# lazzati-astro/MCRaT

Hardware: AMD Instinct MI355X
Metric: photon-scatter-events/sec at 1e6 photons, 2D FLASH jet (higher is better)
Workload: dtype f64

## Files before the change

include/mcrat_hip.h:

```cpp
#ifndef MCRAT_HIP_H
#define MCRAT_HIP_H

#include <stddef.h>
#include <stdint.h>

#ifdef __cplusplus
extern "C" {
#endif
#if defined(__GNUC__)
#pragma GCC visibility push(default)
#endif

#define MCRAT_HIP_ABI_VERSION 1

#define MCRAT_HIP_OK        0
#define MCRAT_HIP_EINVAL   (-1)
#define MCRAT_HIP_ENODEV   (-2)
#define MCRAT_HIP_ENOMEM   (-3)
#define MCRAT_HIP_EHIP     (-4)
#define MCRAT_HIP_ESTATE   (-5)
#define MCRAT_HIP_EREFUSED (-6)

#define MCRAT_HIP_CARTESIAN        0
#define MCRAT_HIP_SPHERICAL        1
// ... 251 lines not shown
#define MCRAT_HIP_MODE_FAST  1
int mcrat_hip_propagate_frame_mode(mcrat_hip_ctx *ctx, double *time_now, double remaining_time, uint64_t seed, int mode, int fast_windows,
                                   mcrat_hip_frame_stats *stats);
int mcrat_hip_pool_propagate_frames_fast(mcrat_hip_ctx *pool, const int *open, const uint64_t *seeds, const double *time_now,
                                         const double *remaining_time, int fast_windows, mcrat_hip_frame_stats *stats);
int mcrat_hip_fast_cadence(mcrat_hip_ctx *ctx, int set_windows);

int mcrat_hip_begin_frame(mcrat_hip_ctx *ctx, uint64_t seed, double time_now, double remaining_time);
int mcrat_hip_run(mcrat_hip_ctx *ctx, long long max_iterations, mcrat_hip_frame_stats *stats);

int mcrat_hip_snapshot_photons(mcrat_hip_ctx *ctx);
int mcrat_hip_restore_photons(mcrat_hip_ctx *ctx);

int mcrat_hip_num_virtual_ranks(const mcrat_hip_ctx *ctx);
int mcrat_hip_rank_stats(mcrat_hip_ctx *ctx, int rank, mcrat_hip_frame_stats *stats);

typedef struct mcrat_hip_rank_summary {
    double min_r, max_r, min_theta, max_theta;
    double avg_scatt, avg_r;
    double avg_energy;
    int    max_scatt, min_scatt;
    int    num_output;
    int    list_capacity;
} mcrat_hip_rank_summary;
int mcrat_hip_profile_totals(const mcrat_hip_ctx *ctx, double *loop_kernel_ms, long long *loop_kernel_launches);
int mcrat_hip_pool_create(mcrat_hip_ctx *pool, int n_ranks, int slots_per_rank);
int mcrat_hip_pool_rank(mcrat_hip_ctx *pool, int rank, uint32_t rng_stream, mcrat_hip_ctx **view);
int mcrat_hip_pool_summaries(mcrat_hip_ctx *pool, mcrat_hip_rank_summary *out );
typedef struct mcrat_hip_pool_cs_list {
    int      open;
    int      emit_pool;
    int      scatt_frame_number, inj_frame_number;
    uint64_t seed;
    double   time_now, remaining_time;
    double   r_inj, ph_weight_suggest, theta_min, theta_max;
} mcrat_hip_pool_cs_list;
int mcrat_hip_pool_scatter_frames_cyclosynch(mcrat_hip_ctx *pool, const mcrat_hip_cyclosynch *cs, int max_photons, double fps,
                                             const mcrat_hip_pool_cs_list *lists, mcrat_hip_frame_stats *stats, mcrat_hip_cyclosynch_counts *counts);
typedef struct mcrat_hip_pool_inject_list {
    int      inject;
    char     spect;
    int      min_photons, max_photons;
    double   r_inj, ph_weight, theta_min, theta_max;
    uint64_t seed;
    int      num_photons;
    double   ph_weight_adjusted;
    int      status;
} mcrat_hip_pool_inject_list;
int mcrat_hip_pool_inject_photons(mcrat_hip_ctx *pool, double fps, mcrat_hip_pool_inject_list *lists);
int mcrat_hip_pool_set_photons(mcrat_hip_ctx *pool, int count, const int *rank_of, const mcrat_hip_photon_list *lists);
int mcrat_hip_pool_begin_frames(mcrat_hip_ctx *pool, const int *open, const uint64_t *seeds, const double *time_now, const double *remaining_time);
int mcrat_hip_pool_frame_stats(mcrat_hip_ctx *pool, mcrat_hip_frame_stats *out );
int mcrat_hip_pool_layout(const mcrat_hip_ctx *pool, int *n_ranks, int *slots_per_rank);
typedef struct mcrat_hip_frame_plan {
    int n_frames;
    int chain_clock;
    int restore_each_frame;
    int capture_frames;
    const int      *open;
    const uint64_t *seeds;
    const double   *time_now;
    const double   *remaining_time;
    const double   *frame_end;
    mcrat_hip_ctx *const *hydro;
} mcrat_hip_frame_plan;
int mcrat_hip_pool_run_frames(mcrat_hip_ctx *pool, const mcrat_hip_frame_plan *plan, mcrat_hip_frame_stats *stats );

int mcrat_hip_pool_select_frame(mcrat_hip_ctx *pool, int frame);

int mcrat_hip_step_locate_sample(mcrat_hip_ctx *ctx, int find_nearest_block_switch);
int mcrat_hip_frame_statistics(mcrat_hip_ctx *ctx, mcrat_hip_frame_stats *stats);
int mcrat_hip_update_photon_position(mcrat_hip_ctx *ctx, double t);
int mcrat_hip_step_event(mcrat_hip_ctx *ctx, mcrat_hip_frame_stats *stats);

size_t mcrat_hip_shared_clock_bytes_per_rank(void);
int mcrat_hip_shared_clock_attach(mcrat_hip_ctx *ctx, int world, int rank, long long slot_base, void *send, void *recv);
int mcrat_hip_shared_clock_buffers(mcrat_hip_ctx *ctx, void **send, void **recv);
int mcrat_hip_shared_clock_attach_device(mcrat_hip_ctx *ctx, int world, int rank, long long slot_base);
int mcrat_hip_shared_clock_peer_buffers(mcrat_hip_ctx *ctx, void **recv, size_t *recv_bytes, void **flags, size_t *flags_bytes);
int mcrat_hip_shared_clock_set_peers(mcrat_hip_ctx *ctx, void *const *peer_recv, void *const *peer_flags);
int mcrat_hip_shared_clock_exchange_push(mcrat_hip_ctx *ctx);
int mcrat_hip_shared_clock_exchange_wait(mcrat_hip_ctx *ctx);
int mcrat_hip_shared_clock_exchange(mcrat_hip_ctx *ctx);
int mcrat_hip_shared_clock_reset_exchange(mcrat_hip_ctx *ctx);
int mcrat_hip_shared_clock_propose(mcrat_hip_ctx *ctx);
int mcrat_hip_shared_clock_resolve(mcrat_hip_ctx *ctx);
int mcrat_hip_shared_clock_poll(mcrat_hip_ctx *ctx, int *frame_done, mcrat_hip_frame_stats *stats);
int mcrat_hip_shared_clock_finish(mcrat_hip_ctx *ctx, mcrat_hip_frame_stats *stats);

int mcrat_hip_set_rng_tape(mcrat_hip_ctx *ctx, const double *uniforms, long long n);
int mcrat_hip_rng_tape_position(mcrat_hip_ctx *ctx, long long *position, int *ran_out);

int mcrat_hip_pool_set_rng_tapes(mcrat_hip_ctx *pool, const double *const *uniforms , const long long *n );
int mcrat_hip_pool_rng_tape_positions(mcrat_hip_ctx *pool, long long *position , int *ran_out );

#define MCRAT_HIP_FN_KN_CROSS_SECTION       1
#define MCRAT_HIP_FN_LORENTZ_BOOST_PHOTON   2
#define MCRAT_HIP_FN_LORENTZ_BOOST_ELECTRON 3
#define MCRAT_HIP_FN_STOKES_ROTATION        4
#define MCRAT_HIP_FN_THERMAL_ELECTRON       5
#define MCRAT_HIP_FN_THERMAL_ELECTRON_WAVE  6
#define MCRAT_HIP_FN_ELECTRON_AND_SCATTER   7
#define MCRAT_HIP_FN_RCP_NR                 8
#define MCRAT_HIP_FN_RSQRT_NR               9
#define MCRAT_HIP_FN_SQRT_NR               10
#define MCRAT_HIP_FN_CELL_OPERANDS         11
#define MCRAT_HIP_FN_BOOST_WITH_PHOTON     12
#define MCRAT_HIP_FN_BOOST_WITH_ELECTRON   13
#define MCRAT_HIP_FN_BOOST_STAGED_PHOTON   14
#define MCRAT_HIP_FN_OPTICAL_DEPTH_STAGED  15
#define MCRAT_HIP_FN_AZIMUTH               16
#define MCRAT_HIP_FN_HYDRO_COORDS          17
#define MCRAT_HIP_FN_THERMAL_CROSS_SECTION 18
#define MCRAT_HIP_FN_KN_CROSS_SECTION_IEEE 19
#define MCRAT_HIP_FN_COUNT                 20
int mcrat_hip_eval_function(mcrat_hip_ctx *ctx, int fn, int n, const double *in, double *out, uint64_t seed);

int mcrat_hip_ph_minmax(mcrat_hip_ctx *ctx, double *min_r, double *max_r, double *min_theta, double *max_theta);
int mcrat_hip_scatt_stats(mcrat_hip_ctx *ctx, int *max_scatt, int *min_scatt, double *avg_scatt, double *avg_r);
int mcrat_hip_avg_energy(mcrat_hip_ctx *ctx, double *erg);

typedef struct mcrat_hip_observer {
    int n_obs; const double *cos_obs, *sin_obs, *cos_lo, *cos_hi;
    int n_t;   const double *t_edges;
    int n_e;   const double *e_edges;
} mcrat_hip_observer;
typedef struct mcrat_hip_observation {
    long long *count; double *w, *we, *i, *q, *u, *v;
    long long *n_accepted, *n_outside;
} mcrat_hip_observation;
int mcrat_hip_observe(mcrat_hip_ctx *ctx, const mcrat_hip_observer *obs, double time_now, mcrat_hip_observation *out);
int mcrat_hip_pool_observe(mcrat_hip_ctx *pool, const mcrat_hip_observer *obs, const double *time_now , mcrat_hip_observation *out);
int mcrat_hip_observe_path(const mcrat_hip_ctx *ctx);

#define MCRAT_HIP_SIGHTLINE_SKIPPED 0
#define MCRAT_HIP_SIGHTLINE_LEFT_MESH 1
#define MCRAT_HIP_SIGHTLINE_OPAQUE 2
#define MCRAT_HIP_SIGHTLINE_STEP_CAP 3
#define MCRAT_HIP_SIGHTLINE_OFF_TABLE 4
typedef struct mcrat_hip_sightline_params { double step_frac, h_min; int max_steps; double tau_stop, surface_level; } mcrat_hip_sightline_params;
typedef struct mcrat_hip_sightlines {
    double *tau, *path; int *steps, *status; int *surface_step; double *surface_r0, *surface_r1, *surface_r2;
    long long n_status[5];
} mcrat_hip_sightlines;
int mcrat_hip_sightline_rays(mcrat_hip_ctx *ctx, const mcrat_hip_ctx *hydro , const mcrat_hip_sightline_params *params, int n,
                             const double *r0, const double *r1, const double *r2, const double *p0, const double *p1, const double *p2,
                             const double *p3 , mcrat_hip_sightlines *out);
int mcrat_hip_sightline_photons(mcrat_hip_ctx *ctx, const mcrat_hip_ctx *hydro, const mcrat_hip_sightline_params *params, mcrat_hip_sightlines *out);
int mcrat_hip_pool_sightline_photons(mcrat_hip_ctx *pool, const mcrat_hip_ctx *hydro, const mcrat_hip_sightline_params *params, mcrat_hip_sightlines *out);

int mcrat_hip_synchronize(mcrat_hip_ctx *ctx);
size_t mcrat_hip_device_bytes(const mcrat_hip_ctx *ctx);
int mcrat_hip_lookup_cell(mcrat_hip_ctx *ctx, int n, const double *a0, const double *a1, const double *a2, int *cell_out);

#if defined(__GNUC__)
#pragma GCC visibility pop
#endif
#ifdef __cplusplus
}
#endif
#endif
```

mcrat_amd/csrc/device_types.hpp:

```cpp
#pragma once
#include <stddef.h>
#include <stdint.h>

namespace mcrat {

constexpr double A_RAD = 7.56e-15;
constexpr double C_LIGHT = 2.99792458e10;
constexpr double PL_CONST = 6.6260755e-27;
constexpr double K_B = 1.380658e-16;
constexpr double M_P = 1.6726231e-24;
constexpr double THOM_X_SECT = 6.65246e-25;
constexpr double M_EL = 9.1093879e-28;

constexpr int GEOM_CARTESIAN = 0, GEOM_SPHERICAL = 1, GEOM_CYLINDRICAL = 2, GEOM_POLAR = 3;
constexpr int DIM_TWO = 0, DIM_TWO_POINT_FIVE = 1, DIM_THREE = 2;

constexpr unsigned FLAG_RECALC = 1u;
constexpr unsigned FLAG_MOVES = 2u;
constexpr unsigned FLAG_VALID = 4u;
constexpr unsigned FLAG_TAU_FRESH = 8u;

constexpr int TOPK = 4;
constexpr int MAX_SEG = 8;
constexpr int STEP_BLOCK = 256;
constexpr int STEP_QCAP = 1024;
#ifndef MCRAT_EVENT_BLOCK
#define MCRAT_EVENT_BLOCK 256
#endif
constexpr int SHORTLIST_CAP = MCRAT_EVENT_BLOCK;
constexpr int EVENT_BLOCK = MCRAT_EVENT_BLOCK;

struct PhotonDev {
    double *r0, *r1, *r2;
    double *p0, *p1, *p2, *p3;
    double *c0, *c1, *c2, *c3;
    double *s0, *s1, *s2, *s3;
    double *num_scatt;
    double *weight;
    double *tau;
    double *tts;
    double *u0, *u1, *u2;
    double *ntau;
    double *tau_next;
    int *idx;
    unsigned char *flags;
    char *type;
    int n;
    int n_pad;
    unsigned col_stride;
};
#if defined(__HIPCC__)
__host__ __device__
#endif
inline void offset_photons(PhotonDev &ph, size_t first)
{
    double **cols[24] = {&ph.r0, &ph.r1, &ph.r2, &ph.p0, &ph.p1, &ph.p2, &ph.p3, &ph.c0, &ph.c1, &ph.c2, &ph.c3, &ph.s0, &ph.s1, &ph.s2, &ph.s3,
                         &ph.num_scatt, &ph.weight, &ph.tau, &ph.tts, &ph.u0, &ph.u1, &ph.u2, &ph.ntau, &ph.tau_next};
    for (int k = 0; k < 24; ++k) *cols[k] += first;
    ph.idx += first; ph.flags += first; ph.type += first;
}

struct alignas(32) CellGeom {
    double c0, c1, s0, s1;
};
struct alignas(16) CellGeom2 {
    double c2, s2;
};
struct alignas(32) CellFluid {
    double a, b, c, w;
    double nsig, gam, kf, pad;
};
#if defined(__HIPCC__)
__host__ __device__
#endif
inline void cell_staged_operands(double a, double b, double c, double gamma_cell, double dens_lab, CellFluid &f)
{
    const double beta_g = __builtin_sqrt(1.0 - 1.0 / (gamma_cell * gamma_cell));
    const double v2 = (a * a + b * b) + c * c;
    f.a = a; f.b = b; f.c = c;
    f.w = beta_g / __builtin_sqrt(v2);
    f.nsig = (dens_lab / M_P) * THOM_X_SECT;
    f.gam = 1.0 / __builtin_sqrt(1.0 - v2);
    f.kf = (f.gam * f.gam) / (f.gam + 1.0);
    f.pad = 0.0;
}

struct alignas(32) FatCell {
    double c0, c1, s0, s1;
    double a, b, w, nsig;
    double gam;
    int cell;
    int pad;
    double c;
    double c2, s2;
    double pad2[3];
};
static_assert(sizeof(FatCell) == 128, "one cache line per bucket-list entry");

constexpr unsigned GRID_NO_HINT = 15u;
constexpr int GRID_CODE_OCT_SHIFT = 27;
constexpr int GRID_CODE_HINT_OK = 1 << 30;
constexpr int GRID_CODE_BUCKET_MASK = (1 << GRID_CODE_OCT_SHIFT) - 1;
struct alignas(16) BucketDir {
    int e0;
    int n;
    unsigned hints;
    unsigned pad;
};

struct GridDev {
    const BucketDir *dir;
    const FatCell *cells;
    double org[3];
    double inv[3];
    int dim[3];
    int logmap[3];
    int naxes;
};

struct HydroDev {
    const CellGeom *geom;
    const CellGeom2 *geom2;
    const CellFluid *fluid;
    const double *temp;
    const double *fluid_c;
    const double *gamma;
    const double *k2e;
    int M;
    double dom0[2], dom1[2], dom2[2];
    GridDev grid;
    const double *hot_table;
    int hot_n_ph_e, hot_n_t;
    double hot_e0, hot_de, hot_t0, hot_dt;
    int *table_fallbacks;
    int hot_fallback_calls;
};

struct alignas(16) Cand {
    double t;
    int idx;
    int pad;
};

struct alignas(256) LoopState {
    double remaining_time;
    double time_now;
    unsigned long long iteration;
    int done;
    int nseg;
    int skip_idx;
    int last_scattered_index;
    double seg[MAX_SEG];
    double last_time_step;
    double last_scattered_temp;
    long long iterations;
    long long frame_scatt_cnt;
    long long n_relocated;
    long long not_found;
    long long kn_rejections;
    long long rescans;
    double t_cut;
    double t_est;
    int force_relocate;
    int photon_event_called;
    union {
        long long stamps[8];
        long long slot_steps;
    };
};

struct alignas(16) Shortlist {
    int count;
    int pad[3];
    Cand items[SHORTLIST_CAP];
};

struct alignas(16) RankDesc {
    int len;
    uint32_t stream;
    uint64_t seed;
};

struct RngKey {
    uint64_t seed;
    uint32_t stream;
    uint32_t slot_base;
};

constexpr int SC_K = 4;
constexpr int SC_MAX_WORLD = 16;
constexpr int LOOP_DONE = 1;
constexpr int LOOP_MIDPASS = 2;
constexpr int LOOP_SC_GAVE_UP = 4;

struct alignas(16) ScRecord {
    double t;
    long long gid;
    double r[3], u[3], p[4], pc[4], s[4];
    int cell;
    unsigned flags;
};

struct alignas(16) ScProposal {
    int n;
    int pad0;
    long long horizon_gid;
    double horizon_t;
    double pad1;
    ScRecord rec[SC_K];
};

struct alignas(64) ScState {
    double cursor_t;
    long long cursor_gid;
    double old_scatt_time;
    double t_first;
    double cut_mid;
    int first;
    int pad0;
    long long rounds, midpass_rounds;
};

}
```

mcrat_amd/csrc/engine.hip:

```cpp
#include <hip/hip_runtime.h>
#include <algorithm>
#include <chrono>
#include <cmath>
#include <cstdio>
#include <cstdlib>
#include <cstring>
#include <mutex>
#include <new>
#include <string>
#include <vector>

#include "../../include/mcrat_hip.h"
#include "device_types.hpp"
#include "launch.hpp"
#include "observe_plan.hpp"
#include "sightline_plan.hpp"
#include "photon_cols.hpp"
#include "photon_plan.hpp"
#include "rng.hpp"

using namespace mcrat;

static_assert(sizeof(mcrat_hip_photon) == 176, "struct photon layout (Src/mcrat.h:142-171) must be 176 bytes");
static_assert(offsetof(mcrat_hip_photon, num_scatt) == 128 && offsetof(mcrat_hip_photon, recalc_properties) == 136 &&
// ... 360 lines not shown
    if (c->obs_buf) (void)hipFree(c->obs_buf);
    if (c->sl_buf) (void)hipFree(c->sl_buf);
    if (c->own_stream && c->stream) (void)hipStreamDestroy(c->stream);
    delete c;
}

extern "C" int mcrat_hip_bind_thread(mcrat_hip_ctx *c)
{
    if (!c) return MCRAT_HIP_EINVAL;
    if (hipSetDevice(c->cfg.device) != hipSuccess) return MCRAT_HIP_ENODEV;
    return MCRAT_HIP_OK;
}

extern "C" int mcrat_hip_synchronize(mcrat_hip_ctx *c)
{
    if (!c) return MCRAT_HIP_EINVAL;
    HIPCHK(c, hipStreamSynchronize(c->stream));
    return MCRAT_HIP_OK;
}

extern "C" size_t mcrat_hip_device_bytes(const mcrat_hip_ctx *c)
{
    if (!c) return 0;
    return c->ph_bytes + c->hy_bytes + c->grid_bytes + c->grid_count_cap * sizeof(unsigned) + sizeof(Shortlist) + sizeof(LoopState) + c->partials_bytes +
           sizeof(ReducePartial) * mcrat_hip_ctx::RED_BLOCKS + c->obs_bytes + c->sl_bytes;
}

extern "C" int mcrat_hip_create_hot_cross_section(mcrat_hip_ctx *c, double *thermal_table, int n_ph_e, int n_t, double log_ph_e_min,
                                                  double log_ph_e_max, double log_t_min, double log_t_max, long long calls, uint64_t seed)
{
    if (!c || !thermal_table || n_ph_e < 1 || n_t < 1 || n_ph_e > 100000 || n_t > 100000 || calls < 1 || !(log_ph_e_max > log_ph_e_min) ||
        !(log_t_max > log_t_min))
        return MCRAT_HIP_EINVAL;
    const size_t count = (size_t)(n_ph_e + 1) * (size_t)(n_t + 1);
    if (count > 0x7fffffffull) return MCRAT_HIP_EINVAL;
    double *d = nullptr;
    HIPCHK(c, hipMalloc((void **)&d, count * sizeof(double)));
    HotTableParams p{n_ph_e, n_t, log_ph_e_min, log_ph_e_max, log_t_min, log_t_max, calls, (unsigned long long)seed};
    __atomic_store_n(&c->hot_creating, 1, __ATOMIC_RELEASE);
    hipError_t e = launch_hot_table(p, d, c->stream);
    if (e == hipSuccess) e = hipMemcpyAsync(thermal_table, d, count * sizeof(double), hipMemcpyDeviceToHost, c->stream);
    if (e == hipSuccess) e = hipStreamSynchronize(c->stream);
    __atomic_store_n(&c->hot_creating, 0, __ATOMIC_RELEASE);
    (void)hipFree(d);
    HIPCHK(c, e);
    return MCRAT_HIP_OK;
}


static void apply_hot_table(mcrat_hip_ctx *c)
{
    HydroDev &hy = c->hy;
    const bool table = c->cfg.tau_calculation == MCRAT_HIP_TAU_TABLE && c->d_hot_table;
    hy.hot_table = table ? c->d_hot_table : nullptr;
    hy.hot_n_ph_e = c->hot_n_ph_e; hy.hot_n_t = c->hot_n_t;
    hy.hot_e0 = c->hot_grid[0]; hy.hot_t0 = c->hot_grid[2];
    hy.hot_de = table ? (c->hot_grid[1] - c->hot_grid[0]) / c->hot_n_ph_e : 0.0;
    hy.hot_dt = table ? (c->hot_grid[3] - c->hot_grid[2]) / c->hot_n_t : 0.0;
    hy.table_fallbacks = c->d_table_fallbacks;
    hy.hot_fallback_calls = c->hot_fallback_calls;
}

extern "C" int mcrat_hip_table_fallback_calls(mcrat_hip_ctx *c, int calls)
{
    if (!c) return MCRAT_HIP_EINVAL;
    if (calls > 0) {
        c->hot_fallback_calls = calls;
        apply_hot_table(c);
        drop_graph(c);
        sync_views(c);
    }
    return c->hot_fallback_calls;
}

extern "C" int mcrat_hip_set_hot_cross_section(mcrat_hip_ctx *c, const double *thermal_table, int n_ph_e, int n_t,
                                               double log_ph_e_min, double log_ph_e_max, double log_t_min, double log_t_max)
{
    if (!c || !thermal_table || n_ph_e < 1 || n_t < 1 || !(log_ph_e_max > log_ph_e_min) || !(log_t_max > log_t_min)) return MCRAT_HIP_EINVAL;
    if (c->parent) return view_refuses(c, "set_hot_cross_section");
    if (c->cfg.tau_calculation != MCRAT_HIP_TAU_TABLE) { c->last_error = "the context was created with TAU_CALCULATION == DIRECT"; return MCRAT_HIP_ESTATE; }
    const size_t count = (size_t)(n_ph_e + 1) * (size_t)(n_t + 1);
    for (size_t k = 0; k < count; ++k)
        if (!(thermal_table[k] == thermal_table[k])) { c->last_error = "NaN in the cross-section table"; return MCRAT_HIP_EINVAL; }
    HIPCHK(c, hipStreamSynchronize(c->stream));
    release_shared_hydro(c);
    detach_sharers(c, "replaced its cross-section table");
    if (c->d_hot_table) { (void)hipFree(c->d_hot_table); c->d_hot_table = nullptr; }
    HIPCHK(c, hipMalloc((void **)&c->d_hot_table, count * sizeof(double)));
    HIPCHK(c, hipMemcpy(c->d_hot_table, thermal_table, count * sizeof(double), hipMemcpyHostToDevice));
    c->hot_n_ph_e = n_ph_e; c->hot_n_t = n_t;
    c->hot_grid[0] = log_ph_e_min; c->hot_grid[1] = log_ph_e_max; c->hot_grid[2] = log_t_min; c->hot_grid[3] = log_t_max;
    apply_hot_table(c);
    drop_graph(c);
    sync_views(c);
    return MCRAT_HIP_OK;
}

static int ensure_aos(mcrat_hip_ctx *c, size_t bytes);
static int flush_pending(mcrat_hip_ctx *c);

static void sync_views(mcrat_hip_ctx *c)
{
    for (mcrat_hip_ctx *v : c->views) {
        if (!v) continue;
        v->hy = c->hy;
        v->hcol = c->hcol; v->hcol_buf = c->hcol_buf; v->hcol_M = c->hcol_M;
        v->have_hydro = c->have_hydro;
        v->d_hot_table = c->d_hot_table; v->hot_n_ph_e = c->hot_n_ph_e; v->hot_n_t = c->hot_n_t;
        v->hot_fallback_calls = c->hot_fallback_calls;
        for (int k = 0; k < 4; ++k) v->hot_grid[k] = c->hot_grid[k];
        drop_graph(v);
    }
}

static int ensure_counts(mcrat_hip_ctx *c, size_t n)
{
    if (c->parent) {
        int rc = ensure_counts(c->parent, n);
        c->grid_count = c->parent->grid_count; c->grid_count_cap = c->parent->grid_count_cap; c->d_grid_total = c->parent->d_grid_total;
        return rc;
    }
    if (!c->d_grid_total) HIPCHK(c, hipMalloc((void **)&c->d_grid_total, sizeof(unsigned long long)));
    if (c->grid_count_cap < n) {
        if (c->grid_count) { HIPCHK(c, hipFree(c->grid_count)); c->grid_count = nullptr; c->grid_count_cap = 0; }
        HIPCHK(c, hipMalloc((void **)&c->grid_count, sizeof(unsigned) * n));
        c->grid_count_cap = n;
    }
    return MCRAT_HIP_OK;
}

static int view_refuses(mcrat_hip_ctx *c, const char *what)
{
    c->last_error = std::string(what) + ": a rank view shares its pool's hydro frame; call this on the pool context";
    return MCRAT_HIP_ESTATE;
}

static int capture_refuses(mcrat_hip_ctx *c, const char *what)
{
    if (c->selected_frame < 0) return MCRAT_HIP_OK;
    c->last_error = std::string(what) + ": a captured frame is selected (mcrat_hip_pool_select_frame(pool, -1) first)";
    return MCRAT_HIP_ESTATE;
}

namespace {

struct HydroStage {
    mcrat_hip_ctx *c;
    int M, naxes;
    CellLayout cells{};
    GridLayout grid{};
    GridScale scale{};
    GridPlan plan{};
    long long nb = 0, entries = 0;
    bool any_hot = false;
    template <class T> T *cell_at(size_t o) const { return reinterpret_cast<T *>(static_cast<char *>(c->hy_buf) + o); }
    template <class T> T *grid_at(size_t o) const { return reinterpret_cast<T *>(static_cast<char *>(c->grid_buf) + o); }
};
struct HostFrame {
    const mcrat_hip_hydro *h;
    GridHost grid;
    std::vector<char> image;
};

int host_build_grid(HydroStage &s, HostFrame &hf)
{
    const mcrat_hip_hydro *h = hf.h;
    const double *ctr[3] = {h->r0, h->r1, h->r2}, *size[3] = {h->r0_size, h->r1_size, h->r2_size};
    if (!build_grid(ctr, size, s.M, s.naxes, hf.grid)) { s.c->last_error = "cell-lookup grid: degenerate mesh"; return MCRAT_HIP_EINVAL; }
    s.plan = hf.grid.plan; s.nb = hf.grid.nb; s.entries = (long long)hf.grid.cells.size();
    for (int i = 0; i < s.M; ++i) s.any_hot = s.any_hot || (h->temp[i] >= 1e7);
    return MCRAT_HIP_OK;
}

int ensure_cell_buffer(HydroStage &s, bool reserve_k2e)
{
    mcrat_hip_ctx *c = s.c;
    s.cells = cell_layout(c->kc.dimensions, s.M, reserve_k2e);
    HIPCHK(c, hipStreamSynchronize(c->stream));
    return ensure_device_bytes(c, &c->hy_buf, &c->hy_bytes, s.cells.total);
}

int stage_cells_device(HydroStage &s)
{
    mcrat_hip_ctx *c = s.c;
    const CellLayout &l = s.cells;
    const int M = s.M, nblk = stage_cells_blocks(M), stride = plan_stride(M), nsamp = (M + stride - 1) / stride;
    const size_t scratch_bytes = sizeof(StagePartial) * (size_t)nblk + sizeof(double) * 2 * s.naxes * (size_t)nsamp;
    int rc = ensure_aos(c, scratch_bytes);
    if (rc) return rc;
    StagePartial *d_part = static_cast<StagePartial *>(c->aos_buf);
    double *d_samp = reinterpret_cast<double *>(d_part + nblk);
    HIPCHK(c, launch_stage_cells(c->kc.dimensions, c->kc.geometry, c->hcol, M, s.cell_at<CellGeom>(l.geom), l.has_geom2 ? s.cell_at<CellGeom2>(l.geom2) : nullptr,
                                 s.cell_at<CellFluid>(l.fluid), l.has_fluid_c ? s.cell_at<double>(l.fluid_c) : nullptr, s.cell_at<double>(l.temp),
                                 s.cell_at<double>(l.gamma), d_part, d_samp, stride, nsamp, c->stream));
    std::vector<char> hs(scratch_bytes);
    HIPCHK(c, hipMemcpyAsync(hs.data(), c->aos_buf, scratch_bytes, hipMemcpyDeviceToHost, c->stream));
    HIPCHK(c, hipStreamSynchronize(c->stream));
    const StagePartial *part = reinterpret_cast<const StagePartial *>(hs.data());
    const MeshStats ms = mesh_stats_from_partials(part, nblk, reinterpret_cast<const double *>(part + nblk), nsamp, s.naxes, &s.any_hot);
    if (!grid_plan_from_stats(ms, M, s.naxes, s.scale)) { c->last_error = "cell-lookup grid: degenerate mesh"; return MCRAT_HIP_EINVAL; }
    return MCRAT_HIP_OK;
}

int stage_cells_host(HydroStage &s, HostFrame &hf)
{
    mcrat_hip_ctx *c = s.c;
    const mcrat_hip_hydro *h = hf.h;
    const CellLayout &l = s.cells;
    const int M = s.M;
    hf.image.assign(l.total, 0);
    char *host = hf.image.data();
    CellGeom *geom = reinterpret_cast<CellGeom *>(host + l.geom);
    CellFluid *fluid = reinterpret_cast<CellFluid *>(host + l.fluid);
    double *fc = l.has_fluid_c ? reinterpret_cast<double *>(host + l.fluid_c) : nullptr;
    for (int i = 0; i < M; ++i) {
        geom[i].c0 = h->r0[i]; geom[i].c1 = h->r1[i]; geom[i].s0 = h->r0_size[i]; geom[i].s1 = h->r1_size[i];
        double v[3];
        cell_velocity_staged(c->kc.dimensions, c->kc.geometry, h->v0[i], h->v1[i], l.has_fluid_c ? h->v2[i] : 0.0, h->r1[i], l.has_geom2 ? h->r2[i] : 0.0, v);
        if (fc) fc[i] = v[2];
        cell_staged_operands(v[0], v[1], v[2], h->gamma[i], h->dens_lab[i], fluid[i]);
    }
    if (l.has_geom2) {
        CellGeom2 *g2 = reinterpret_cast<CellGeom2 *>(host + l.geom2);
        for (int i = 0; i < M; ++i) { g2[i].c2 = h->r2[i]; g2[i].s2 = h->r2_size[i]; }
    }
    memcpy(host + l.temp, h->temp, sizeof(double) * M);
    memcpy(host + l.gamma, h->gamma, sizeof(double) * M);
    HIPCHK(c, hipMemcpy(c->hy_buf, host, l.total, hipMemcpyHostToDevice));
    return MCRAT_HIP_OK;
}

void publish_cells(HydroStage &s, const double *dom0, const double *dom1, const double *dom2)
{
    const CellLayout &l = s.cells;
    HydroDev &hy = s.c->hy;
    hy.geom = s.cell_at<const CellGeom>(l.geom);
    hy.geom2 = l.has_geom2 ? s.cell_at<const CellGeom2>(l.geom2) : nullptr;
    hy.fluid = s.cell_at<const CellFluid>(l.fluid);
    hy.temp = s.cell_at<const double>(l.temp);
    hy.fluid_c = l.has_fluid_c ? s.cell_at<const double>(l.fluid_c) : nullptr;
    hy.k2e = s.any_hot ? s.cell_at<const double>(l.k2e) : nullptr;
    hy.gamma = s.cell_at<const double>(l.gamma);
    hy.M = s.M;
    hy.dom0[0] = dom0[0]; hy.dom0[1] = dom0[1];
    hy.dom1[0] = dom1[0]; hy.dom1[1] = dom1[1];
    hy.dom2[0] = dom2[0]; hy.dom2[1] = dom2[1];
}

int count_grid_entries(HydroStage &s, const GridPlan &plan, long long nb, unsigned long long *total)
{
    mcrat_hip_ctx *c = s.c;
    { int rc = ensure_counts(c, (size_t)nb); if (rc) return rc; }
    HIPCHK(c, grid_count(plan, c->hy.geom, c->hy.geom2, s.M, c->grid_count, nb, c->d_grid_total, c->stream));
    HIPCHK(c, hipMemcpyAsync(total, c->d_grid_total, sizeof *total, hipMemcpyDeviceToHost, c->stream));
    HIPCHK(c, hipStreamSynchronize(c->stream));
    return MCRAT_HIP_OK;
}
int choose_scale_device(HydroStage &s)
{
    mcrat_hip_ctx *c = s.c;
    int rc = ensure_counts(c, 1);
    if (rc) return rc;
    const GridChoice ch = choose_grid_scale(s.scale, s.M, [&](const GridPlan &plan, long long nb, long long) {
        unsigned long long total = 0;
        rc = count_grid_entries(s, plan, nb, &total);
        return rc ? -1LL : (long long)std::min(total, 0x7fffffffffffffffull);
    });
    if (ch.result == GRID_SCALE_ABANDONED) return rc;
    if (ch.result != GRID_SCALE_OK) { c->last_error = "cell-lookup grid: no bucket size fits this mesh"; return MCRAT_HIP_EINVAL; }
    s.plan = ch.plan; s.nb = ch.nb; s.entries = ch.entries;
    if (getenv("MCRAT_HIP_VERBOSE"))
        fprintf(stderr, "mcrat_hip: cell-lookup grid %d x %d x %d buckets, %lld entries for %d cells (%.2f per bucket), built on the device\n",
                s.plan.dim[0], s.plan.dim[1], s.plan.dim[2], s.entries, s.M, (double)s.entries / (double)s.nb);
    return MCRAT_HIP_OK;
}

int ensure_grid_buffer(HydroStage &s)
{
    s.grid = grid_layout(s.nb, s.entries, grid_scan_scratch_ints(s.nb));
    return ensure_device_bytes(s.c, &s.c->grid_buf, &s.c->grid_bytes, s.grid.total);
}

int build_grid_device(HydroStage &s)
{
    mcrat_hip_ctx *c = s.c;
    const GridLayout &g = s.grid;
    HIPCHK(c, grid_build(s.plan, c->hy.geom, c->hy.geom2, c->hy.fluid, c->hy.fluid_c, s.M, c->grid_count, s.grid_at<int>(g.start), s.grid_at<int>(g.scan),
                         s.grid_at<int>(g.entries), s.grid_at<FatCell>(g.cells), s.grid_at<BucketDir>(g.dir), s.nb, s.entries, c->stream));
    HIPCHK(c, hipStreamSynchronize(c->stream));
    return MCRAT_HIP_OK;
}

int upload_host_grid(HydroStage &s, const HostFrame &hf)
{
    const GridHost &g = hf.grid;
    const CellGeom *geom = reinterpret_cast<const CellGeom *>(hf.image.data() + s.cells.geom);
    const CellFluid *fluid = reinterpret_cast<const CellFluid *>(hf.image.data() + s.cells.fluid);
    const bool three = s.cells.has_geom2;
    std::vector<char> gh(s.grid.start, 0);
    BucketDir *dir = reinterpret_cast<BucketDir *>(gh.data() + s.grid.dir);
    for (size_t b = 0; b < (size_t)s.nb; ++b) {
        dir[b].e0 = g.start[b]; dir[b].n = g.start[b + 1] - g.start[b]; dir[b].hints = g.hints[b]; dir[b].pad = 0;
    }
    FatCell *fat = reinterpret_cast<FatCell *>(gh.data() + s.grid.cells);
    for (size_t e = 0; e < g.cells.size(); ++e) {
        const int ci = g.cells[e];
        fat[e] = fat_cell(geom[ci], fluid[ci], three ? hf.h->r2[ci] : 0.0, three ? hf.h->r2_size[ci] : 0.0, ci);
    }
    HIPCHK(s.c, hipMemcpy(s.c->grid_buf, gh.data(), s.grid.start, hipMemcpyHostToDevice));
    return MCRAT_HIP_OK;
}

void publish_grid(HydroStage &s)
{
    HydroDev &hy = s.c->hy;
    hy.grid.dir = s.grid_at<const BucketDir>(s.grid.dir);
    hy.grid.cells = s.grid_at<const FatCell>(s.grid.cells);
    grid_plan_to_dev(s.plan, hy.grid);
    apply_hot_table(s.c);
}

int finish_frame(HydroStage &s)
{
    mcrat_hip_ctx *c = s.c;
    if (s.any_hot) {
        HIPCHK(c, launch_k2e(c->hy.temp, s.cell_at<double>(s.cells.k2e), s.M, c->stream));
        HIPCHK(c, hipStreamSynchronize(c->stream));
    }
    c->have_hydro = true;
    drop_graph(c);
    sync_views(c);
    return MCRAT_HIP_OK;
}

}

static int stage_hydro_device(HydroStage &s, const double *dom0, const double *dom1, const double *dom2)
{
    int rc;
    if ((rc = ensure_cell_buffer(s, true))) return rc;
    if ((rc = stage_cells_device(s))) return rc;
    publish_cells(s, dom0, dom1, dom2);
    if ((rc = choose_scale_device(s))) return rc;
    if ((rc = ensure_grid_buffer(s))) return rc;
    if ((rc = build_grid_device(s))) return rc;
    publish_grid(s);
    return finish_frame(s);
}
static int stage_hydro_host(HydroStage &s, const mcrat_hip_hydro *h, const double *dom0, const double *dom1, const double *dom2)
{
    HostFrame hf{h};
    int rc;
    if ((rc = host_build_grid(s, hf))) return rc;
    if ((rc = ensure_cell_buffer(s, s.any_hot))) return rc;
    if ((rc = stage_cells_host(s, hf))) return rc;
    publish_cells(s, dom0, dom1, dom2);
    if ((rc = ensure_grid_buffer(s))) return rc;
    if ((rc = upload_host_grid(s, hf))) return rc;
    publish_grid(s);
    return finish_frame(s);
}
static int stage_hydro(mcrat_hip_ctx *c, const mcrat_hip_hydro *h, int M, const double *dom0, const double *dom1, const double *dom2)
{
    if (c->hydro_owner) { c->last_error = "stage_hydro on a context that reads another one's frame"; return MCRAT_HIP_ESTATE; }
    HydroStage s{c, M, c->kc.dimensions == DIM_THREE ? 3 : 2};
    return h ? stage_hydro_host(s, h, dom0, dom1, dom2) : stage_hydro_device(s, dom0, dom1, dom2);
}

static void release_shared_hydro(mcrat_hip_ctx *c)
{
    std::lock_guard<std::mutex> lock(g_share_mutex);
    if (!c->hydro_owner) return;
    auto &v = c->hydro_owner->hydro_sharers;
    v.erase(std::remove(v.begin(), v.end(), c), v.end());
    forget_shared_frame(c);
}

extern "C" int mcrat_hip_share_hydro(mcrat_hip_ctx *c, mcrat_hip_ctx *owner)
{
    if (!c || !owner || c == owner) return MCRAT_HIP_EINVAL;
    if (c->parent) return view_refuses(c, "share_hydro");
    if (owner->parent) owner = owner->parent;
    if (!owner->have_hydro || owner->hydro_owner == c) return MCRAT_HIP_ESTATE;
    if (owner->hydro_owner) owner = owner->hydro_owner;
    if (c->kc.dimensions != owner->kc.dimensions || c->kc.geometry != owner->kc.geometry || c->kc.table != owner->kc.table ||
        c->cfg.device != owner->cfg.device) {
        c->last_error = "share_hydro: the two contexts differ in DIMENSIONS / GEOMETRY / TAU_CALCULATION or device";
        return MCRAT_HIP_EINVAL;
    }
    HIPCHK(c, hipStreamSynchronize(c->stream));
    HIPCHK(c, hipStreamSynchronize(owner->stream));
    release_shared_hydro(c);
    detach_sharers(c, "shares another context's frame now");
    if (c->hy_buf) { HIPCHK(c, hipFree(c->hy_buf)); c->hy_buf = nullptr; c->hy_bytes = 0; }
    if (c->grid_buf) { HIPCHK(c, hipFree(c->grid_buf)); c->grid_buf = nullptr; c->grid_bytes = 0; }
    if (c->hcol_buf) { HIPCHK(c, hipFree(c->hcol_buf)); c->hcol_buf = nullptr; c->hcol_bytes = 0; }
    if (c->d_hot_table) { HIPCHK(c, hipFree(c->d_hot_table)); c->d_hot_table = nullptr; }
    c->hy = owner->hy;
    c->hcol = owner->hcol; c->hcol_buf = owner->hcol_buf; c->hcol_M = owner->hcol_M;
    c->d_hot_table = owner->d_hot_table; c->hot_n_ph_e = owner->hot_n_ph_e; c->hot_n_t = owner->hot_n_t;
    for (int k = 0; k < 4; ++k) c->hot_grid[k] = owner->hot_grid[k];
    apply_hot_table(c);
    c->have_hydro = true;
    {
        std::lock_guard<std::mutex> lock(g_share_mutex);
        c->hydro_owner = owner;
        owner->hydro_sharers.push_back(c);
    }
    c->frame_open = false;
    drop_graph(c);
    sync_views(c);
    return MCRAT_HIP_OK;
}

static int ensure_hcol(mcrat_hip_ctx *c, int M)
{
    release_shared_hydro(c);
    detach_sharers(c, "staged another frame");
    const size_t stride = align_up(sizeof(double) * (size_t)M, 256), total = 19 * stride;
    HIPCHK(c, hipStreamSynchronize(c->stream));
    { int rc = ensure_device_bytes(c, &c->hcol_buf, &c->hcol_bytes, total); if (rc) return rc; }
    char *b = static_cast<char *>(c->hcol_buf);
    double **cols[19] = {&c->hcol.r0, &c->hcol.r1, &c->hcol.r2, &c->hcol.s0, &c->hcol.s1, &c->hcol.s2, &c->hcol.v0, &c->hcol.v1, &c->hcol.v2,
                         &c->hcol.dens, &c->hcol.dens_lab, &c->hcol.pres, &c->hcol.temp, &c->hcol.gamma, &c->hcol.r, &c->hcol.theta,
                         &c->hcol.B0, &c->hcol.B1, &c->hcol.B2};
    for (int k = 0; k < 19; ++k) *cols[k] = reinterpret_cast<double *>(b + k * stride);
    c->hcol_M = M;
    return MCRAT_HIP_OK;
}

extern "C" int mcrat_hip_set_hydro(mcrat_hip_ctx *c, const mcrat_hip_hydro *h)
{
    if (!c || !h || h->num_elements <= 0) return MCRAT_HIP_EINVAL;
    if (c->parent) return view_refuses(c, "set_hydro");
    const int M = h->num_elements;
    const bool three = c->kc.dimensions == DIM_THREE, two = c->kc.dimensions == DIM_TWO;
    if (!h->r0 || !h->r1 || !h->r0_size || !h->r1_size || !h->v0 || !h->v1 || !h->dens_lab || !h->temp || !h->gamma) return MCRAT_HIP_EINVAL;
    if (three && (!h->r2 || !h->r2_size)) return MCRAT_HIP_EINVAL;
    if (!two && !h->v2) return MCRAT_HIP_EINVAL;
    c->have_hydro = false;
    sync_views(c);
    int rc = ensure_hcol(c, M);
    if (rc) return rc;
    HIPCHK(c, hipMemsetAsync(c->hcol_buf, 0, c->hcol_bytes, c->stream));
    const struct { double *dst; const double *src; } copy[12] = {
        {c->hcol.r0, h->r0}, {c->hcol.r1, h->r1}, {c->hcol.r2, three ? h->r2 : nullptr}, {c->hcol.s0, h->r0_size}, {c->hcol.s1, h->r1_size},
        {c->hcol.s2, three ? h->r2_size : nullptr}, {c->hcol.v0, h->v0}, {c->hcol.v1, h->v1}, {c->hcol.v2, !two ? h->v2 : nullptr},
        {c->hcol.dens_lab, h->dens_lab}, {c->hcol.temp, h->temp}, {c->hcol.gamma, h->gamma}};
    for (const auto &cp : copy)
        if (cp.src) HIPCHK(c, hipMemcpyAsync(cp.dst, cp.src, sizeof(double) * (size_t)M, hipMemcpyHostToDevice, c->stream));
    HIPCHK(c, launch_fill_spherical(c->kc.dimensions, c->kc.geometry, c->hcol, M, c->stream));
    return stage_hydro(c, getenv("MCRAT_HIP_HOST_GRID") ? h : nullptr, M, h->r0_domain, h->r1_domain, h->r2_domain);
}

extern "C" void mcrat_hip_outflow_defaults(int simulation_type, mcrat_hip_outflow *o)
{
    if (!o) return;
    memset(o, 0, sizeof *o);
    o->simulation_type = simulation_type;
    if (simulation_type == MCRAT_HIP_CYLINDRICAL_OUTFLOW) { o->gamma_infinity = 100; o->t_comov = 1e5; o->ddensity = 3e-7; }
    if (simulation_type == MCRAT_HIP_SPHERICAL_OUTFLOW) { o->gamma_infinity = 100; o->lumi = 1e54; o->r00 = 1e8; }
    if (simulation_type == MCRAT_HIP_STRUCTURED_SPHERICAL_OUTFLOW) { o->gamma_infinity = 100; o->lumi = 1e52; o->r00 = 1e8; o->theta_j = 1e-2; o->p = 4; }
}

namespace {

struct RawPacker {
    mcrat_hip_ctx *c;
    size_t off = 0;
    std::vector<std::pair<size_t, std::pair<const void *, size_t>>> items;
    size_t add(const void *src, size_t bytes) { const size_t o = off; off = align_up(off + bytes, 256); items.push_back({o, {src, bytes}}); return o; }
// ... 2965 lines not shown
    double *d_in = reinterpret_cast<double *>(d + plan.out_bytes);
    ObserveDev a{};
    a.n_slots = n_slots; a.n_obs = plan.n_obs; a.n_t = plan.n_t; a.n_e = plan.n_e; a.n_bins = plan.n_bins;
    a.staged = d_in;
    a.clocks = clocks ? d_in + plan.staged_doubles : nullptr;
    a.slots_per_clock = slots_per_clock;
    a.time_now = time_now;
    a.cube = reinterpret_cast<double *>(d);
    a.n_accepted = reinterpret_cast<unsigned long long *>(d + plan.cube_bytes);
    a.n_outside = a.n_accepted + n_obs;
    HIPCHK(c, hipMemsetAsync(d, 0, plan.out_bytes, c->stream));
    HIPCHK(c, hipMemcpyAsync(d_in, in.data(), sizeof(double) * in.size(), hipMemcpyHostToDevice, c->stream));
    HIPCHK(c, launch_observe(c->ph, a, plan, c->kc.stokes != 0, device_cus(c), c->stream));
    const size_t plane = sizeof(double) * (size_t)plan.n_bins;
    void *planes[OBSERVE_PLANES] = {out->count, out->w, out->we, out->i, out->q, out->u, out->v};
    static_assert(sizeof(long long) == 8, "the count plane is read back as it is");
    for (int k = 0; k < OBSERVE_PLANES; ++k)
        if (planes[k]) HIPCHK(c, hipMemcpyAsync(planes[k], d + plane * (size_t)k, plane, hipMemcpyDeviceToHost, c->stream));
    if (out->n_accepted) HIPCHK(c, hipMemcpyAsync(out->n_accepted, a.n_accepted, sizeof(long long) * n_obs, hipMemcpyDeviceToHost, c->stream));
    if (out->n_outside) HIPCHK(c, hipMemcpyAsync(out->n_outside, a.n_outside, sizeof(long long) * n_obs, hipMemcpyDeviceToHost, c->stream));
    HIPCHK(c, hipStreamSynchronize(c->stream));
    c->obs_path = plan.path;
    return MCRAT_HIP_OK;
}

extern "C" int mcrat_hip_observe(mcrat_hip_ctx *c, const mcrat_hip_observer *obs, double time_now, mcrat_hip_observation *out)
{
    if (!c || !obs || !out) return MCRAT_HIP_EINVAL;
    if (!c->have_photons) return MCRAT_HIP_ESTATE;
    if (c->is_pool) { c->last_error = "observe: a rank pool's lists have clocks of their own (mcrat_hip_pool_observe, or mcrat_hip_observe on a view)"; return MCRAT_HIP_ESTATE; }
    int rc = flush_pending(c);
    if (rc) return rc;
    return observe_run(c, obs, c->ph.n, nullptr, 0, 1, time_now, out);
}

extern "C" int mcrat_hip_pool_observe(mcrat_hip_ctx *c, const mcrat_hip_observer *obs, const double *time_now, mcrat_hip_observation *out)
{
    if (!c || !obs || !time_now || !out) return MCRAT_HIP_EINVAL;
    if (!c->is_pool) return MCRAT_HIP_ESTATE;
    return observe_run(c, obs, c->ph.n, time_now, c->n_ranks, c->rank_stride, 0.0, out);
}

extern "C" int mcrat_hip_observe_path(const mcrat_hip_ctx *c) { return c ? c->obs_path : 0; }

static int sightline_run(mcrat_hip_ctx *c, const mcrat_hip_ctx *hydro, const mcrat_hip_sightline_params *params, int n, const double *const *rays,
                         mcrat_hip_sightlines *out)
{
    const mcrat_hip_ctx *h = hydro ? hydro : c;
    if (!h->have_hydro) { c->last_error = "sightline: no staged hydro frame"; return MCRAT_HIP_ESTATE; }
    if (h != c && (h->kc.dimensions != c->kc.dimensions || h->kc.geometry != c->kc.geometry || h->kc.table != c->kc.table || h->cfg.device != c->cfg.device)) {
        c->last_error = "sightline: a frame staged on a context with other switches (DIMENSIONS, GEOMETRY, TAU_CALCULATION) or on another device";
        return MCRAT_HIP_EINVAL;
    }
    if (c->kc.table && !h->hy.hot_table) {
        c->last_error = "TAU_CALCULATION == TABLE needs mcrat_hip_set_hot_cross_section first";
        return MCRAT_HIP_ESTATE;
    }
    const SightlineParams p{params->step_frac, params->h_min, params->max_steps, params->tau_stop, params->surface_level};
    int forced;
    SightlinePlan plan;
    const SightlineRefusal bad_switch = sightline_refill_switch(getenv("MCRAT_HIP_SIGHTLINE_REFILL"), &forced);
    SightlineRefusal why = sightline_plan(n, p, forced, &plan);
    if (why == SIGHTLINE_OK) why = bad_switch;
    if (why != SIGHTLINE_OK) { c->last_error = sightline_refusal_text(why); return MCRAT_HIP_EINVAL; }

    mcrat_hip_ctx *owner = c->parent ? c->parent : c;
    HIPCHK(c, hipStreamSynchronize(c->stream));
    if (h != c) HIPCHK(c, hipStreamSynchronize(h->stream));
    int rc = ensure_device_bytes(c, &owner->sl_buf, &owner->sl_bytes, plan.ray_offset + (rays ? plan.ray_bytes : 0));
    if (rc) return rc;
    char *d = static_cast<char *>(owner->sl_buf);
    const int blocks = sightline_grid(plan, device_cus(c));
    SightlineDev a{};
    a.n = n;
    a.step_frac = p.step_frac; a.h_min = p.h_min; a.max_steps = p.max_steps; a.tau_stop = p.tau_stop; a.surface_level = p.surface_level;
    a.head = reinterpret_cast<unsigned long long *>(d);
    a.f8 = reinterpret_cast<double *>(d + plan.f8_offset);
    a.i4 = reinterpret_cast<int *>(d + plan.i4_offset);
    a.refill = plan.refill ? 1 : 0;
    a.own_rays = plan.refill ? sightline_own_rays(n, blocks) : 0;
    HIPCHK(c, hipMemsetAsync(d, 0, sizeof(unsigned long long) * SIGHTLINE_HEAD_WORDS, c->stream));
    if (rays) {
        double *d_ray = reinterpret_cast<double *>(d + plan.ray_offset);
        for (int k = 0; k < SIGHTLINE_RAY_PLANES; ++k)
            HIPCHK(c, hipMemcpyAsync(d_ray + (size_t)k * (size_t)n, rays[k], sizeof(double) * (size_t)n, hipMemcpyHostToDevice, c->stream));
        a.ray = d_ray;
    }
    HIPCHK(c, launch_sightline(c->kc, c->ph, h->hy, a, blocks, c->stream));
    double *f8[SIGHTLINE_F8_PLANES] = {out->tau, out->path, out->surface_r0, out->surface_r1, out->surface_r2};
    int *i4[SIGHTLINE_I4_PLANES] = {out->steps, out->status, out->surface_step};
    for (int k = 0; k < SIGHTLINE_F8_PLANES; ++k)
        if (f8[k]) HIPCHK(c, hipMemcpyAsync(f8[k], d + sightline_f8_plane(plan, k), sizeof(double) * (size_t)n, hipMemcpyDeviceToHost, c->stream));
    for (int k = 0; k < SIGHTLINE_I4_PLANES; ++k)
        if (i4[k]) HIPCHK(c, hipMemcpyAsync(i4[k], d + sightline_i4_plane(plan, k), sizeof(int) * (size_t)n, hipMemcpyDeviceToHost, c->stream));
    static_assert(sizeof(long long) == 8, "the status counts are read back as they are");
    HIPCHK(c, hipMemcpyAsync(out->n_status, d, sizeof(long long) * SIGHTLINE_N_STATUS, hipMemcpyDeviceToHost, c->stream));
    HIPCHK(c, hipStreamSynchronize(c->stream));
    return MCRAT_HIP_OK;
}

extern "C" int mcrat_hip_sightline_rays(mcrat_hip_ctx *c, const mcrat_hip_ctx *hydro, const mcrat_hip_sightline_params *params, int n, const double *r0,
                                        const double *r1, const double *r2, const double *p0, const double *p1, const double *p2, const double *p3,
                                        mcrat_hip_sightlines *out)
{
    if (!c || !params || !out) return MCRAT_HIP_EINVAL;
    if (n > 0 && (!r0 || !r1 || !r2 || !p0 || !p1 || !p2 || !p3)) { c->last_error = "sightline: a null ray array"; return MCRAT_HIP_EINVAL; }
    if (c->have_photons) {
        int rc = flush_pending(c);
        if (rc) return rc;
    }
    const double *const rays[SIGHTLINE_RAY_PLANES] = {r0, r1, r2, p0, p1, p2, p3};
    return sightline_run(c, hydro, params, n, rays, out);
}

extern "C" int mcrat_hip_sightline_photons(mcrat_hip_ctx *c, const mcrat_hip_ctx *hydro, const mcrat_hip_sightline_params *params, mcrat_hip_sightlines *out)
{
    if (!c || !params || !out) return MCRAT_HIP_EINVAL;
    if (!c->have_photons) return MCRAT_HIP_ESTATE;
    if (c->is_pool) { c->last_error = "sightline: one list is a stand-alone context or a view of a pool (mcrat_hip_pool_sightline_photons takes the pool)"; return MCRAT_HIP_ESTATE; }
    int rc = flush_pending(c);
    if (rc) return rc;
    return sightline_run(c, hydro, params, c->ph.n, nullptr, out);
}

extern "C" int mcrat_hip_pool_sightline_photons(mcrat_hip_ctx *c, const mcrat_hip_ctx *hydro, const mcrat_hip_sightline_params *params, mcrat_hip_sightlines *out)
{
    if (!c || !params || !out) return MCRAT_HIP_EINVAL;
    if (!c->is_pool) return MCRAT_HIP_ESTATE;
    int rc = flush_pending(c);
    if (rc) return rc;
    return sightline_run(c, hydro, params, c->ph.n, nullptr, out);
}

extern "C" int mcrat_hip_eval_function(mcrat_hip_ctx *c, int fn, int n, const double *in, double *out, uint64_t seed)
{
    static const int in_w[MCRAT_HIP_FN_COUNT] = {0, 1, 7, 7, 13, 5, 5, 9, 1, 1, 1, 5, 9, 9, 7, 9, 2, 3, 2, 1};
    static const int out_w[MCRAT_HIP_FN_COUNT] = {0, 1, 4, 4, 4, 4, 4, 13, 1, 1, 1, 5, 4, 4, 4, 2, 4, 3, 4, 1};
    if (!c || n <= 0 || !in || !out || fn < 1 || fn >= MCRAT_HIP_FN_COUNT) return MCRAT_HIP_EINVAL;
    if (fn == MCRAT_HIP_FN_THERMAL_CROSS_SECTION && __atomic_load_n(&c->hot_creating, __ATOMIC_ACQUIRE)) return MCRAT_HIP_EINVAL;
    const size_t bi = sizeof(double) * (size_t)in_w[fn] * (size_t)n, bo = sizeof(double) * (size_t)out_w[fn] * (size_t)n;
    double *d_in = nullptr, *d_out = nullptr;
    HIPCHK(c, hipMalloc((void **)&d_in, bi));
    if (hipMalloc((void **)&d_out, bo) != hipSuccess) { (void)hipFree(d_in); return MCRAT_HIP_ENOMEM; }
    hipError_t e = hipMemcpyAsync(d_in, in, bi, hipMemcpyHostToDevice, c->stream);
    if (e == hipSuccess) e = launch_eval_function(c->kc, c->hy, fn, n, d_in, d_out, seed, c->key.stream, c->stream);
    if (e == hipSuccess) e = hipMemcpyAsync(out, d_out, bo, hipMemcpyDeviceToHost, c->stream);
    if (e == hipSuccess) e = hipStreamSynchronize(c->stream);
    (void)hipFree(d_in);
    (void)hipFree(d_out);
    HIPCHK(c, e);
    return MCRAT_HIP_OK;
}

extern "C" int mcrat_hip_lookup_cell(mcrat_hip_ctx *c, int n, const double *a0, const double *a1, const double *a2, int *out)
{
    if (!c || n <= 0 || !a0 || !a1 || !out) return MCRAT_HIP_EINVAL;
    if (!c->have_hydro) return MCRAT_HIP_ESTATE;
    double *d = nullptr;
    int *dout = nullptr;
    HIPCHK(c, hipMalloc((void **)&d, sizeof(double) * 3 * (size_t)n));
    if (hipMalloc((void **)&dout, sizeof(int) * (size_t)n) != hipSuccess) { (void)hipFree(d); return MCRAT_HIP_ENOMEM; }
    int rc = MCRAT_HIP_OK;
    std::vector<double> zeros;
    if (!a2) { zeros.assign(n, 0.0); a2 = zeros.data(); }
    if (hipMemcpy(d, a0, sizeof(double) * n, hipMemcpyHostToDevice) != hipSuccess ||
        hipMemcpy(d + n, a1, sizeof(double) * n, hipMemcpyHostToDevice) != hipSuccess ||
        hipMemcpy(d + 2 * (size_t)n, a2, sizeof(double) * n, hipMemcpyHostToDevice) != hipSuccess ||
        launch_lookup(c->kc, c->hy, n, d, d + n, d + 2 * (size_t)n, dout, c->stream) != hipSuccess ||
        hipStreamSynchronize(c->stream) != hipSuccess ||
        hipMemcpy(out, dout, sizeof(int) * n, hipMemcpyDeviceToHost) != hipSuccess) {
        c->last_error = "lookup_cell failed";
        rc = MCRAT_HIP_EHIP;
    }
    (void)hipFree(d);
    (void)hipFree(dout);
    return rc;
}
```

mcrat_amd/csrc/grid_build.hip:

```cpp
#include <hip/hip_runtime.h>
#include <math.h>
#include "device_types.hpp"
#include "launch.hpp"

namespace mcrat {

namespace {

__device__ __forceinline__ int bucket_of(double x, int logmap, double org, double inv, int dim)
{
    const double u = logmap ? log(x) : x;
    const double f = floor((u - org) * inv);
    if (!(f == f)) return 0;
    if (f < 0.0) return 0;
    if (f > (double)(dim - 1)) return dim - 1;
    return (int)f;
}

struct CellBox {
    double c[3], s[3];
};

__device__ __forceinline__ CellBox load_box(const CellGeom *geom, const CellGeom2 *geom2, int i, int naxes)
{
// ... 1 lines not shown
    CellBox b;
    b.c[0] = g.c0; b.c[1] = g.c1; b.s[0] = g.s0; b.s[1] = g.s1;
    b.c[2] = 0; b.s[2] = 0;
    if (naxes == 3) { const CellGeom2 g2 = geom2[i]; b.c[2] = g2.c2; b.s[2] = g2.s2; }
    return b;
}

__device__ __forceinline__ void bucket_range(const GridPlan &p, const CellBox &b, int lo[3], int hi[3])
{
#pragma unroll
    for (int k = 0; k < 3; ++k) {
        lo[k] = 0; hi[k] = 0;
        if (k < p.naxes) {
            const double m = 1e-9 * (fabs(b.c[k]) + b.s[k]);
            double a = b.c[k] - 0.5 * b.s[k] - m;
            const double e = b.c[k] + 0.5 * b.s[k] + m;
            if (p.logmap[k] && a <= 0) a = 1e-300;
            lo[k] = bucket_of(a, p.logmap[k], p.org[k], p.inv[k], p.dim[k]);
            hi[k] = bucket_of(e, p.logmap[k], p.org[k], p.inv[k], p.dim[k]);
        }
    }
}

__global__ __launch_bounds__(256) void grid_count_kernel(GridPlan p, const CellGeom *__restrict__ geom, const CellGeom2 *__restrict__ geom2, int M,
                                                         unsigned *__restrict__ count, unsigned long long *__restrict__ total)
{
    __shared__ unsigned long long s_sum[4];
    const int i = blockIdx.x * 256 + threadIdx.x;
    unsigned long long mine = 0;
    if (i < M) {
        const CellBox b = load_box(geom, geom2, i, p.naxes);
        int lo[3], hi[3];
        bucket_range(p, b, lo, hi);
        mine = (unsigned long long)(hi[0] - lo[0] + 1) * (hi[1] - lo[1] + 1) * (hi[2] - lo[2] + 1);
        if (mine > 4096) mine = 1ull << 40;
        else
            for (int z = lo[2]; z <= hi[2]; ++z)
                for (int y = lo[1]; y <= hi[1]; ++y)
                    for (int x = lo[0]; x <= hi[0]; ++x) atomicAdd(&count[((size_t)z * p.dim[1] + y) * p.dim[0] + x], 1u);
    }
    for (int off = 32; off > 0; off >>= 1) mine += __shfl_xor(mine, off, 64);
    if ((threadIdx.x & 63) == 0) s_sum[threadIdx.x >> 6] = mine;
    __syncthreads();
    if (threadIdx.x == 0) atomicAdd(total, s_sum[0] + s_sum[1] + s_sum[2] + s_sum[3]);
}

constexpr int SCAN_PER_BLOCK = 2048;

__global__ __launch_bounds__(256) void scan_blocks_kernel(const unsigned *__restrict__ count, long long n, int *__restrict__ start, int *__restrict__ sums)
{
    __shared__ int s_w[4];
    const long long base = (long long)blockIdx.x * SCAN_PER_BLOCK + (long long)threadIdx.x * 8;
    int v[8], acc = 0;
#pragma unroll
    for (int k = 0; k < 8; ++k) {
        const long long e = base + k;
        const int c = (e < n) ? (int)count[e] : 0;
        v[k] = acc;
        acc += c;
    }
    int incl = acc;
    const int lane = threadIdx.x & 63, w = threadIdx.x >> 6;
    for (int off = 1; off < 64; off <<= 1) {
        const int o = __shfl_up(incl, off, 64);
        if (lane >= off) incl += o;
    }
    if (lane == 63) s_w[w] = incl;
    __syncthreads();
    int wbase = 0;
    for (int k = 0; k < w; ++k) wbase += s_w[k];
    const int excl = wbase + incl - acc;
#pragma unroll
    for (int k = 0; k < 8; ++k) {
        const long long e = base + k;
        if (e < n) start[e] = excl + v[k];
    }
    if (threadIdx.x == 255) sums[blockIdx.x] = wbase + incl;
}

__global__ __launch_bounds__(256) void scan_sums_kernel(int *__restrict__ sums, int nblocks)
{
    __shared__ int s_w[4];
    __shared__ int s_carry;
    if (threadIdx.x == 0) s_carry = 0;
    __syncthreads();
    for (int b0 = 0; b0 < nblocks; b0 += 256) {
        const int e = b0 + threadIdx.x;
        const int c = (e < nblocks) ? sums[e] : 0;
        int incl = c;
        const int lane = threadIdx.x & 63, w = threadIdx.x >> 6;
        for (int off = 1; off < 64; off <<= 1) {
            const int o = __shfl_up(incl, off, 64);
            if (lane >= off) incl += o;
        }
        if (lane == 63) s_w[w] = incl;
        __syncthreads();
        int wbase = s_carry;
        for (int k = 0; k < w; ++k) wbase += s_w[k];
        if (e < nblocks) sums[e] = wbase + incl - c;
        __syncthreads();
        if (threadIdx.x == 255) s_carry = wbase + incl;
        __syncthreads();
    }
}

__global__ __launch_bounds__(256) void scan_add_kernel(int *__restrict__ start, long long n, const int *__restrict__ sums, int total)
{
    const long long e = (long long)blockIdx.x * 256 + threadIdx.x;
    if (e < n) start[e] += sums[e / SCAN_PER_BLOCK];
    if (e == n) start[e] = total;
}

__global__ __launch_bounds__(256) void grid_fill_kernel(GridPlan p, const CellGeom *__restrict__ geom, const CellGeom2 *__restrict__ geom2, int M,
                                                        const int *__restrict__ start, unsigned *__restrict__ cursor, int *__restrict__ entries)
{
    const int i = blockIdx.x * 256 + threadIdx.x;
    if (i >= M) return;
    const CellBox b = load_box(geom, geom2, i, p.naxes);
    int lo[3], hi[3];
    bucket_range(p, b, lo, hi);
    for (int z = lo[2]; z <= hi[2]; ++z)
        for (int y = lo[1]; y <= hi[1]; ++y)
            for (int x = lo[0]; x <= hi[0]; ++x) {
                const size_t bk = ((size_t)z * p.dim[1] + y) * p.dim[0] + x;
                const unsigned pos = atomicAdd(&cursor[bk], 1u);
                entries[start[bk] + (int)pos] = i;
            }
}

__device__ __forceinline__ double mapped(double x, int logmap) { return logmap ? log(fmax(x, 1e-300)) : x; }

__global__ __launch_bounds__(256) void grid_records_kernel(int naxes, long long total, const int *__restrict__ entries,
                                                           const CellGeom *__restrict__ geom, const CellGeom2 *__restrict__ geom2,
                                                           const CellFluid *__restrict__ fluid, const double *__restrict__ fluid_c,
                                                           FatCell *__restrict__ cells)
{
    const long long e = (long long)blockIdx.x * 256 + threadIdx.x;
    if (e >= total) return;
    const int ci = entries[e];
    const CellGeom g = geom[ci];
    const CellFluid f = fluid[ci];
    FatCell fc;
    fc.c0 = g.c0; fc.c1 = g.c1; fc.s0 = g.s0; fc.s1 = g.s1;
    fc.a = f.a; fc.b = f.b; fc.c = f.c; fc.w = f.w;
    fc.nsig = f.nsig; fc.gam = f.gam;
    fc.c2 = 0; fc.s2 = 0;
    if (naxes == 3) { const CellGeom2 g2 = geom2[ci]; fc.c2 = g2.c2; fc.s2 = g2.s2; }
    fc.cell = ci; fc.pad = 0; fc.pad2[0] = fc.pad2[1] = fc.pad2[2] = 0.0;
    cells[e] = fc;
}

__global__ __launch_bounds__(256) void grid_finish_kernel(GridPlan p, long long nb, const int *__restrict__ start, int *__restrict__ entries,
                                                          const CellGeom *__restrict__ geom, const CellGeom2 *__restrict__ geom2,
                                                          BucketDir *__restrict__ dir)
{
    const long long b = (long long)blockIdx.x * 256 + threadIdx.x;
    if (b >= nb) return;
    const int e0 = start[b], n = start[b + 1] - e0;
    for (int a = 1; a < n; ++a) {
        const int key = entries[e0 + a];
        int j = a - 1;
        while (j >= 0 && entries[e0 + j] > key) { entries[e0 + j + 1] = entries[e0 + j]; --j; }
        entries[e0 + j + 1] = key;
    }
    int bi[3];
    bi[0] = (int)(b % p.dim[0]);
    bi[1] = (int)((b / p.dim[0]) % p.dim[1]);
    bi[2] = (int)(b / ((long long)p.dim[0] * p.dim[1]));
    const int nocts = 1 << p.naxes;
    double olo[3][2] = {{0, 0}, {0, 0}, {0, 0}}, half[3] = {0, 0, 0};
    for (int k = 0; k < p.naxes; ++k) {
        const double w = 1.0 / p.inv[k];
        olo[k][0] = p.org[k] + (bi[k] + 0.0) * w;
        olo[k][1] = p.org[k] + (bi[k] + 0.5) * w;
        half[k] = 0.5 * w;
    }
    unsigned char cnt[8] = {0, 0, 0, 0, 0, 0, 0, 0}, first[8] = {0, 0, 0, 0, 0, 0, 0, 0};
    for (int e = 0; e < n; ++e) {
        const int ci = entries[e0 + e];
        const CellGeom g = geom[ci];
        double c2 = 0, s2 = 0;
        if (p.naxes == 3) { const CellGeom2 g2 = geom2[ci]; c2 = g2.c2; s2 = g2.s2; }
        const double cc[3] = {g.c0, g.c1, c2}, ss[3] = {g.s0, g.s1, s2};
        bool r[3][2] = {{true, true}, {true, true}, {true, true}};
        for (int k = 0; k < p.naxes; ++k) {
            const double m = 1e-9 * (fabs(cc[k]) + ss[k]);
            const double clo = mapped(cc[k] - 0.5 * ss[k] + m, p.logmap[k]), chi = mapped(cc[k] + 0.5 * ss[k] - m, p.logmap[k]);
            for (int h = 0; h < 2; ++h) r[k][h] = (clo < olo[k][h] + half[k]) && (chi > olo[k][h]);
        }
        for (int o = 0; o < nocts; ++o) {
            const bool reaches = r[0][o & 1] && r[1][(o >> 1) & 1] && r[2][(o >> 2) & 1];
            if (reaches) {
                if (cnt[o] == 0) first[o] = (unsigned char)(e < (int)GRID_NO_HINT ? e : GRID_NO_HINT);
                if (cnt[o] < 2) cnt[o] += 1;
            }
        }
    }
    unsigned hints = 0;
    for (int o = 0; o < 8; ++o) {
        const unsigned pick = (o < nocts && cnt[o] == 1) ? (unsigned)first[o] : GRID_NO_HINT;
        hints |= pick << (4 * o);
    }
    BucketDir d;
    d.e0 = e0; d.n = n; d.hints = hints; d.pad = 0;
    dir[b] = d;
}

}

hipError_t grid_count(const GridPlan &p, const CellGeom *geom, const CellGeom2 *geom2, int M, unsigned *count, long long nb,
                      unsigned long long *d_total, hipStream_t stream)
{
    hipError_t e = hipMemsetAsync(count, 0, sizeof(unsigned) * (size_t)nb, stream);
    if (e != hipSuccess) return e;
    if ((e = hipMemsetAsync(d_total, 0, sizeof(unsigned long long), stream)) != hipSuccess) return e;
    grid_count_kernel<<<dim3((M + 255) / 256), dim3(256), 0, stream>>>(p, geom, geom2, M, count, d_total);
    return hipGetLastError();
}

size_t grid_scan_scratch_ints(long long nb) { return (size_t)((nb + SCAN_PER_BLOCK - 1) / SCAN_PER_BLOCK) + 1; }

hipError_t launch_exclusive_scan(const unsigned *count, long long n, int *start, int *scratch, long long total, hipStream_t stream)
{
    const int nblocks = (int)((n + SCAN_PER_BLOCK - 1) / SCAN_PER_BLOCK);
    scan_blocks_kernel<<<dim3(nblocks), dim3(256), 0, stream>>>(count, n, start, scratch);
    scan_sums_kernel<<<dim3(1), dim3(256), 0, stream>>>(scratch, nblocks);
    scan_add_kernel<<<dim3((unsigned)((n + 1 + 255) / 256)), dim3(256), 0, stream>>>(start, n, scratch, (int)total);
    return hipGetLastError();
}

hipError_t grid_build(const GridPlan &p, const CellGeom *geom, const CellGeom2 *geom2, const CellFluid *fluid, const double *fluid_c, int M,
                      unsigned *count, int *start, int *scan_scratch, int *entries, FatCell *cells, BucketDir *dir, long long nb,
                      long long total, hipStream_t stream)
{
    hipError_t e = launch_exclusive_scan(count, nb, start, scan_scratch, total, stream);
    if (e != hipSuccess) return e;
    e = hipMemsetAsync(count, 0, sizeof(unsigned) * (size_t)nb, stream);
    if (e != hipSuccess) return e;
    grid_fill_kernel<<<dim3((M + 255) / 256), dim3(256), 0, stream>>>(p, geom, geom2, M, start, count, entries);
    grid_finish_kernel<<<dim3((unsigned)((nb + 255) / 256)), dim3(256), 0, stream>>>(p, nb, start, entries, geom, geom2, dir);
    if (total > 0)
        grid_records_kernel<<<dim3((unsigned)((total + 255) / 256)), dim3(256), 0, stream>>>(p.naxes, total, entries, geom, geom2, fluid, fluid_c, cells);
    return hipGetLastError();
}

}
```

mcrat_amd/csrc/hydro_plan.hpp:

```cpp
#pragma once
#include <math.h>
#include <stddef.h>
#include <stdio.h>
#include <stdlib.h>
#include <string.h>
#include <algorithm>
#include <vector>
#include "../../include/mcrat_hip.h"
#include "device_types.hpp"

namespace mcrat {

struct GridPlan {
    double org[3], inv[3];
    int dim[3], logmap[3];
    int naxes;
};
struct StagePartial {
    double lo[3], hi[3], smin[3], smax[3];
    int any_hot, pad;
};
struct SlabDev {
    int dimensions, geometry, ph_inj_switch;
    double r_inj_095;
    double r_lo, r_hi, th_lo, th_hi;
};
struct ChomboBox {
    long long first_cell;
    long long data_off;
    int level;
    int lo[3], n[3];
    int cb[3];
    int pad[2];
};


inline int bucket_of(double x, int logmap, double org, double inv, int dim)
{
    double u = logmap ? log(x) : x;
    double f = floor((u - org) * inv);
    if (!(f == f)) return 0;
    if (f < 0.0) return 0;
    if (f > (double)(dim - 1)) return dim - 1;
    return (int)f;
}

struct MeshStats {
    double lo[3], hi[3], smin[3], smax[3];
    std::vector<double> sc[3], ss[3];
};
inline int plan_stride(int M) { return std::max(1, M / 4096); }

inline MeshStats mesh_stats_from_columns(const double *const c[3], const double *const s[3], int M, int naxes)
{
    MeshStats ms{};
    for (int k = 0; k < naxes; ++k) {
        double lo = INFINITY, hi = -INFINITY, smin = INFINITY, smax = 0;
        for (int i = 0; i < M; ++i) {
            lo = std::min(lo, c[k][i] - 0.5 * s[k][i]);
            hi = std::max(hi, c[k][i] + 0.5 * s[k][i]);
            smin = std::min(smin, s[k][i]);
            smax = std::max(smax, s[k][i]);
        }
        ms.lo[k] = lo; ms.hi[k] = hi; ms.smin[k] = smin; ms.smax[k] = smax;
        for (int i = 0; i < M; i += plan_stride(M)) { ms.sc[k].push_back(c[k][i]); ms.ss[k].push_back(s[k][i]); }
    }
    return ms;
}
inline MeshStats mesh_stats_from_partials(const StagePartial *part, int nblk, const double *samp, int nsamp, int naxes, bool *any_hot)
{
    MeshStats ms{};
    for (int k = 0; k < naxes; ++k) {
        double lo = INFINITY, hi = -INFINITY, smin = INFINITY, smax = 0;
        for (int b = 0; b < nblk; ++b) {
            lo = std::min(lo, part[b].lo[k]);
            hi = std::max(hi, part[b].hi[k]);
            smin = (part[b].smin[k] < smin || !(part[b].smin[k] == part[b].smin[k])) ? part[b].smin[k] : smin;
            smax = std::max(smax, part[b].smax[k]);
        }
        ms.lo[k] = lo; ms.hi[k] = hi; ms.smin[k] = smin; ms.smax[k] = smax;
        ms.sc[k].assign(samp + (size_t)(2 * k) * nsamp, samp + (size_t)(2 * k + 1) * nsamp);
        ms.ss[k].assign(samp + (size_t)(2 * k + 1) * nsamp, samp + (size_t)(2 * k + 2) * nsamp);
    }
    *any_hot = false;
    for (int b = 0; b < nblk; ++b) *any_hot = *any_hot || part[b].any_hot;
    return ms;
}

struct GridScale {
    double ext_lo[3] = {0, 0, 0}, ext_hi[3] = {0, 0, 0}, ncell[3] = {1, 1, 1}, f0 = 1.0;
    int logmap[3] = {0, 0, 0}, naxes = 2;
};
inline bool grid_plan_from_stats(const MeshStats &ms, int M, int naxes, GridScale &g)
{
    g.naxes = naxes;
    for (int k = 0; k < naxes; ++k) {
        const double lo = ms.lo[k], hi = ms.hi[k], smin = ms.smin[k], smax = ms.smax[k];
        if (!(hi > lo) || !(smin > 0)) return false;
        g.logmap[k] = (lo > 0 && smax / smin > 4.0) ? 1 : 0;
        std::vector<double> w;
        for (size_t i = 0; i < ms.sc[k].size(); ++i) {
            const double a = ms.sc[k][i] - 0.5 * ms.ss[k][i], b = ms.sc[k][i] + 0.5 * ms.ss[k][i];
            w.push_back(g.logmap[k] ? log(b) - log(std::max(a, 1e-300)) : b - a);
        }
        if (w.empty()) return false;
        std::nth_element(w.begin(), w.begin() + w.size() / 4, w.end());
        const double med = w[w.size() / 4];
        g.ext_lo[k] = g.logmap[k] ? log(lo) : lo;
        g.ext_hi[k] = g.logmap[k] ? log(hi) : hi;
        g.ncell[k] = std::max(1.0, (g.ext_hi[k] - g.ext_lo[k]) / med);
    }
    double prod = 1;
    for (int k = 0; k < naxes; ++k) prod *= g.ncell[k];
    const double target = std::min(std::max(4.0 * (double)M, 1.0), 16777216.0);
    g.f0 = (prod > target) ? pow(target / prod, 1.0 / naxes) : 1.0;
    return true;
}

inline GridPlan grid_dims(const GridScale &g, double f, long long *nb)
{
    GridPlan p{};
    p.naxes = g.naxes;
    *nb = 1;
    for (int k = 0; k < 3; ++k) {
        p.dim[k] = 1; p.org[k] = 0; p.inv[k] = 0; p.logmap[k] = g.logmap[k];
        if (k < g.naxes) {
            const int nbk = (int)std::max(1.0, std::min(65536.0, floor(g.ncell[k] * f)));
            const double width = (g.ext_hi[k] - g.ext_lo[k]) / nbk;
            p.dim[k] = nbk + 1;
            p.org[k] = g.ext_lo[k] - 0.5 * width;
            p.inv[k] = 1.0 / width;
        }
        *nb *= p.dim[k];
    }
    return p;
}
inline void grid_plan_to_dev(const GridPlan &p, GridDev &d)
{
    for (int k = 0; k < 3; ++k) { d.org[k] = p.org[k]; d.inv[k] = p.inv[k]; d.dim[k] = p.dim[k]; d.logmap[k] = p.logmap[k]; }
    d.naxes = p.naxes;
}

enum GridScaleResult { GRID_SCALE_OK = 0, GRID_SCALE_NONE_FITS, GRID_SCALE_ABANDONED };
struct GridChoice {
    GridScaleResult result;
    GridPlan plan;
    long long nb, entries;
};
template <class Count>
inline GridChoice choose_grid_scale(const GridScale &g, int M, Count count)
{
    GridChoice ch{};
    const long long limit = std::min(64LL * M + 1024, 2000000000LL);
    double f = g.f0;
    for (int attempt = 0; attempt < 12; ++attempt, f *= 0.5) {
        ch.plan = grid_dims(g, f, &ch.nb);
        if (ch.nb > (long long)GRID_CODE_BUCKET_MASK) continue;
        ch.entries = count(ch.plan, ch.nb, limit);
        if (ch.entries < 0) { ch.result = GRID_SCALE_ABANDONED; return ch; }
        if (ch.entries > limit) continue;
        ch.result = GRID_SCALE_OK;
        return ch;
    }
    ch.result = GRID_SCALE_NONE_FITS;
    return ch;
}

struct GridHost {
    GridPlan plan;
    long long nb = 0;
    std::vector<int> start, cells;
    std::vector<unsigned> hints;
};
inline void cell_bucket_range(const GridPlan &p, int k, double c, double s, int &b0, int &b1)
{
    const double m = 1e-9 * (fabs(c) + s);
    double a = c - 0.5 * s - m, b = c + 0.5 * s + m;
    if (p.logmap[k] && a <= 0) a = 1e-300;
    b0 = bucket_of(a, p.logmap[k], p.org[k], p.inv[k], p.dim[k]);
    b1 = bucket_of(b, p.logmap[k], p.org[k], p.inv[k], p.dim[k]);
}
inline unsigned bucket_hints(const GridPlan &p, const int bi[3], const int *list, int n, const double *const c[3], const double *const s[3])
{
    const int naxes = p.naxes, nocts = 1 << naxes;
    unsigned h = 0;
    for (int o = 0; o < 8; ++o) {
        unsigned pick = GRID_NO_HINT;
        if (o < nocts) {
            int found = 0;
            for (int e = 0; e < n && found < 2; ++e) {
                const int ci = list[e];
                bool reaches = true;
                for (int k = 0; k < naxes && reaches; ++k) {
                    const double w = 1.0 / p.inv[k];
                    const double olo = p.org[k] + (bi[k] + 0.5 * ((o >> k) & 1)) * w, ohi = olo + 0.5 * w;
                    const double m = 1e-9 * (fabs(c[k][ci]) + s[k][ci]);
                    double clo = c[k][ci] - 0.5 * s[k][ci] + m, chi = c[k][ci] + 0.5 * s[k][ci] - m;
                    if (p.logmap[k]) { clo = log(std::max(clo, 1e-300)); chi = log(std::max(chi, 1e-300)); }
                    reaches = (clo < ohi) && (chi > olo);
                }
                if (reaches) { found += 1; if (e < (int)GRID_NO_HINT) pick = (unsigned)e; else found = 2; }
            }
            if (found != 1) pick = GRID_NO_HINT;
        }
        h |= pick << (4 * o);
    }
    return h;
}
inline bool build_grid(const double *const c[3], const double *const s[3], int M, int naxes, GridHost &g)
{
    GridScale scale;
    if (!grid_plan_from_stats(mesh_stats_from_columns(c, s, M, naxes), M, naxes, scale)) return false;
    std::vector<long long> count;
    const GridChoice ch = choose_grid_scale(scale, M, [&](const GridPlan &p, long long nb, long long limit) {
        count.assign((size_t)nb + 1, 0);
        long long total = 0;
        for (int i = 0; i < M && total <= limit; ++i) {
            int lo[3] = {0, 0, 0}, hi[3] = {0, 0, 0};
            for (int k = 0; k < naxes; ++k) cell_bucket_range(p, k, c[k][i], s[k][i], lo[k], hi[k]);
            for (int z = lo[2]; z <= hi[2]; ++z)
                for (int y = lo[1]; y <= hi[1]; ++y)
                    for (int x = lo[0]; x <= hi[0]; ++x) count[((size_t)z * p.dim[1] + y) * p.dim[0] + x + 1]++;
            total += (long long)(hi[0] - lo[0] + 1) * (hi[1] - lo[1] + 1) * (hi[2] - lo[2] + 1);
        }
        return total;
    });
    if (ch.result != GRID_SCALE_OK) return false;
    const GridPlan &p = g.plan = ch.plan;
    const long long nb = g.nb = ch.nb, total = ch.entries;
    for (size_t b = 0; b < (size_t)nb; ++b) count[b + 1] += count[b];
    g.start.resize((size_t)nb + 1);
    for (size_t b = 0; b <= (size_t)nb; ++b) g.start[b] = (int)count[b];
    if (getenv("MCRAT_HIP_VERBOSE"))
        fprintf(stderr, "mcrat_hip: cell-lookup grid %d x %d x %d buckets, %lld entries for %d cells (%.2f per bucket)\n",
                p.dim[0], p.dim[1], p.dim[2], total, M, (double)total / (double)nb);
    g.cells.assign((size_t)total, -1);
    std::vector<int> fill(g.start.begin(), g.start.end() - 1);
    for (int i = 0; i < M; ++i) {
        int lo[3] = {0, 0, 0}, hi[3] = {0, 0, 0};
        for (int k = 0; k < naxes; ++k) cell_bucket_range(p, k, c[k][i], s[k][i], lo[k], hi[k]);
        for (int z = lo[2]; z <= hi[2]; ++z)
            for (int y = lo[1]; y <= hi[1]; ++y)
                for (int x = lo[0]; x <= hi[0]; ++x) g.cells[(size_t)fill[((size_t)z * p.dim[1] + y) * p.dim[0] + x]++] = i;
    }
    g.hints.assign((size_t)nb, 0);
    for (long long b = 0; b < nb; ++b) {
        const int bi[3] = {(int)(b % p.dim[0]), (int)((b / p.dim[0]) % p.dim[1]), (int)(b / ((long long)p.dim[0] * p.dim[1]))};
        const int e0 = g.start[(size_t)b];
        g.hints[(size_t)b] = bucket_hints(p, bi, g.cells.data() + e0, g.start[(size_t)b + 1] - e0, c, s);
    }
    if (getenv("MCRAT_HIP_VERBOSE")) {
        const int nocts = 1 << naxes;
        long long hinted = 0;
        for (long long b = 0; b < nb; ++b)
            for (int o = 0; o < nocts; ++o) hinted += ((g.hints[(size_t)b] >> (4 * o)) & 15u) != GRID_NO_HINT;
        fprintf(stderr, "mcrat_hip: %.1f %% of the bucket octants have a single-cell hint\n", 100.0 * hinted / ((double)nb * nocts));
    }
    return true;
}

inline void cell_velocity_staged(int dimensions, int geometry, double v0, double v1, double v2, double x1, double x2, double out[3])
{
    if (dimensions != DIM_THREE) {
        if (geometry == GEOM_SPHERICAL) {
            out[0] = v0 * sin(x1) + v1 * cos(x1);
            out[1] = v0 * cos(x1) - v1 * sin(x1);
        } else {
            out[0] = v0;
            out[1] = v1;
        }
        out[2] = v2;
    } else if (geometry == GEOM_CARTESIAN) {
        out[0] = v0; out[1] = v1; out[2] = v2;
    } else if (geometry == GEOM_SPHERICAL) {
        out[0] = v0 * sin(x1) * cos(x2) + v1 * cos(x1) * cos(x2) - v2 * sin(x2);
        out[1] = v0 * sin(x1) * sin(x2) + v1 * cos(x1) * sin(x2) + v2 * cos(x2);
        out[2] = v0 * cos(x1) - v1 * sin(x1);
    } else {
        out[0] = v0 * cos(x1) - v1 * sin(x1);
        out[1] = v0 * sin(x1) + v1 * cos(x1);
        out[2] = v2;
    }
}
inline FatCell fat_cell(const CellGeom &geom, const CellFluid &fluid, double c2, double s2, int ci)
{
    FatCell f{};
    f.c0 = geom.c0; f.c1 = geom.c1; f.s0 = geom.s0; f.s1 = geom.s1;
    f.a = fluid.a; f.b = fluid.b; f.c = fluid.c; f.w = fluid.w;
    f.nsig = fluid.nsig; f.gam = fluid.gam;
    f.c2 = c2; f.s2 = s2;
    f.cell = ci; f.pad = 0; f.pad2[0] = f.pad2[1] = f.pad2[2] = 0.0;
    return f;
}

inline size_t layout_take(size_t &off, size_t bytes) { const size_t o = off; off = (off + bytes + 255) / 256 * 256; return o; }
struct CellLayout {
    size_t geom, geom2, fluid, temp, fluid_c, k2e, gamma, total;
    bool has_geom2, has_fluid_c, has_k2e;
};
inline CellLayout cell_layout(int dimensions, int M, bool reserve_k2e)
{
    CellLayout l{};
    l.has_geom2 = dimensions == DIM_THREE; l.has_fluid_c = dimensions != DIM_TWO; l.has_k2e = reserve_k2e;
    size_t off = 0;
    l.geom = layout_take(off, sizeof(CellGeom) * M);
    l.geom2 = l.has_geom2 ? layout_take(off, sizeof(CellGeom2) * M) : 0;
    l.fluid = layout_take(off, sizeof(CellFluid) * M);
    l.temp = layout_take(off, sizeof(double) * M);
    l.fluid_c = l.has_fluid_c ? layout_take(off, sizeof(double) * M) : 0;
    l.k2e = l.has_k2e ? layout_take(off, sizeof(double) * M) : 0;
    l.gamma = layout_take(off, sizeof(double) * M);
    l.total = off;
    return l;
}
struct GridLayout {
    size_t dir, cells, start, scan, entries, total;
};
inline GridLayout grid_layout(long long nb, long long entries, size_t scan_scratch_ints)
{
    GridLayout l{};
    size_t off = 0;
    l.dir = layout_take(off, sizeof(BucketDir) * (size_t)nb);
    l.cells = layout_take(off, sizeof(FatCell) * std::max<size_t>((size_t)entries, 1));
    l.start = layout_take(off, sizeof(int) * ((size_t)nb + 1));
    l.scan = layout_take(off, sizeof(int) * scan_scratch_ints);
    l.entries = layout_take(off, sizeof(int) * std::max<size_t>((size_t)entries, 1));
    l.total = off;
    return l;
}

inline SlabDev slab_for(int dimensions, int geometry, const mcrat_hip_slab *s, int elem_factor)
{
    SlabDev d{};
    d.dimensions = dimensions; d.geometry = geometry; d.ph_inj_switch = s->ph_inj_switch;
    d.r_inj_095 = 0.95 * s->r_inj;
    if (s->ph_inj_switch == 0) {
        d.r_lo = s->min_r - elem_factor * C_LIGHT / s->fps;
        d.r_hi = s->max_r + elem_factor * C_LIGHT / s->fps;
        d.th_lo = s->min_theta - 2 * 0.017453292519943295;
        d.th_hi = s->max_theta + 2 * 0.017453292519943295;
    }
    return d;
}
inline bool slab_ok(const mcrat_hip_slab *s) { return s && s->fps > 0 && (s->ph_inj_switch == 0 || s->ph_inj_switch == 1); }
inline bool outflow_ok(const mcrat_hip_outflow *o) { return !o || (o->simulation_type >= MCRAT_HIP_SCIENCE && o->simulation_type <= MCRAT_HIP_STRUCTURED_SPHERICAL_OUTFLOW); }

struct ChomboPlan {
    std::vector<ChomboBox> boxes;
    std::vector<int> level_first_box;
    std::vector<double> xs[3], dxs[3];
    long long total = 0, cells = 0;
    int kv[5] = {-1, -1, -1, -1, -1};
};
inline const char *chombo_plan(const mcrat_hip_chombo *h, int dimensions, ChomboPlan &p)
{
    const bool three = dimensions == DIM_THREE;
    const int nd = three ? 3 : 2, bi = 2 * nd, nl = h->num_levels, nv = h->num_vars;
    p = ChomboPlan{};
    p.level_first_box.assign(nl + 1, 0);
    std::vector<ChomboBox> &boxes = p.boxes;
    long long total = 0;
    for (int i = 0; i < nl; ++i) {
        const mcrat_hip_chombo_level &L = h->levels[i];
        if (L.n_boxes < 0 || (L.n_boxes > 0 && (!L.boxes || !L.box_offsets)) || L.data_len < 0 || L.ref_ratio <= 0) return "";
        int ext[3] = {1, 1, 1}, cb[3] = {0, 0, 0};
        for (int a = 0; a < nd; ++a) {
            ext[a] = L.prob_domain[nd + a] - L.prob_domain[a] + 1;
            if (ext[a] <= 0) return "";
            cb[a] = (int)p.xs[a].size();
        }
        for (int j = 0; j < ext[0]; ++j) {
            const int g = L.prob_domain[0] + j;
            if (L.logr == 0) { p.xs[0].push_back(L.dombeg1 + L.dx * (g + 0.5)); p.dxs[0].push_back(L.dx); }
            else {
                p.xs[0].push_back(L.dombeg1 * 0.5 * (exp(L.dx * (g + 1)) + exp(L.dx * g)));
                p.dxs[0].push_back(L.dombeg1 * (exp(L.dx * (g + 1)) - exp(L.dx * g)));
            }
        }
        for (int j = 0; j < ext[1]; ++j) { p.xs[1].push_back(L.dombeg2 + L.dx * L.g_x2stretch * (L.prob_domain[1] + j + 0.5)); p.dxs[1].push_back(L.dx * L.g_x2stretch); }
        for (int j = 0; three && j < ext[2]; ++j) { p.xs[2].push_back(L.dombeg3 + L.dx * L.g_x3stretch * (L.prob_domain[2] + j + 0.5)); p.dxs[2].push_back(L.dx * L.g_x3stretch); }
        p.level_first_box[i] = (int)boxes.size();
        for (int j = 0; j < L.n_boxes; ++j) {
            const int *b = L.boxes + (size_t)j * bi;
            ChomboBox r{};
            r.level = i;
            long long ncell = 1;
            for (int a = 0; a < 3; ++a) {
                r.lo[a] = a < nd ? b[a] : 0;
                r.n[a] = a < nd ? b[nd + a] - b[a] + 1 : 1;
                r.cb[a] = cb[a];
                if (r.n[a] <= 0 || (a < nd && (r.lo[a] < 0 || r.lo[a] + r.n[a] > ext[a]))) return "PLUTO-Chombo ingest: a box lies outside its level's prob_domain";
                ncell *= r.n[a];
            }
            r.data_off = total + L.box_offsets[j];
            r.first_cell = r.data_off / nv;
            if (L.box_offsets[j] < 0 || L.box_offsets[j] + ncell * nv > L.data_len) return "PLUTO-Chombo ingest: a box's data lies outside its level's data";
            if (!boxes.empty() && r.first_cell != boxes.back().first_cell + (long long)boxes.back().n[0] * boxes.back().n[1] * boxes.back().n[2])
                return "PLUTO-Chombo ingest: box data do not follow one another in data:offsets order";
            boxes.push_back(r);
        }
        total += L.data_len;
    }
    p.level_first_box[nl] = (int)boxes.size();
    p.total = total;
    p.cells = total / nv;
    if (boxes.empty() || p.cells <= 0 || p.cells > 0x7fffffffLL || boxes.front().first_cell != 0) return "";
    static const char *want[5] = {"rho", "vx1", "vx2", "vx3", "prs"};
    for (int k = 0; k < nv; ++k)
        for (int w = 0; w < 5; ++w)
            if (h->var_names[k] && strcmp(h->var_names[k], want[w]) == 0) p.kv[w] = k;
    if (p.kv[0] < 0 || p.kv[1] < 0 || p.kv[2] < 0 || p.kv[4] < 0 || (dimensions != DIM_TWO && p.kv[3] < 0))
        return "PLUTO-Chombo ingest: a component (rho, vx1, vx2, [vx3], prs) is missing";
    return nullptr;
}

}
```

mcrat_amd/csrc/kernels.hip:

```cpp
#include <hip/hip_runtime.h>
#include <limits.h>
#include <math.h>
#include <stdio.h>
#include <type_traits>
#include "device_types.hpp"
#include "launch.hpp"
#include "sc_exchange.hpp"
#include "physics.hpp"
#include "photon_cols.hpp"
#include "rng.hpp"
#include "cs_device.hpp"

#if !defined(MCRAT_TAU_TABLE_TU) || !defined(MCRAT_TU_DIMS)
#error "compile kernels.hip through kernels_d*.hip / kernels_table_d*.hip"
#endif
#define MCRAT_NS_CAT2(a, b) a##b
#define MCRAT_NS_CAT(a, b) MCRAT_NS_CAT2(a, b)
#if MCRAT_TAU_TABLE_TU
#define MCRAT_TU_NS MCRAT_NS_CAT(tau_table_d, MCRAT_TU_DIMS)
#else
#define MCRAT_TU_NS MCRAT_NS_CAT(tau_direct_d, MCRAT_TU_DIMS)
#endif

namespace mcrat {
// ... 91 lines not shown
    i = __builtin_amdgcn_readlane(i, 63);
}

template <int CTRL, int ROWS>
__device__ __forceinline__ int dpp_add_step(int v) { return v + __builtin_amdgcn_update_dpp(0, v, CTRL, ROWS, 0xf, false); }

__device__ __forceinline__ int wave_sum_lane63_dpp(int v)
{
    v = dpp_add_step<0x111, 0xf>(v);
    v = dpp_add_step<0x112, 0xf>(v);
    v = dpp_add_step<0x114, 0xf>(v);
    v = dpp_add_step<0x118, 0xf>(v);
    v = dpp_add_step<0x142, 0xa>(v);
    v = dpp_add_step<0x143, 0xc>(v);
    return v;
}

template <int NW>
__device__ __forceinline__ void block_topk(TopK &mine, Cand (*s_w)[TOPK], Cand *out)
{
    static_assert(NW * TOPK <= 64, "second stage is one wave");
    const int lane = threadIdx.x & 63, w = threadIdx.x >> 6;
#pragma unroll
    for (int r = 0; r < TOPK; ++r) {
        double ht = mine.t[0];
        int hi = mine.i[0];
        wave_min_pair(ht, hi);
        if (mine.i[0] == hi && mine.t[0] == ht) mine.pop();
        if (lane == 0) { s_w[w][r].t = ht; s_w[w][r].idx = hi; }
    }
    __syncthreads();
    if (w == 0) {
        TopK m2;
        m2.init();
        if (lane < NW * TOPK) m2.insert(s_w[lane / TOPK][lane % TOPK].t, s_w[lane / TOPK][lane % TOPK].idx);
#pragma unroll
        for (int r = 0; r < TOPK; ++r) {
            double ht = m2.t[0];
            int hi = m2.i[0];
            wave_min_pair(ht, hi);
            if (m2.i[0] == hi && m2.t[0] == ht) m2.pop();
            if (lane == 0) { out[r].t = ht; out[r].idx = hi; out[r].pad = 0; }
        }
    }
    __syncthreads();
}

__device__ __forceinline__ double div_by_c(double x)
{
    constexpr double INV_C = 1.0 / C_LIGHT;
    const double q = x * INV_C;
    const double r = fma(-q, C_LIGHT, x);
    return fma(r, INV_C, q);
}

__device__ __forceinline__ double sample_free_time(double ntau , uint64_t bits)
{
    const double rnd = bits_to_uniform_pos(bits);
    const double mfp = ntau * log(rnd);
    return div_by_c(mfp);
}

__device__ __forceinline__ int xcd_contiguous_chunk(int b, int G)
{
    const int x = b & 7, q = G >> 3, rem = G & 7;
    return x * q + (x < rem ? x : rem) + (b >> 3);
}

struct MinCand {
    double t;
    int i;
    __device__ __forceinline__ void init() { t = INFINITY; i = INT_MAX; }
    __device__ __forceinline__ void offer(double tt, int ii)
    {
        if (tt != tt) tt = INFINITY;
        if (cand_less(tt, ii, t, i)) { t = tt; i = ii; }
    }
};

__device__ __forceinline__ void shortlist_push(Shortlist *sl, double t, int i)
{
    const int pos = atomicAdd(&sl->count, 1);
    if (pos < SHORTLIST_CAP) { sl->items[pos].t = t; sl->items[pos].idx = i; sl->items[pos].pad = 0; }
}

constexpr int Q_RECALC_ONLY = (int)0x80000000;
constexpr int Q_DEFERRED = 0x40000000;

template <int DIMS, int GEOM, bool FORCE, class PH>
__device__ __forceinline__ double fast_one(const PH &ph, const HydroDev &hy, int i, unsigned fl, int cell,
                                           double r0, double r1, double r2, double ntau, uint64_t bits, int &queue, int &bucket,
                                           double &a0, double &a1, double &a2)
{
    queue = 0;
    bucket = -1;
    a0 = a1 = a2 = 0;
    if (!(fl & FLAG_VALID)) return INFINITY;
    if (MC_DIAG(DIAG_SKIP_COORDS)) { a0 = r0 + r1; a1 = r2; a2 = 0; }
    else phys::hydro_coords<DIMS, GEOM>(r0, r1, r2, a0, a1, a2);
    if (phys::in_domain<DIMS>(hy, a0, a1, a2) && (cell != -1)) {
        if constexpr (FORCE) {
            queue = 1;
        } else {
            if (MC_DIAG(DIAG_SKIP_INCELL)) queue = 0;
            else if (!phys::check_in_block<DIMS>(hy, cell, a0, a1, a2)) queue = 1;
            else if (fl & FLAG_RECALC) {
                if (fl & FLAG_TAU_FRESH) {
                    ph.flags(i) = (unsigned char)(fl & ~(FLAG_RECALC | FLAG_TAU_FRESH));
                    ph.tau(i) = ph.tau_next(i);
                } else {
                    queue = 2;
                }
            }
        }
        if (queue == 1) bucket = phys::grid_bucket_of<DIMS>(hy.grid, a0, a1, a2);
        if (queue) return INFINITY;
        if (MC_DIAG(DIAG_SKIP_SAMPLE)) return 1e-3 + (double)i * 1e-12 + (double)(bits & 1) * 0.0 + ntau * 0.0;
        return sample_free_time(ntau, bits);
    }
    if (cell != -1) ph.idx(i) = -1;
    return 1e12 / C_LIGHT;
}

__device__ __forceinline__ double free_time_from_log(double ntau, double log_u) { return div_by_c(ntau * log_u); }

struct TableSite {
    uint64_t seed, pass;
    uint32_t stream, slot_base;
    int first;
    int mode;
    bool deferred;
    double norm, eps, theta;
    __device__ __forceinline__ TableSite(const RngKey &key, unsigned long long iter, int first_ = 0, int mode_ = 0)
        : seed(key.seed), pass(iter), stream(key.stream), slot_base(key.slot_base), first(first_), mode(mode_), deferred(false), norm(1), eps(0), theta(0) {}
};

template <int DIMS, int GEOM, bool LOGS = false, class PH>
__device__ __forceinline__ double slow_one(const PH &ph, const HydroDev &hy, int i, bool relocate, int bucket, bool count_it,
                                           uint64_t bits, int &relocated, int &not_found, TableSite &ts)
{
    const double r0 = ph.r0(i), r1 = ph.r1(i), r2 = ph.r2(i);
    const double p0 = ph.p0(i), p1 = ph.p1(i), p2 = ph.p2(i), p3 = ph.p3(i);
    const unsigned fl = ph.flags(i);
    int cell;
    bool need_tau = (fl & FLAG_RECALC) != 0;
    bool new_cell = false;
    double fa = 0, fb = 0, fc = 0, fw = 0, fnsig = 0, fgam = 1, fkf = 0.5;
    double a0 = 0, a1 = 0, a2 = 0;
    if (MC_DIAG(DIAG_SLOW_EMPTY)) { ph.tts(i) = 1e-3 + i * 1e-12; return 1e-3 + i * 1e-12; }
    if (MC_DIAG(DIAG_SLOW_NO_SEARCH)) relocate = false;
    if (relocate) {
        phys::hydro_coords<DIMS, GEOM>(r0, r1, r2, a0, a1, a2);
        FatCell hit;
        cell = phys::find_in_bucket<DIMS>(hy.grid, bucket, a0, a1, a2, hit);
        ph.idx(i) = cell;
        if (cell != -1) {
            fa = hit.a; fb = hit.b; fc = hit.c; fw = hit.w; fnsig = hit.nsig; fgam = hit.gam; fkf = phys::kf_of_gamma(hit.gam);
            new_cell = true;
            need_tau = true;
            if (count_it) relocated += 1;
        } else {
            not_found += 1;
        }
    } else {
        cell = ph.idx(i);
        if (cell != -1) {
            const CellFluid f = hy.fluid[cell];
            fa = f.a; fb = f.b; fc = f.c; fw = f.w; fnsig = f.nsig;
        }
    }
    double t;
    if (MC_DIAG(DIAG_SLOW_NO_PHYSICS)) need_tau = false;
    if (cell != -1) {
        double ntau;
        if (need_tau) {
            double cphi, sphi;
            if (new_cell) phys::relocation_azimuth<DIMS, GEOM>(r0, r1, a0, cphi, sphi);
            else phys::cos_sin_of_atan2(r1, r0, cphi, sphi);
            double beta[3];
            phys::beta_from_record<DIMS>(fa, fb, fc, cphi, sphi, beta);
            double comv0 = 0;
            if (new_cell) {
                const double lab[4] = {p0, p1, p2, p3};
                double comv[4];
                phys::boost_with<true>(beta, fgam, fkf, lab, comv);
                ph.c0(i) = comv[0]; ph.c1(i) = comv[1]; ph.c2(i) = comv[2]; ph.c3(i) = comv[3];
                comv0 = comv[0];
            }
            double norm = 1.0;
            if constexpr (TABLE_MODE) {
                if (!new_cell) comv0 = ph.c0(i);
                if (ts.mode == 2) {
                    norm = ts.norm;
                } else if (phys::thermal_cross_section_lookup(hy, comv0, hy.temp[cell], norm, ts.eps, ts.theta)) {
                    if (ts.mode == 1) {
                        ts.deferred = true;
                        if (new_cell && count_it) relocated -= 1;
                        return 0.0;
                    }
                    norm = phys::table_fallback_lane(ts.eps, ts.theta, ts.seed, ts.pass, ts.slot_base + (uint32_t)(i - ts.first), ts.stream, hy.hot_fallback_calls);
                    atomicAdd(hy.table_fallbacks, 1);
                }
            }
            const double tau = phys::optical_depth_staged(beta, fw, fnsig, p1, p2, p3, norm);
            ntau = -phys::rcp_nr(tau);
            ph.tau(i) = tau;
            ph.ntau(i) = ntau;
            if (fl & FLAG_RECALC) ph.flags(i) = (unsigned char)(fl & ~(FLAG_RECALC | FLAG_TAU_FRESH));
        } else {
            ntau = ph.ntau(i);
        }
        t = LOGS ? free_time_from_log(ntau, __longlong_as_double((long long)bits)) : sample_free_time(ntau, bits);
    } else {
        t = 1e12 / C_LIGHT;
    }
    ph.tts(i) = t;
    return t;
}

struct LockstepProbe {
    const int *cached;
    bool force;
    bool *same;
};

template <int DIMS, int GEOM, int K, bool LOGS = false, class PH>
__device__ __forceinline__ void relocate_lockstep(const PH &ph, const HydroDev &hy, const int (&slot)[K], bool (&todo)[K],
                                                  const double (&r0)[K], const double (&r1)[K], const double (&a0)[K], const double (&a1)[K],
                                                  const double (&a2)[K], const int (&code)[K], const uint64_t (&bits)[K], const unsigned (&fl)[K],
                                                  bool count_it, double (&t)[K], int &relocated, const LockstepProbe *probe = nullptr)
{
    static_assert(!TABLE_MODE, "DIRECT optical depths");
    const GridDev &g = hy.grid;
    BucketDir d[K];
    double p0[K], p1[K], p2[K], p3[K];
    bool take[K];
#pragma unroll
    for (int k = 0; k < K; ++k) {
        take[k] = todo[k] && code[k] >= 0;
        d[k] = g.dir[take[k] ? (code[k] & GRID_CODE_BUCKET_MASK) : 0];
        const int i = slot[k];
        p0[k] = ph.p0(i); p1[k] = ph.p1(i); p2[k] = ph.p2(i); p3[k] = ph.p3(i);
    }
    FatCell f[K];
#pragma unroll
    for (int k = 0; k < K; ++k) {
        const unsigned hint = (d[k].hints >> (4 * ((code[k] >> GRID_CODE_OCT_SHIFT) & 7))) & 15u;
        take[k] = take[k] & (d[k].n > 0) & ((code[k] & GRID_CODE_HINT_OK) != 0) & (hint != GRID_NO_HINT);
        f[k] = g.cells[take[k] ? d[k].e0 + (int)hint : 0];
    }
    double comv[K][4], tau[K], ntau[K];
#pragma unroll
    for (int k = 0; k < K; ++k) {
        take[k] = take[k] & phys::well_in_fat_cell<DIMS>(f[k], a0[k], a1[k], a2[k]);
        double cphi, sphi;
        phys::relocation_azimuth<DIMS, GEOM>(r0[k], r1[k], a0[k], cphi, sphi);
        double beta[3];
        phys::beta_from_record<DIMS>(f[k].a, f[k].b, f[k].c, cphi, sphi, beta);
        const double lab[4] = {p0[k], p1[k], p2[k], p3[k]};
        phys::boost_with<true>(beta, f[k].gam, phys::kf_of_gamma(f[k].gam), lab, comv[k]);
        tau[k] = phys::optical_depth_staged(beta, f[k].w, f[k].nsig, p1[k], p2[k], p3[k], 1.0);
        ntau[k] = -phys::rcp_nr(tau[k]);
        t[k] = LOGS ? free_time_from_log(ntau[k], __longlong_as_double((long long)bits[k])) : sample_free_time(ntau[k], bits[k]);
    }
#pragma unroll
    for (int k = 0; k < K; ++k)
        asm volatile("" : "+v"(comv[k][0]), "+v"(comv[k][1]), "+v"(comv[k][2]), "+v"(comv[k][3]), "+v"(tau[k]), "+v"(ntau[k]), "+v"(t[k]));
#pragma unroll
    for (int k = 0; k < K; ++k) {
        if (!take[k]) continue;
        if (probe) {
            probe->same[k] = !probe->force && f[k].cell == probe->cached[k];
            if (probe->same[k]) { todo[k] = false; continue; }
        }
        const int i = slot[k];
        ph.idx(i) = f[k].cell;
        ph.c0(i) = comv[k][0]; ph.c1(i) = comv[k][1]; ph.c2(i) = comv[k][2]; ph.c3(i) = comv[k][3];
        ph.tau(i) = tau[k];
        ph.ntau(i) = ntau[k];
        if (fl[k] & FLAG_RECALC) ph.flags(i) = (unsigned char)(fl[k] & ~(FLAG_RECALC | FLAG_TAU_FRESH));
        ph.tts(i) = t[k];
        if (count_it) relocated += 1;
        todo[k] = false;
    }
}

struct PairIn {
    double2 R0, R1, R2, U0, U1, U2, NTAU;
    int2 ID;
    uchar2 FL;
};

__device__ __forceinline__ PairIn load_pair(const PhotonDev &ph, int i0, bool need_u)
{
    PairIn in;
    in.R0 = *reinterpret_cast<const double2 *>(ph.r0 + i0);
    in.R1 = *reinterpret_cast<const double2 *>(ph.r1 + i0);
    in.R2 = *reinterpret_cast<const double2 *>(ph.r2 + i0);
    in.NTAU = *reinterpret_cast<const double2 *>(ph.ntau + i0);
    in.ID = *reinterpret_cast<const int2 *>(ph.idx + i0);
    in.FL = *reinterpret_cast<const uchar2 *>(ph.flags + i0);
    if (need_u) {
        in.U0 = *reinterpret_cast<const double2 *>(ph.u0 + i0);
        in.U1 = *reinterpret_cast<const double2 *>(ph.u1 + i0);
        in.U2 = *reinterpret_cast<const double2 *>(ph.u2 + i0);
    } else {
        in.U0 = in.U1 = in.U2 = make_double2(0, 0);
    }
    return in;
}

template <int DIMS, int GEOM, bool FORCE>
#ifndef STEP_WAVES_PER_SIMD
#define STEP_WAVES_PER_SIMD 3
#endif
__global__ __launch_bounds__(STEP_BLOCK, STEP_WAVES_PER_SIMD) void step_kernel(PhotonDev ph, HydroDev hy, LoopState *st, RngKey key,
                                                          Cand *__restrict__ block_min, Shortlist *sl)
{
    __shared__ int s_qn;
    __shared__ int s_q[STEP_QCAP];
    __shared__ int s_qb[STEP_QCAP];
    __shared__ double s_wt[STEP_BLOCK / 64];
    __shared__ int s_wi[STEP_BLOCK / 64];
    if (st->done) return;
    const PtrCols pc(ph);
    const int nseg = st->nseg;
    const int skip = st->skip_idx;
    const unsigned long long iter = st->iteration;
    const double t_cut = st->t_cut;
    const int G = gridDim.x;
    const int lane = threadIdx.x & 63;

    MinCand best;
    best.init();
    int relocated = 0, not_found = 0;
    TableSite ts(key, iter);
    const int nchunks = ph.n_pad / (2 * STEP_BLOCK);
    if (threadIdx.x == 0) s_qn = 0;
    for (int e = threadIdx.x; e < STEP_QCAP; e += STEP_BLOCK) s_q[e] = -1;
    __syncthreads();

    auto process = [&](PairIn &in, int pair) {
        const int i0 = pair << 1;
        if (nseg > 0 && !MC_DIAG(DIAG_SKIP_ADVANCE)) {
            const bool m0 = (in.FL.x & FLAG_MOVES) && (i0 != skip);
            const bool m1 = (in.FL.y & FLAG_MOVES) && (i0 + 1 != skip);
            for (int s = 0; s < nseg; ++s) {
                const double t = st->seg[s];
                if (m0) { in.R0.x += in.U0.x * t; in.R1.x += in.U1.x * t; in.R2.x += in.U2.x * t; }
                if (m1) { in.R0.y += in.U0.y * t; in.R1.y += in.U1.y * t; in.R2.y += in.U2.y * t; }
            }
            *reinterpret_cast<double2 *>(ph.r0 + i0) = in.R0;
            *reinterpret_cast<double2 *>(ph.r1 + i0) = in.R1;
            *reinterpret_cast<double2 *>(ph.r2 + i0) = in.R2;
        }
        Philox4 blk;
        if (MC_DIAG(DIAG_SKIP_PHILOX)) { blk.w[0] = pair * 2654435761u; blk.w[1] = pair ^ 0x9e3779b9u; blk.w[2] = ~blk.w[0]; blk.w[3] = blk.w[1] + 7u; }
        else blk = keyed_block(key.seed, iter, (uint32_t)pair + (key.slot_base >> 1), RNG_FREEPATH, key.stream);
        const uint64_t bits0 = (uint64_t)blk.w[0] | ((uint64_t)blk.w[1] << 32);
        const uint64_t bits1 = (uint64_t)blk.w[2] | ((uint64_t)blk.w[3] << 32);

        int q0, q1, b0, b1;
        double2 T;
        double A0[2], A1[2], A2[2];
        T.x = fast_one<DIMS, GEOM, FORCE>(pc, hy, i0, in.FL.x, in.ID.x, in.R0.x, in.R1.x, in.R2.x, in.NTAU.x, bits0, q0, b0, A0[0], A1[0], A2[0]);
        T.y = fast_one<DIMS, GEOM, FORCE>(pc, hy, i0 + 1, in.FL.y, in.ID.y, in.R0.y, in.R1.y, in.R2.y, in.NTAU.y, bits1, q1, b1, A0[1], A1[1], A2[1]);
        if constexpr (FORCE) {
            if constexpr (!TABLE_MODE) {
                const int slot[2] = {i0, i0 + 1}, code[2] = {b0, b1};
                bool todo[2] = {q0 != 0, q1 != 0};
                const double R0[2] = {in.R0.x, in.R0.y}, R1[2] = {in.R1.x, in.R1.y};
                const uint64_t bits[2] = {bits0, bits1};
                const unsigned fl[2] = {in.FL.x, in.FL.y};
                double tt[2];
                int dummy = 0;
                if (todo[0] || todo[1]) {
                    relocate_lockstep<DIMS, GEOM, 2>(pc, hy, slot, todo, R0, R1, A0, A1, A2, code, bits, fl, false, tt, dummy);
                    if (q0 && !todo[0]) { T.x = tt[0]; q0 = 0; }
                    if (q1 && !todo[1]) { T.y = tt[1]; q1 = 0; }
                }
            }
            if (q0) T.x = slow_one<DIMS, GEOM>(pc, hy, i0, true, b0, false, bits0, relocated, not_found, ts);
            if (q1) T.y = slow_one<DIMS, GEOM>(pc, hy, i0 + 1, true, b1, false, bits1, relocated, not_found, ts);
            q0 = q1 = 0;
        } else {
            const unsigned long long m0 = __ballot(q0 != 0), m1 = __ballot(q1 != 0);
            if (m0 | m1) {
                const int c0 = __popcll(m0), c1 = __popcll(m1);
                int base = 0;
                if (lane == 0) base = atomicAdd(&s_qn, c0 + c1);
                base = __builtin_amdgcn_readfirstlane(base);
                if (base + c0 + c1 <= STEP_QCAP) {
                    const unsigned long long below = (lane == 0) ? 0ull : (~0ull >> (64 - lane));
                    if (q0) { const int e = base + __popcll(m0 & below); s_q[e] = i0 | (q0 == 2 ? Q_RECALC_ONLY : 0); s_qb[e] = b0; }
                    if (q1) { const int e = base + c0 + __popcll(m1 & below); s_q[e] = (i0 + 1) | (q1 == 2 ? Q_RECALC_ONLY : 0); s_qb[e] = b1; }
                } else {
                    if (q0) { T.x = slow_one<DIMS, GEOM>(pc, hy, i0, q0 == 1, b0, true, bits0, relocated, not_found, ts); q0 = 0; }
                    if (q1) { T.y = slow_one<DIMS, GEOM>(pc, hy, i0 + 1, q1 == 1, b1, true, bits1, relocated, not_found, ts); q1 = 0; }
                }
            }
        }
        if (q0) T.x = __longlong_as_double((long long)bits0);
        if (q1) T.y = __longlong_as_double((long long)bits1);
        *reinterpret_cast<double2 *>(ph.tts + i0) = T;
        if ((in.FL.x & FLAG_VALID) && !q0) { best.offer(T.x, i0); if (T.x < t_cut) shortlist_push(sl, T.x, i0); }
        if ((in.FL.y & FLAG_VALID) && !q1) { best.offer(T.y, i0 + 1); if (T.y < t_cut) shortlist_push(sl, T.y, i0 + 1); }
    };

    for (int chunk = xcd_contiguous_chunk(blockIdx.x, G); chunk < nchunks; chunk += G) {
        const int pa = chunk * STEP_BLOCK + threadIdx.x;
        PairIn A = load_pair(ph, pa << 1, nseg > 0);
        process(A, pa);
    }

    if constexpr (!FORCE) {
        __syncthreads();
        int qn = s_qn;
        if (qn > STEP_QCAP) qn = STEP_QCAP;
        if (MC_DIAG(DIAG_SKIP_SLOW)) qn = 0;
        for (int e = threadIdx.x; e < qn; e += STEP_BLOCK) {
            const int entry = s_q[e];
            if (entry == -1) continue;
            const int i = entry & ~Q_RECALC_ONLY;
            const uint64_t bits = (uint64_t)__double_as_longlong(ph.tts[i]);
            const double t = slow_one<DIMS, GEOM>(pc, hy, i, !(entry & Q_RECALC_ONLY), s_qb[e], true, bits, relocated, not_found, ts);
            best.offer(t, i);
            if (t < t_cut) shortlist_push(sl, t, i);
        }
    }

    wave_min_pair_dpp(best.t, best.i);
    if (lane == 0) { s_wt[threadIdx.x >> 6] = best.t; s_wi[threadIdx.x >> 6] = best.i; }
    __syncthreads();
    if (threadIdx.x == 0) {
        MinCand m;
        m.init();
#pragma unroll
// ... 1797 lines not shown
```

mcrat_amd/csrc/launch.hpp:

```cpp
#pragma once
#include <hip/hip_runtime.h>
#include "device_types.hpp"
#include "frame_queue.hpp"
#include "list_plan.hpp"
#include "hydro_plan.hpp"
#include "rank_form_plan.hpp"

namespace mcrat {

struct KernelConfig {
    int dimensions;
    int geometry;
    int stokes;
    int table;
};

struct ReducePartial {
    double r_min, r_max, th_min, th_max;
    double sum_scatt, sum_r, e_sum, w_sum;
    double max_scatt, min_scatt;
    long long count;
};

int step_grid_blocks(int n_pad);
// ... 106 lines not shown
hipError_t launch_inject_count(const InjectParams &p, const HydroDev &hy, double ph_weight_adjusted, unsigned long long attempt, RngKey key,
                               unsigned *count, unsigned long long *d_total, hipStream_t stream);
hipError_t launch_inject_generate(const InjectParams &p, const HydroDev &hy, double ph_weight_adjusted, RngKey key, const int *start,
                                  const PhotonDev &ph, hipStream_t stream);
struct alignas(8) InjectSlabCell { int cell; int pad; double v43, g; };
constexpr int POOL_INJECT_CAP = 8192;
struct alignas(8) PoolInject {
    int inject, group;
    unsigned long long seed;
    unsigned stream; int pad;
    double weight_in;
    int min_photons, max_photons;
    double weight_out;
    int n, error;
};
hipError_t launch_inject_slab_flag(const InjectParams &p, const HydroDev &hy, unsigned *flag, unsigned long long *d_total, int *n_slab, hipStream_t stream);
hipError_t launch_inject_slab_write(const InjectParams &p, const HydroDev &hy, const unsigned *flag, int n_slab, int *start, int *scratch, InjectSlabCell *out,
                                    hipStream_t stream);
hipError_t launch_inject_pool(const InjectParams &p, const HydroDev &hy, const PhotonDev &pool, int stride, int n_ranks, const InjectSlabCell *slab, int n_slab,
                              PoolInject *lists, int group, hipStream_t stream);
struct HydroCols {
    double *r0, *r1, *r2, *s0, *s1, *s2;
    double *v0, *v1, *v2;
    double *dens, *dens_lab, *pres, *temp, *gamma;
    double *r, *theta;
    double *B0, *B1, *B2;
};
struct FlashDev {
    const double *coord, *bsize;
    const int *node;
    const double *velx, *vely, *dens, *pres;
    int coord_stride, bsize_stride;
    long long n_blocks;
    double L, D, P;
};
struct PlutoDev {
    int nx, ny, nz;
    const double *x1, *dx1, *x2, *dx2, *x3, *dx3;
    const double *rho, *vx1, *vx2, *vx3, *prs;
    double L, D, P;
};
struct ChomboDev {
    const ChomboBox *boxes;
    int n_boxes;
    long long cells;
    const double *data;
    const double *x[3], *dx[3];
    const unsigned char *covered;
    int kv[5];
    double L, D, P;
};
hipError_t ingest_count_chombo(const ChomboDev &h, const SlabDev &slab, unsigned *block_count, unsigned long long *d_total, hipStream_t stream);
hipError_t ingest_write_chombo(const ChomboDev &h, const SlabDev &slab, const int *block_start, const HydroCols &out, hipStream_t stream);
hipError_t launch_chombo_mask(const ChomboBox *boxes, int c0, int c1, int f0, int f1, int ref_ratio, int three, unsigned char *covered, hipStream_t stream);
struct CsParams {
    int dimensions, b_field_calc;
    double epsilon_b;
};
struct CsAbsPartial { double abs_weight; int abs_count, scatt_count; };
int cs_absorb_blocks(int n);
hipError_t launch_cs_absorb(const CsParams &p, const PhotonDev &ph, const double *temp, const HydroCols &h, CsAbsPartial *partials, hipStream_t stream);
struct OutflowDev {
    int simulation_type;
    double gamma_infinity, lumi, r00, t_comov, ddensity, theta_j, p;
};
long long ingest_blocks(long long n_virtual);
hipError_t ingest_count_flash(const FlashDev &f, const SlabDev &slab, unsigned *block_count, unsigned long long *d_total, hipStream_t stream);
hipError_t ingest_write_flash(const FlashDev &f, const SlabDev &slab, const int *block_start, const HydroCols &out, hipStream_t stream);
hipError_t ingest_count_pluto(const PlutoDev &g, const SlabDev &slab, unsigned *block_count, unsigned long long *d_total, hipStream_t stream);
hipError_t ingest_write_pluto(const PlutoDev &g, const SlabDev &slab, const int *block_start, const HydroCols &out, hipStream_t stream);
hipError_t launch_fill_spherical(int dims, int geom, const HydroCols &h, int M, hipStream_t stream);
hipError_t launch_outflow_prep(int dims, int geom, const OutflowDev &o, const HydroCols &h, int M, hipStream_t stream);
int stage_cells_blocks(int M);
hipError_t launch_stage_cells(int dims, int geom, const HydroCols &h, int M, CellGeom *og, CellGeom2 *og2, CellFluid *of, double *ofc, double *otemp,
                              double *ogamma, StagePartial *partials, double *samples, int stride, int nsamp, hipStream_t stream);
constexpr int HOT_TABLE_SUBSTREAMS = 256;
struct HotTableParams {
    int n_ph_e, n_t;
    double log_ph_e_min, log_ph_e_max, log_t_min, log_t_max;
    long long calls;
    unsigned long long seed;
};
hipError_t launch_hot_table(const HotTableParams &p, double *table, hipStream_t stream);
struct CsEmitParams {
    int dimensions, geometry, b_field_calc;
    double epsilon_b;
    double rmin, rmax, theta_min, theta_max;
};
struct CsHookArgs { CsEmitParams p; HydroCols h; };
hipError_t launch_cs_emit_count(const CsEmitParams &p, const HydroDev &hy, const HydroCols &h, double ph_weight_adjusted, unsigned long long attempt,
                                RngKey key, unsigned *count, unsigned long long *d_total, unsigned *d_flags, hipStream_t stream);
hipError_t launch_cs_emit_generate(const CsEmitParams &p, const HydroDev &hy, const HydroCols &h, double ph_weight_adjusted, RngKey key, const int *start,
                                   int n_emit, const int *null_slots, const PhotonDev &ph, hipStream_t stream);
constexpr int LOOP_CS_HALT = 3;
constexpr int CS_HALT_GROW = 1;
constexpr int CS_HALT_REBIN = 2;
constexpr int CS_HALT_HOOK = 3;
struct CsFrame {
    int halt;
    int saved_done;
    int emitted;
    int scatt_num;
    int max_photons;
    int pad;
    unsigned long long last_iteration;
    double n_comptonized;
};
hipError_t launch_cs_replace(const CsEmitParams &p, const HydroDev &hy, const HydroCols &h, RngKey key, LoopState *st, const PhotonDev &ph,
                             CsFrame *frame, int resume, hipStream_t stream);
struct alignas(8) CsShellCell { int cell; int pad; double integral; double volume; };
struct alignas(8) CsPoolEmit {
    int open, group;
    unsigned long long seed;
    double weight_in, max_photons;
    double weight_out;
    int n_emit, error;
};
hipError_t launch_cs_shell_flag(const CsEmitParams &p, const HydroDev &hy, unsigned *flag, unsigned long long *d_total, int *n_shell, hipStream_t stream);
hipError_t launch_cs_shell_write(const CsEmitParams &p, const HydroDev &hy, const HydroCols &h, const unsigned *flag, int n_shell, int *start, int *scratch,
                                 CsShellCell *out, unsigned *not_converged, hipStream_t stream);
hipError_t launch_cs_emit_pool(const CsEmitParams &p, const HydroDev &hy, const HydroCols &h, const PhotonDev &pool, int stride, int n_ranks, RankDesc *desc,
                               const CsShellCell *shell, int n_shell, CsPoolEmit *lists, int group, hipStream_t stream);
hipError_t launch_cs_absorb_pool(const CsParams &p, const PhotonDev &pool, int stride, int n_ranks, const RankDesc *desc, const int *open, const double *temp,
                                 const HydroCols &h, CsAbsPartial *per_list, hipStream_t stream);
hipError_t launch_cs_replace_pool(const CsEmitParams &p, const HydroDev &hy, const HydroCols &h, LoopState *states, const PhotonDev &pool, int stride,
                                  int n_ranks, RankDesc *desc, CsFrame *frames, hipStream_t stream);
hipError_t launch_null_count(const PhotonDev &ph, unsigned *block_count, unsigned long long *d_total, hipStream_t stream);
hipError_t launch_null_write(const PhotonDev &ph, const int *block_start, int *null_slots, hipStream_t stream);
hipError_t launch_null_fill(const PhotonDev &ph, int first, int count, hipStream_t stream);
int rebin_range_blocks(int n);
hipError_t launch_rebin_range(const PhotonDev &ph, int three, RebinRange *partials, hipStream_t stream);
hipError_t launch_rebin_assign(const PhotonDev &ph, const RebinAxes &ax, int *bin_of, unsigned *bin_count, hipStream_t stream);
hipError_t launch_rebin_fill(const PhotonDev &ph, const int *bin_of, const int *bin_start, unsigned *cursor, int *members, hipStream_t stream);
struct RebinRec {
    double weight, p0, p1, p2, p3, r0, r1, r2, s0, s1, s2, s3, num_scatt;
    int valid, pad;
};
hipError_t launch_rebin_create(const PhotonDev &ph, const RebinAxes &ax, const int *bin_start, int *members, RebinRec *recs,
                               unsigned *empty_bins, hipStream_t stream);
hipError_t launch_rebin_place(const PhotonDev &ph, const RebinRec *recs, int total_bins, const int *null_slots, hipStream_t stream);
hipError_t launch_rebin_nullify(const PhotonDev &ph, hipStream_t stream);
struct RebinPoolList {
    int first, n;
    RebinAxes ax;
    unsigned long long scratch;
    int status;
    int empty_bins, n_null;
    int pad;
};
size_t rebin_pool_scratch_bytes(int n, int total_bins);
hipError_t launch_rebin_pool_range(const PhotonDev &pool, int three, const RebinPoolList *lists, int n_lists, RebinRange *out, hipStream_t stream);
hipError_t launch_rebin_pool(const PhotonDev &pool, RebinPoolList *lists, int n_lists, char *scratch, hipStream_t stream);
hipError_t grid_build(const GridPlan &p, const CellGeom *geom, const CellGeom2 *geom2, const CellFluid *fluid, const double *fluid_c, int M,
                      unsigned *count, int *start, int *scan_scratch, int *entries, FatCell *cells, BucketDir *dir, long long nb,
                      long long total, hipStream_t stream);
hipError_t launch_lookup(const KernelConfig &kc, const HydroDev &hy, int n, const double *a0, const double *a1,
                         const double *a2, int *out, hipStream_t stream);
struct TuLaunchers {
    decltype(&launch_step) step;
    decltype(&launch_event) event;
    decltype(&launch_tape_pass) tape_pass;
    decltype(&launch_rank_loop) rank_loop;
    decltype(&launch_rank_loop_tape) rank_loop_tape;
    decltype(&launch_sc_propose) sc_propose;
    decltype(&launch_sc_resolve) sc_resolve;
    decltype(&launch_fast_frame) fast_frame;
};
hipError_t launch_eval_function(const KernelConfig &kc, const HydroDev &hy, int fn, int n, const double *in, double *out, uint64_t seed, uint32_t stream_id,
                                hipStream_t stream);

}
```

mcrat_amd/csrc/physics.hpp:

```cpp
#pragma once
#include <hip/hip_runtime.h>
#include "device_types.hpp"
#include "rng.hpp"

namespace mcrat {
namespace phys {

constexpr int REJECTION_CAP = 1 << 22;

#if defined(MCRAT_IEEE_ARITH) && MCRAT_IEEE_ARITH
__device__ __forceinline__ double rcp_nr(double x) { return 1.0 / x; }
__device__ __forceinline__ double rsqrt_nr(double x) { return 1.0 / sqrt(x); }
__device__ __forceinline__ double sqrt_nr(double x) { return sqrt(x); }
#else
__device__ __forceinline__ double rcp_nr(double x)
{
    const double r0 = __builtin_amdgcn_rcp(x);
    double e = fma(-x, r0, 1.0);
    double r = fma(r0, e, r0);
    e = fma(-x, r, 1.0);
    r = fma(r, e, r);
    return (fabs(r0) < INFINITY && r0 != 0.0) ? r : r0;
}
__device__ __forceinline__ double rsqrt_nr(double x)
{
    const double y0 = __builtin_amdgcn_rsq(x);
    const double h = 0.5 * x;
    double e = fma(-(h * y0), y0, 0.5);
    double y = fma(y0, e, y0);
    e = fma(-(h * y), y, 0.5);
    y = fma(y, e, y);
    return (y0 < INFINITY && y0 > 0.0) ? y : y0;
}
__device__ __forceinline__ double sqrt_nr(double x)
{
    const double y = x * rsqrt_nr(x);
    return (x == 0.0) ? 0.0 : y;
}
#endif


template <int DIMS, int GEOM>
__device__ __forceinline__ void hydro_coords(double x, double y, double z, double &a0, double &a1, double &a2)
{
    a0 = -1; a1 = -1; a2 = -1;
    if constexpr (DIMS == DIM_TWO || DIMS == DIM_TWO_POINT_FIVE) {
        if constexpr (GEOM == GEOM_CARTESIAN || GEOM == GEOM_CYLINDRICAL) {
            a0 = sqrt(x * x + y * y);
            a1 = z;
        } else if constexpr (GEOM == GEOM_SPHERICAL) {
            a0 = sqrt(x * x + y * y + z * z);
            a1 = acos(z / a0);
        }
    } else {
        if constexpr (GEOM == GEOM_CARTESIAN) {
            a0 = x; a1 = y; a2 = z;
        } else if constexpr (GEOM == GEOM_SPHERICAL) {
            a0 = sqrt(x * x + y * y + z * z);
            a1 = acos(z / a0);
            a2 = fmod(atan2(y, x) * 180.0 / M_PI + 360.0, 360.0) * M_PI / 180;
        } else if constexpr (GEOM == GEOM_POLAR) {
            a0 = sqrt(x * x + y * y);
            a1 = fmod(atan2(y, x) * 180.0 / M_PI + 360.0, 360.0) * M_PI / 180;
            a2 = z;
        }
    }
}

template <int DIMS>
__device__ __forceinline__ bool in_domain(const HydroDev &h, double a0, double a1, double a2)
{
    bool in = (a1 < h.dom1[1]) & (a1 > h.dom1[0]) & (a0 < h.dom0[1]) & (a0 > h.dom0[0]);
    if constexpr (DIMS == DIM_THREE) in = (a2 < h.dom2[1]) & (a2 > h.dom2[0]) & in;
    return in;
}

template <int DIMS>
__device__ __forceinline__ bool check_in_block(const HydroDev &h, int cell, double a0, double a1, double a2)
{
    const CellGeom g = h.geom[cell];
    bool in = (2 * fabs(a0 - g.c0) - g.s0 <= 0) & (2 * fabs(a1 - g.c1) - g.s1 <= 0);
    if constexpr (DIMS == DIM_THREE) {
        const CellGeom2 g2 = h.geom2[cell];
        in = in & (2 * fabs(a2 - g2.c2) - g2.s2 <= 0);
    }
    return in;
}

template <int NAXES>
__device__ __forceinline__ int grid_bucket_axes(const GridDev &g, double a0, double a1, double a2)
{
    const double a[3] = {a0, a1, a2};
    int b[3] = {0, 0, 0};
    int oct = 0;
    bool ok = true, nan = false;
#pragma unroll
    for (int k = 0; k < NAXES; ++k) {
        double u = a[k];
        if (g.logmap[k]) u = log(a[k]);
        const double x = (u - g.org[k]) * g.inv[k];
        const double f = floor(x);
        const double fr = x - f;
        const double hi = (double)(g.dim[k] - 1);
        nan = nan | !(f == f);
        ok = ok & (f >= 0.0) & (f <= hi) & (fr > 1e-6) & (fabs(fr - 0.5) > 1e-6) & (1.0 - fr > 1e-6);
        oct |= (fr >= 0.5 ? 1 : 0) << k;
        b[k] = (int)fmin(fmax(f, 0.0), hi);
    }
    const int code = ((b[2] * g.dim[1] + b[1]) * g.dim[0] + b[0]) | (oct << GRID_CODE_OCT_SHIFT) | (ok ? GRID_CODE_HINT_OK : 0);
    return nan ? -1 : code;
}
__device__ __forceinline__ int grid_bucket(const GridDev &g, double a0, double a1, double a2)
{
    return g.naxes == 3 ? grid_bucket_axes<3>(g, a0, a1, a2) : grid_bucket_axes<2>(g, a0, a1, a2);
}
template <int DIMS>
__device__ __forceinline__ int grid_bucket_of(const GridDev &g, double a0, double a1, double a2)
{
    return grid_bucket_axes<DIMS == DIM_THREE ? 3 : 2>(g, a0, a1, a2);
}

template <int DIMS>
__device__ __forceinline__ bool in_fat_cell(const FatCell &f, double a0, double a1, double a2)
{
    bool in = (2 * fabs(a0 - f.c0) - f.s0 <= 0) && (2 * fabs(a1 - f.c1) - f.s1 <= 0);
    if constexpr (DIMS == DIM_THREE) in = in && (2 * fabs(a2 - f.c2) - f.s2 <= 0);
    return in;
}

template <int DIMS>
__device__ __forceinline__ bool well_in_fat_cell(const FatCell &f, double a0, double a1, double a2)
{
    bool in = (2 * fabs(a0 - f.c0) - f.s0 < -1e-8 * f.s0) & (2 * fabs(a1 - f.c1) - f.s1 < -1e-8 * f.s1);
    if constexpr (DIMS == DIM_THREE) in = in & (2 * fabs(a2 - f.c2) - f.s2 < -1e-8 * f.s2);
    return in;
}

template <int DIMS>
__device__ __forceinline__ int walk_bucket(const GridDev &g, int e0, int n, double a0, double a1, double a2, FatCell &hit)
{
    constexpr int BATCH = 4;
    int found = -1;
    for (int b0 = 0; b0 < n && found < 0; b0 += BATCH) {
        bool in[BATCH];
#pragma unroll
        for (int k = 0; k < BATCH; ++k) {
            const FatCell *p = g.cells + e0 + ((b0 + k < n) ? b0 + k : b0);
            const double c0 = p->c0, c1 = p->c1, s0 = p->s0, s1 = p->s1;
            in[k] = (b0 + k < n) && (2 * fabs(a0 - c0) - s0 <= 0) && (2 * fabs(a1 - c1) - s1 <= 0);
            if constexpr (DIMS == DIM_THREE) {
                const double c2 = p->c2, s2 = p->s2;
                in[k] = in[k] && (2 * fabs(a2 - c2) - s2 <= 0);
            }
        }
#pragma unroll
        for (int k = BATCH - 1; k >= 0; --k)
            if (in[k]) found = b0 + k;
    }
    if (found < 0) return -1;
    hit = g.cells[e0 + found];
    return hit.cell;
}

template <int DIMS>
__device__ __forceinline__ int find_in_bucket(const GridDev &g, int code, double a0, double a1, double a2, FatCell &hit)
{
    hit.cell = -1;
    if (code < 0) return -1;
    const BucketDir d = g.dir[code & GRID_CODE_BUCKET_MASK];
    if (d.n <= 0) return -1;
    const unsigned hint = (d.hints >> (4 * ((code >> GRID_CODE_OCT_SHIFT) & 7))) & 15u;
    if ((code & GRID_CODE_HINT_OK) && hint != GRID_NO_HINT) {
        const FatCell f = g.cells[d.e0 + (int)hint];
        if (well_in_fat_cell<DIMS>(f, a0, a1, a2)) { hit = f; return f.cell; }
    }
    return walk_bucket<DIMS>(g, d.e0, d.n, a0, a1, a2, hit);
}

template <int DIMS>
__device__ __forceinline__ int find_containing_block(const HydroDev &h, double a0, double a1, double a2)
{
    FatCell hit;
    return find_in_bucket<DIMS>(h.grid, grid_bucket_of<DIMS>(h.grid, a0, a1, a2), a0, a1, a2, hit);
}

template <int DIMS>
__device__ __forceinline__ void beta_from_record(double a, double b, double c, double cphi, double sphi, double out[3])
{
    if constexpr (DIMS == DIM_TWO) {
        out[0] = a * cphi; out[1] = a * sphi; out[2] = b;
    } else if constexpr (DIMS == DIM_TWO_POINT_FIVE) {
        out[0] = a * cphi - c * sphi; out[1] = a * sphi + c * cphi; out[2] = b;
    } else {
        out[0] = a; out[1] = b; out[2] = c;
    }
}

__device__ __forceinline__ void cos_sin_of_atan2(double y, double x, double &c, double &s)
{
    const double h2 = x * x + y * y;
    const double ih = rsqrt_nr(h2);
    const bool pos = h2 > 0;
    c = pos ? x * ih : ((x < 0 || (x == 0 && signbit(x))) ? -1.0 : 1.0);
    s = pos ? y * ih : 0.0;
}
__device__ __forceinline__ void cos_sin_with_hypot(double y, double x, double h, double &c, double &s)
{
    const double ih = rcp_nr(h);
    const bool pos = h > 0;
    c = pos ? x * ih : ((x < 0 || (x == 0 && signbit(x))) ? -1.0 : 1.0);
    s = pos ? y * ih : 0.0;
}

template <int DIMS, int GEOM>
__device__ __forceinline__ void relocation_azimuth(double x, double y, double a0, double &c, double &s)
{
    if constexpr (DIMS != DIM_THREE && GEOM != GEOM_SPHERICAL) cos_sin_with_hypot(y, x, a0, c, s);
    else cos_sin_of_atan2(y, x, c, s);
}

template <int DIMS>
__device__ __forceinline__ void cell_beta(const CellFluid &f, double cphi, double sphi, double out[3])
{
    beta_from_record<DIMS>(f.a, f.b, f.c, cphi, sphi, out);
}

__device__ __forceinline__ void zero_norm(double p[4])
{
    const double nrm = sqrt(p[1] * p[1] + p[2] * p[2] + p[3] * p[3]);
    const double q1 = (p[1] / nrm) * p[0], q2 = (p[2] / nrm) * p[0], q3 = (p[3] / nrm) * p[0];
    const bool fix = p[0] != nrm;
    p[1] = fix ? q1 : p[1];
    p[2] = fix ? q2 : p[2];
    p[3] = fix ? q3 : p[3];
}

__device__ __forceinline__ void lorentz_boost(const double b[3], const double p[4], double out[4], bool photon)
{
    const double beta = sqrt(b[0] * b[0] + b[1] * b[1] + b[2] * b[2]);
    double r[4];
    {
        const double gamma = 1.0 / sqrt(1 - beta * beta);
        const double b2 = beta * beta, g1 = gamma - 1;
        const double L01 = -1 * b[0] * gamma, L02 = -1 * b[1] * gamma, L03 = -1 * b[2] * gamma;
        const double L11 = 1 + ((g1 * (b[0] * b[0])) / b2);
        const double L12 = g1 * (b[0] * b[1] / b2);
        const double L13 = g1 * (b[0] * b[2] / b2);
        const double L22 = 1 + ((g1 * (b[1] * b[1])) / b2);
        const double L23 = (g1 * (b[1] * b[2])) / b2;
        const double L33 = 1 + ((g1 * (b[2] * b[2])) / b2);
        const double m0 = ((p[0] * gamma + p[1] * L01) + p[2] * L02) + p[3] * L03;
        const double m1 = ((p[0] * L01 + p[1] * L11) + p[2] * L12) + p[3] * L13;
        const double m2 = ((p[0] * L02 + p[1] * L12) + p[2] * L22) + p[3] * L23;
        const double m3 = ((p[0] * L03 + p[1] * L13) + p[2] * L23) + p[3] * L33;
        const bool moving = beta > 0;
        r[0] = moving ? m0 : p[0]; r[1] = moving ? m1 : p[1]; r[2] = moving ? m2 : p[2]; r[3] = moving ? m3 : p[3];
    }
    if (photon) zero_norm(r);
    out[0] = r[0]; out[1] = r[1]; out[2] = r[2]; out[3] = r[3];
}

__device__ __forceinline__ void zero_norm_lean(double p[4])
{
    const double s = p[0] * rsqrt_nr((p[1] * p[1] + p[2] * p[2]) + p[3] * p[3]);
    p[1] *= s; p[2] *= s; p[3] *= s;
}
template <bool PHOTON>
__device__ __forceinline__ void boost_with(const double b[3], double g, double kf, const double p[4], double out[4])
{
    const double bp = (b[0] * p[1] + b[1] * p[2]) + b[2] * p[3];
    const double f = kf * bp - g * p[0];
    out[0] = g * (p[0] - bp);
    out[1] = p[1] + f * b[0];
    out[2] = p[2] + f * b[1];
    out[3] = p[3] + f * b[2];
    if constexpr (PHOTON) zero_norm_lean(out);
}

__device__ __forceinline__ double kf_of_gamma(double gam) { return (gam * gam) * rcp_nr(gam + 1.0); }

__device__ __forceinline__ double optical_depth_staged(const double fluid_beta[3], double w, double nsig, double p1, double p2, double p3,
                                                       double norm_cross_section = 1.0)
{
    const double bp = (fluid_beta[0] * p1 + fluid_beta[1] * p2) + fluid_beta[2] * p3;
    const double ipn = rsqrt_nr((p1 * p1 + p2 * p2) + p3 * p3);
    return (nsig * norm_cross_section) * (1.0 - w * (bp * ipn));
}


__device__ __forceinline__ int table_cell(double x0, double dx, int n_cells, double x)
{
    int i = (int)floor((x - x0) / dx);
    i = i < 0 ? 0 : (i > n_cells - 1 ? n_cells - 1 : i);
    while (i > 0 && x0 + i * dx > x) --i;
    while (i < n_cells - 1 && !(x0 + (i + 1) * dx > x)) ++i;
    return i;
}

__device__ __forceinline__ double kn_cross_section_ieee(double e)
{
    if (e >= 1e-3)
        return (3. / 4.) * (2. / (e * e) + (1. / (2. * e) - (1. + e) / (e * e * e)) * log(1. + 2. * e) + (1. + e) / ((1. + 2. * e) * (1. + 2. * e)));
    return (1. - 2. * e);
}

__device__ __forceinline__ bool thermal_cross_section_lookup(const HydroDev &h, double photon_comv_e, double fluid_temp, double &norm, double &eps, double &theta_out)
{
    norm = 1.0;
    if (!h.hot_table) return false;
    const double normalized_photon_comv_e = photon_comv_e / (M_EL * C_LIGHT);
    const double theta = K_B * fluid_temp / (M_EL * C_LIGHT * C_LIGHT);
    const double x = log10(normalized_photon_comv_e), y = log10(theta);
    const double x_hi = h.hot_e0 + h.hot_n_ph_e * h.hot_de, y_hi = h.hot_t0 + h.hot_n_t * h.hot_dt;
    const bool out = !(x >= h.hot_e0) | (x > x_hi) | !(y >= h.hot_t0) | (y > y_hi);
    if (out) {
        const double theta_min = pow(10.0, h.hot_t0), e_min = pow(10.0, h.hot_e0);
        if (theta < theta_min) { norm = (normalized_photon_comv_e < e_min) ? 1.0 : kn_cross_section_ieee(normalized_photon_comv_e); return false; }
        eps = pow(10.0, x);
        theta_out = pow(10.0, y);
        return true;
    }
    const int xi = table_cell(h.hot_e0, h.hot_de, h.hot_n_ph_e, x);
    const int yi = table_cell(h.hot_t0, h.hot_dt, h.hot_n_t, y);
    const double xmin = h.hot_e0 + xi * h.hot_de, xmax = h.hot_e0 + (xi + 1) * h.hot_de;
    const double ymin = h.hot_t0 + yi * h.hot_dt, ymax = h.hot_t0 + (yi + 1) * h.hot_dt;
    const int ny = h.hot_n_t + 1;
    const double zminmin = h.hot_table[xi * ny + yi], zminmax = h.hot_table[xi * ny + yi + 1];
    const double zmaxmin = h.hot_table[(xi + 1) * ny + yi], zmaxmax = h.hot_table[(xi + 1) * ny + yi + 1];
    const double t = (x - xmin) / (xmax - xmin), u = (y - ymin) / (ymax - ymin);
    const double z = (1. - t) * (1. - u) * zminmin + t * (1. - u) * zmaxmin + (1. - t) * u * zminmax + t * u * zmaxmax;
    norm = pow(10.0, z);
    return false;
}

__device__ __forceinline__ void find_xy(const double v[3], const double ref[3], double x[3], double y[3])
{
// ... 398 lines not shown
```

mcrat_amd/csrc/sightline.hip:

```cpp
#include <hip/hip_runtime.h>
#include "device_types.hpp"
#include "launch.hpp"
#include "observe_plan.hpp"
#include "physics.hpp"
#include "sightline_plan.hpp"

namespace mcrat {

namespace {

template <bool FROM_COLUMNS>
__device__ __forceinline__ void ray_origin(const PhotonDev &ph, const SightlineDev &a, int i, double &x, double &y, double &z)
{
    if constexpr (FROM_COLUMNS) {
        x = ph.r0[i]; y = ph.r1[i]; z = ph.r2[i];
    } else {
        const size_t n = (size_t)a.n;
        x = a.ray[i]; y = a.ray[n + i]; z = a.ray[2 * n + i];
    }
}
template <bool FROM_COLUMNS>
__device__ __forceinline__ void ray_momentum(const PhotonDev &ph, const SightlineDev &a, int i, double p[4])
{
    if constexpr (FROM_COLUMNS) {
        p[0] = ph.p0[i]; p[1] = ph.p1[i]; p[2] = ph.p2[i]; p[3] = ph.p3[i];
    } else {
        const size_t n = (size_t)a.n;
        p[0] = a.ray[3 * n + i]; p[1] = a.ray[4 * n + i]; p[2] = a.ray[5 * n + i]; p[3] = a.ray[6 * n + i];
    }
}

__device__ __forceinline__ void write_surface(const SightlineDev &a, int i, int step, double x, double y, double z)
{
    const size_t n = (size_t)a.n;
    a.i4[SL_SURFACE_STEP * n + i] = step;
    a.f8[SL_SURFACE_R0 * n + i] = x; a.f8[SL_SURFACE_R1 * n + i] = y; a.f8[SL_SURFACE_R2 * n + i] = z;
}
__device__ __forceinline__ void write_march(const SightlineDev &a, int i, double tau, double path, int steps, int status)
{
    const size_t n = (size_t)a.n;
    a.f8[SL_TAU * n + i] = tau; a.f8[SL_PATH * n + i] = path;
    a.i4[SL_STEPS * n + i] = steps; a.i4[SL_STATUS * n + i] = status;
}

template <int DIMS, int GEOM, bool TABLE, bool FROM_COLUMNS>
__global__ __launch_bounds__(SIGHTLINE_BLOCK) void sightline_kernel(PhotonDev ph, HydroDev hy, SightlineDev a)
{
    __shared__ unsigned s_count[SIGHTLINE_N_STATUS];
    __shared__ unsigned s_next;
    const int tid = threadIdx.x, lane = tid & 63;
    const unsigned own_lo = blockIdx.x * (unsigned)a.own_rays, own_hi = own_lo + (unsigned)a.own_rays;
    const unsigned shared_lo = gridDim.x * (unsigned)a.own_rays, n = (unsigned)a.n;
    if (tid < SIGHTLINE_N_STATUS) s_count[tid] = 0u;
    if (tid == 0) s_next = own_lo;
    __syncthreads();

    const double nan = __builtin_nan("");
    int ray = -1, phase = 0, k = 0, k_total = 0;
    double x = 0, y = 0, z = 0, nx = 0, ny = 0, nz = 0, tau = 0, path = 0, tau_total = 0;
    double p[4] = {0, 0, 0, 0};
    bool dry = false, own_dry = a.own_rays == 0;

    for (;;) {
        if (!dry) {
            const unsigned long long idle = __ballot(ray < 0);
            if (idle) {
                int got = -1;
                if (!a.refill) {
                    const unsigned i = blockIdx.x * (unsigned)SIGHTLINE_BLOCK + (unsigned)tid;
                    if (i < n) got = (int)i;
                    dry = true;
                } else {
                    const unsigned long long below = (1ull << lane) - 1ull;
                    if (!own_dry) {
                        const int leader = __ffsll((long long)idle) - 1;
                        const unsigned want = (unsigned)__popcll(idle);
                        unsigned base = 0;
                        if (lane == leader) base = atomicAdd(&s_next, want);
                        base = __shfl(base, leader, 64);
                        const unsigned i = base + (unsigned)__popcll(idle & below);
                        if (ray < 0 && i < own_hi) got = (int)i;
                        own_dry = base + want >= own_hi;
                    }
                    const unsigned long long unserved = __ballot(ray < 0 && got < 0);
                    if (unserved) {
                        const int leader = __ffsll((long long)unserved) - 1;
                        const unsigned long long want = (unsigned long long)__popcll(unserved);
                        unsigned long long base = 0;
                        if (lane == leader) base = atomicAdd(&a.head[SIGHTLINE_COUNTER_WORD], want);
                        base = __shfl(base, leader, 64);
                        const unsigned long long i = (unsigned long long)shared_lo + base + (unsigned long long)__popcll(unserved & below);
                        if (ray < 0 && got < 0 && i < (unsigned long long)n) got = (int)i;
                        dry = (unsigned long long)shared_lo + base + want >= (unsigned long long)n;
                    }
                }
                if (got >= 0) {
                    bool march = true;
                    if constexpr (FROM_COLUMNS) march = observe_observable(ph.flags[got], ph.type[got], ph.weight[got]);
                    if (march) {
                        ray = got; phase = 1; k = 0; tau = 0; path = 0;
                        ray_origin<FROM_COLUMNS>(ph, a, got, x, y, z);
                        ray_momentum<FROM_COLUMNS>(ph, a, got, p);
                        sightline_direction(p[1], p[2], p[3], nx, ny, nz);
                    } else {
                        write_march(a, got, 0.0, 0.0, 0, SIGHTLINE_SKIPPED);
                        write_surface(a, got, -1, nan, nan, nan);
                        atomicAdd(&s_count[SIGHTLINE_SKIPPED], 1u);
                    }
                }
            }
        }
        if (dry && !__ballot(ray >= 0)) break;
        if (ray >= 0) {
            int status = -1;
            bool surface_done = false;
            if (phase == 1) {
                if (k == a.max_steps) status = SIGHTLINE_STEP_CAP;
            } else if (sightline_surface_reached(tau_total, tau, a.surface_level)) {
                write_surface(a, ray, k, x, y, z);
                surface_done = true;
            } else if (k == k_total) {
                write_surface(a, ray, -1, nan, nan, nan);
                surface_done = true;
            }
            if (status < 0 && !surface_done) {
                const double h = sightline_step_length(x, y, z, a.step_frac, a.h_min);
                double mx, my, mz, a0, a1, a2;
                sightline_midpoint(x, y, z, h, nx, ny, nz, mx, my, mz);
                phys::hydro_coords<DIMS, GEOM>(mx, my, mz, a0, a1, a2);
                FatCell hit;
                hit.cell = -1;
                if (phys::in_domain<DIMS>(hy, a0, a1, a2))
                    phys::find_in_bucket<DIMS>(hy.grid, phys::grid_bucket_of<DIMS>(hy.grid, a0, a1, a2), a0, a1, a2, hit);
                if (hit.cell < 0) {
                    status = SIGHTLINE_LEFT_MESH;
                } else {
                    double cphi, sphi, beta[3], norm = 1.0;
                    phys::relocation_azimuth<DIMS, GEOM>(mx, my, a0, cphi, sphi);
                    phys::beta_from_record<DIMS>(hit.a, hit.b, hit.c, cphi, sphi, beta);
                    bool off_table = false;
                    if constexpr (TABLE) {
                        double comv[4], eps, theta;
                        phys::boost_with<false>(beta, hit.gam, phys::kf_of_gamma(hit.gam), p, comv);
                        off_table = phys::thermal_cross_section_lookup(hy, comv[0], hy.temp[hit.cell], norm, eps, theta);
                    }
                    if (off_table) {
                        status = SIGHTLINE_OFF_TABLE;
                    } else {
                        const double kappa = phys::optical_depth_staged(beta, hit.w, hit.nsig, p[1], p[2], p[3], norm);
                        tau += kappa * h;
                        path += h;
                        sightline_advance(x, y, z, h, nx, ny, nz);
                        k += 1;
                        if (phase == 1 && tau >= a.tau_stop) status = SIGHTLINE_OPAQUE;
                    }
                }
                if (phase == 2 && status >= 0) {
                    write_surface(a, ray, -1, nan, nan, nan);
                    surface_done = true;
                }
            }
            if (phase == 1 && status >= 0) {
                write_march(a, ray, tau, path, k, status);
                atomicAdd(&s_count[status], 1u);
                if (a.surface_level >= 0 && status == SIGHTLINE_LEFT_MESH) {
                    phase = 2; tau_total = tau; k_total = k;
                    k = 0; tau = 0; path = 0;
                    ray_origin<FROM_COLUMNS>(ph, a, ray, x, y, z);
                } else {
                    write_surface(a, ray, -1, nan, nan, nan);
                    ray = -1;
                }
            } else if (surface_done) {
                ray = -1;
            }
        }
    }
    __syncthreads();
    if (tid < SIGHTLINE_N_STATUS && s_count[tid]) atomicAdd(&a.head[tid], (unsigned long long)s_count[tid]);
}

template <int DIMS, int GEOM>
hipError_t launch_pair(bool table, const PhotonDev &ph, const HydroDev &hy, const SightlineDev &a, int blocks, hipStream_t stream)
{
    const dim3 grid(blocks), block(SIGHTLINE_BLOCK);
    const bool columns = a.ray == nullptr;
    if (table) {
        if (columns) hipLaunchKernelGGL((sightline_kernel<DIMS, GEOM, true, true>), grid, block, 0, stream, ph, hy, a);
        else hipLaunchKernelGGL((sightline_kernel<DIMS, GEOM, true, false>), grid, block, 0, stream, ph, hy, a);
    } else {
        if (columns) hipLaunchKernelGGL((sightline_kernel<DIMS, GEOM, false, true>), grid, block, 0, stream, ph, hy, a);
        else hipLaunchKernelGGL((sightline_kernel<DIMS, GEOM, false, false>), grid, block, 0, stream, ph, hy, a);
    }
    return hipGetLastError();
}

}

hipError_t launch_sightline(const KernelConfig &kc, const PhotonDev &ph, const HydroDev &hy, const SightlineDev &a, int blocks, hipStream_t stream)
{
    if (a.n <= 0 || blocks <= 0) return hipErrorInvalidValue;
    const bool table = kc.table != 0;
    switch (kc.dimensions * 4 + kc.geometry) {
    case DIM_TWO * 4 + GEOM_CARTESIAN: return launch_pair<DIM_TWO, GEOM_CARTESIAN>(table, ph, hy, a, blocks, stream);
    case DIM_TWO * 4 + GEOM_CYLINDRICAL: return launch_pair<DIM_TWO, GEOM_CYLINDRICAL>(table, ph, hy, a, blocks, stream);
    case DIM_TWO * 4 + GEOM_SPHERICAL: return launch_pair<DIM_TWO, GEOM_SPHERICAL>(table, ph, hy, a, blocks, stream);
    case DIM_TWO_POINT_FIVE * 4 + GEOM_CARTESIAN: return launch_pair<DIM_TWO_POINT_FIVE, GEOM_CARTESIAN>(table, ph, hy, a, blocks, stream);
    case DIM_TWO_POINT_FIVE * 4 + GEOM_CYLINDRICAL: return launch_pair<DIM_TWO_POINT_FIVE, GEOM_CYLINDRICAL>(table, ph, hy, a, blocks, stream);
    case DIM_TWO_POINT_FIVE * 4 + GEOM_SPHERICAL: return launch_pair<DIM_TWO_POINT_FIVE, GEOM_SPHERICAL>(table, ph, hy, a, blocks, stream);
    case DIM_THREE * 4 + GEOM_CARTESIAN: return launch_pair<DIM_THREE, GEOM_CARTESIAN>(table, ph, hy, a, blocks, stream);
    case DIM_THREE * 4 + GEOM_SPHERICAL: return launch_pair<DIM_THREE, GEOM_SPHERICAL>(table, ph, hy, a, blocks, stream);
    case DIM_THREE * 4 + GEOM_POLAR: return launch_pair<DIM_THREE, GEOM_POLAR>(table, ph, hy, a, blocks, stream);
    default: return hipErrorInvalidValue;
    }
}

}
```

mcrat_amd/engine.py:

```python
import ctypes as C
import os

import numpy as np

_HERE = os.path.dirname(os.path.abspath(__file__))
LIB_PATH = os.path.join(_HERE, "libmcrat_hip.so")

ABI_VERSION = 1
CARTESIAN, SPHERICAL, CYLINDRICAL, POLAR = 0, 1, 2, 3
TWO, TWO_POINT_FIVE, THREE = 0, 1, 2
TAU_DIRECT = 1
TAU_TABLE = 2

_dp = C.POINTER(C.c_double)
_ip = C.POINTER(C.c_int)

PHOTON_DTYPE = np.dtype(
    [("type", "S1"),
     ("p0", "f8"), ("p1", "f8"), ("p2", "f8"), ("p3", "f8"),
     ("comv_p0", "f8"), ("comv_p1", "f8"), ("comv_p2", "f8"), ("comv_p3", "f8"),
     ("r0", "f8"), ("r1", "f8"), ("r2", "f8"),
     ("s0", "f8"), ("s1", "f8"), ("s2", "f8"), ("s3", "f8"),
     ("num_scatt", "f8"),
     ("recalc_properties", "i4"),
# ... 122 lines not shown


class OutputColumns(C.Structure):
    _fields_ = [("count", C.c_int)] + [(f, _dp) for f in OUTPUT_COLUMNS] + [("type", C.c_char_p)]


class PoolInjectList(C.Structure):
    _fields_ = [("inject", C.c_int), ("spect", C.c_char), ("min_photons", C.c_int), ("max_photons", C.c_int),
                ("r_inj", C.c_double), ("ph_weight", C.c_double), ("theta_min", C.c_double), ("theta_max", C.c_double),
                ("seed", C.c_uint64), ("num_photons", C.c_int), ("ph_weight_adjusted", C.c_double), ("status", C.c_int)]


class RankSummary(C.Structure):
    _fields_ = [("min_r", C.c_double), ("max_r", C.c_double), ("min_theta", C.c_double), ("max_theta", C.c_double),
                ("avg_scatt", C.c_double), ("avg_r", C.c_double), ("avg_energy", C.c_double),
                ("max_scatt", C.c_int), ("min_scatt", C.c_int), ("num_output", C.c_int), ("list_capacity", C.c_int)]


class PoolCsList(C.Structure):
    _fields_ = [("open", C.c_int), ("emit_pool", C.c_int), ("scatt_frame_number", C.c_int), ("inj_frame_number", C.c_int), ("seed", C.c_uint64),
                ("time_now", C.c_double), ("remaining_time", C.c_double), ("r_inj", C.c_double), ("ph_weight_suggest", C.c_double),
                ("theta_min", C.c_double), ("theta_max", C.c_double)]


class Observer(C.Structure):
    _fields_ = [("n_obs", C.c_int), ("cos_obs", _dp), ("sin_obs", _dp), ("cos_lo", _dp), ("cos_hi", _dp),
                ("n_t", C.c_int), ("t_edges", _dp), ("n_e", C.c_int), ("e_edges", _dp)]


class Observation(C.Structure):
    _fields_ = [("count", C.POINTER(C.c_longlong)), ("w", _dp), ("we", _dp), ("i", _dp), ("q", _dp), ("u", _dp), ("v", _dp),
                ("n_accepted", C.POINTER(C.c_longlong)), ("n_outside", C.POINTER(C.c_longlong))]


OBSERVE_PATH_LDS, OBSERVE_PATH_GLOBAL = 1, 2


class SightlineParams(C.Structure):
    _fields_ = [("step_frac", C.c_double), ("h_min", C.c_double), ("max_steps", C.c_int), ("tau_stop", C.c_double), ("surface_level", C.c_double)]


class Sightlines(C.Structure):
    _fields_ = [("tau", _dp), ("path", _dp), ("steps", _ip), ("status", _ip), ("surface_step", _ip),
                ("surface_r0", _dp), ("surface_r1", _dp), ("surface_r2", _dp), ("n_status", C.c_longlong * 5)]


SIGHTLINE_SKIPPED, SIGHTLINE_LEFT_MESH, SIGHTLINE_OPAQUE, SIGHTLINE_STEP_CAP, SIGHTLINE_OFF_TABLE = 0, 1, 2, 3, 4

SCIENCE, CYLINDRICAL_OUTFLOW, SPHERICAL_OUTFLOW, STRUCTURED_SPHERICAL_OUTFLOW = 0, 1, 2, 3

_ctx = C.c_void_p
MODE_EXACT, MODE_FAST = 0, 1
SYMBOLS = {
    "mcrat_hip_init": (C.c_int, [C.POINTER(_ctx), C.POINTER(Config)]),
    "mcrat_hip_destroy": (None, [_ctx]),
    "mcrat_hip_version": (C.c_char_p, []),
    "mcrat_hip_strerror": (C.c_char_p, [C.c_int]),
    "mcrat_hip_last_error": (C.c_char_p, [_ctx]),
    "mcrat_hip_set_hydro": (C.c_int, [_ctx, C.POINTER(Hydro)]),
    "mcrat_hip_outflow_defaults": (None, [C.c_int, C.POINTER(Outflow)]),
    "mcrat_hip_ingest_flash": (C.c_int, [_ctx, C.POINTER(FlashBlocks), C.POINTER(Slab), C.POINTER(Outflow), C.POINTER(IngestResult)]),
    "mcrat_hip_ingest_pluto": (C.c_int, [_ctx, C.POINTER(PlutoGrid), C.POINTER(Slab), C.POINTER(Outflow), C.POINTER(IngestResult)]),
    "mcrat_hip_ingest_chombo": (C.c_int, [_ctx, C.POINTER(Chombo), C.POINTER(Slab), C.POINTER(Outflow), C.POINTER(IngestResult)]),
    "mcrat_hip_set_hydro_extras": (C.c_int, [_ctx, _dp, _dp, _dp, _dp]),
    "mcrat_hip_emit_cyclosynch_pool": (C.c_int, [_ctx, C.POINTER(Cyclosynch), C.c_double, C.c_double, C.c_int, C.c_double, C.c_double, C.c_double,
                                                 C.c_uint64, _ip, _dp, _ip]),
    "mcrat_hip_rebin_cyclosynch": (C.c_int, [_ctx, C.POINTER(Cyclosynch), C.c_int, _ip, _ip, _ip]),
    "mcrat_hip_scatter_frame_cyclosynch": (C.c_int, [_ctx, C.POINTER(Cyclosynch), _dp, C.c_double, C.c_uint64, C.c_double, C.c_double, C.c_int,
                                                     C.c_double, C.c_double, C.c_double, C.c_int, C.c_longlong, C.POINTER(FrameStats),
                                                     C.POINTER(CyclosynchCounts)]),
    "mcrat_hip_num_photon_slots": (C.c_int, [_ctx]),
    "mcrat_hip_absorb_cyclosynch": (C.c_int, [_ctx, C.POINTER(Cyclosynch), _ip, _ip, _dp]),
    "mcrat_hip_get_hydro": (C.c_int, [_ctx, C.POINTER(HydroColumns)]),
    "mcrat_hip_get_output": (C.c_int, [_ctx, C.POINTER(OutputColumns)]),
    "mcrat_hip_convert_comptonized": (C.c_int, [_ctx, _ip]),
    "mcrat_hip_get_photons_range": (C.c_int, [_ctx, C.c_int, C.c_int, C.c_void_p]),
    "mcrat_hip_inject_photons": (C.c_int, [_ctx, C.c_double, C.c_double, C.c_int, C.c_int, C.c_char, C.c_double, C.c_double, C.c_double,
                                           C.c_uint64, _ip, _dp]),
    "mcrat_hip_set_hot_cross_section": (C.c_int, [_ctx, _dp, C.c_int, C.c_int, C.c_double, C.c_double, C.c_double, C.c_double]),
    "mcrat_hip_table_fallback_calls": (C.c_int, [_ctx, C.c_int]),
    "mcrat_hip_pool_select_frame": (C.c_int, [_ctx, C.c_int]),
    "mcrat_hip_create_hot_cross_section": (C.c_int, [_ctx, _dp, C.c_int, C.c_int, C.c_double, C.c_double, C.c_double, C.c_double, C.c_longlong,
                                                     C.c_uint64]),
    "mcrat_hip_set_photons": (C.c_int, [_ctx, C.POINTER(PhotonList)]),
    "mcrat_hip_register_host": (C.c_int, [_ctx, C.c_void_p, C.c_size_t]),
    "mcrat_hip_unregister_host": (C.c_int, [_ctx, C.c_void_p]),
    "mcrat_hip_get_photons": (C.c_int, [_ctx, C.POINTER(PhotonList)]),
    "mcrat_hip_set_photons_soa": (C.c_int, [_ctx, C.POINTER(PhotonSoA)]),
    "mcrat_hip_get_photons_soa": (C.c_int, [_ctx, C.POINTER(PhotonSoA)]),
    "mcrat_hip_num_photon_slots": (C.c_int, [_ctx]),
    "mcrat_hip_pool_inject_photons": (C.c_int, [_ctx, C.c_double, C.POINTER(PoolInjectList)]),
    "mcrat_hip_pool_set_photons": (C.c_int, [_ctx, C.c_int, _ip, C.c_void_p]),
    "mcrat_hip_profile_totals": (C.c_int, [_ctx, C.POINTER(C.c_double), C.POINTER(C.c_longlong)]),
    "mcrat_hip_outbox_create": (C.c_int, [_ctx, C.POINTER(C.c_void_p)]),
    "mcrat_hip_outbox_destroy": (None, [C.c_void_p]),
    "mcrat_hip_outbox_post": (C.c_int, [_ctx, C.c_void_p, C.c_int, C.c_int]),
    "mcrat_hip_outbox_wait": (C.c_int, [C.c_void_p, C.POINTER(C.c_void_p), C.POINTER(C.c_int), C.c_void_p]),
    "mcrat_hip_bind_thread": (C.c_int, [_ctx]),
    "mcrat_hip_share_hydro": (C.c_int, [_ctx, _ctx]),
    "mcrat_hip_propagate_frame": (C.c_int, [_ctx, _dp, C.c_double, C.c_uint64, C.POINTER(FrameStats)]),
    "mcrat_hip_propagate_frame_mode": (C.c_int, [_ctx, _dp, C.c_double, C.c_uint64, C.c_int, C.c_int, C.POINTER(FrameStats)]),
    "mcrat_hip_fast_cadence": (C.c_int, [_ctx, C.c_int]),
    "mcrat_hip_pool_propagate_frames_fast": (C.c_int, [_ctx, C.POINTER(C.c_int), C.POINTER(C.c_uint64), _dp, _dp, C.c_int, C.POINTER(FrameStats)]),
    "mcrat_hip_begin_frame": (C.c_int, [_ctx, C.c_uint64, C.c_double, C.c_double]),
    "mcrat_hip_run": (C.c_int, [_ctx, C.c_longlong, C.POINTER(FrameStats)]),
    "mcrat_hip_snapshot_photons": (C.c_int, [_ctx]),
    "mcrat_hip_restore_photons": (C.c_int, [_ctx]),
    "mcrat_hip_num_virtual_ranks": (C.c_int, [_ctx]),
    "mcrat_hip_rank_stats": (C.c_int, [_ctx, C.c_int, C.POINTER(FrameStats)]),
    "mcrat_hip_pool_create": (C.c_int, [_ctx, C.c_int, C.c_int]),
    "mcrat_hip_pool_rank": (C.c_int, [_ctx, C.c_int, C.c_uint32, C.POINTER(_ctx)]),
    "mcrat_hip_pool_summaries": (C.c_int, [_ctx, C.POINTER(RankSummary)]),
    "mcrat_hip_pool_scatter_frames_cyclosynch": (C.c_int, [_ctx, C.POINTER(Cyclosynch), C.c_int, C.c_double, C.POINTER(PoolCsList), C.POINTER(FrameStats),
                                                           C.POINTER(CyclosynchCounts)]),
    "mcrat_hip_pool_begin_frames": (C.c_int, [_ctx, _ip, C.POINTER(C.c_uint64), _dp, _dp]),
    "mcrat_hip_pool_frame_stats": (C.c_int, [_ctx, C.POINTER(FrameStats)]),
    "mcrat_hip_pool_layout": (C.c_int, [_ctx, _ip, _ip]),
    "mcrat_hip_pool_run_frames": (C.c_int, [_ctx, C.POINTER(FramePlan), C.POINTER(FrameStats)]),
    "mcrat_hip_step_locate_sample": (C.c_int, [_ctx, C.c_int]),
    "mcrat_hip_step_event": (C.c_int, [_ctx, C.POINTER(FrameStats)]),
    "mcrat_hip_update_photon_position": (C.c_int, [_ctx, C.c_double]),
    "mcrat_hip_frame_statistics": (C.c_int, [_ctx, C.POINTER(FrameStats)]),
    "mcrat_hip_shared_clock_bytes_per_rank": (C.c_size_t, []),
    "mcrat_hip_shared_clock_attach": (C.c_int, [_ctx, C.c_int, C.c_int, C.c_longlong, C.c_void_p, C.c_void_p]),
    "mcrat_hip_shared_clock_attach_device": (C.c_int, [_ctx, C.c_int, C.c_int, C.c_longlong]),
    "mcrat_hip_shared_clock_peer_buffers": (C.c_int, [_ctx, C.POINTER(C.c_void_p), C.POINTER(C.c_size_t), C.POINTER(C.c_void_p), C.POINTER(C.c_size_t)]),
    "mcrat_hip_shared_clock_set_peers": (C.c_int, [_ctx, C.POINTER(C.c_void_p), C.POINTER(C.c_void_p)]),
    "mcrat_hip_shared_clock_exchange_push": (C.c_int, [_ctx]),
    "mcrat_hip_shared_clock_exchange_wait": (C.c_int, [_ctx]),
    "mcrat_hip_set_rng_tape": (C.c_int, [_ctx, _dp, C.c_longlong]),
    "mcrat_hip_rng_tape_position": (C.c_int, [_ctx, C.POINTER(C.c_longlong), _ip]),
    "mcrat_hip_pool_set_rng_tapes": (C.c_int, [_ctx, C.POINTER(_dp), C.POINTER(C.c_longlong)]),
    "mcrat_hip_pool_rng_tape_positions": (C.c_int, [_ctx, C.POINTER(C.c_longlong), _ip]),
    "mcrat_hip_shared_clock_exchange": (C.c_int, [_ctx]),
    "mcrat_hip_shared_clock_reset_exchange": (C.c_int, [_ctx]),
    "mcrat_hip_shared_clock_buffers": (C.c_int, [_ctx, C.POINTER(C.c_void_p), C.POINTER(C.c_void_p)]),
    "mcrat_hip_shared_clock_propose": (C.c_int, [_ctx]),
    "mcrat_hip_shared_clock_resolve": (C.c_int, [_ctx]),
    "mcrat_hip_shared_clock_poll": (C.c_int, [_ctx, _ip, C.POINTER(FrameStats)]),
    "mcrat_hip_shared_clock_finish": (C.c_int, [_ctx, C.POINTER(FrameStats)]),
    "mcrat_hip_ph_minmax": (C.c_int, [_ctx, _dp, _dp, _dp, _dp]),
    "mcrat_hip_scatt_stats": (C.c_int, [_ctx, _ip, _ip, _dp, _dp]),
    "mcrat_hip_avg_energy": (C.c_int, [_ctx, _dp]),
    "mcrat_hip_observe": (C.c_int, [_ctx, C.POINTER(Observer), C.c_double, C.POINTER(Observation)]),
    "mcrat_hip_pool_observe": (C.c_int, [_ctx, C.POINTER(Observer), _dp, C.POINTER(Observation)]),
    "mcrat_hip_observe_path": (C.c_int, [_ctx]),
    "mcrat_hip_sightline_rays": (C.c_int, [_ctx, _ctx, C.POINTER(SightlineParams), C.c_int, _dp, _dp, _dp, _dp, _dp, _dp, _dp, C.POINTER(Sightlines)]),
    "mcrat_hip_sightline_photons": (C.c_int, [_ctx, _ctx, C.POINTER(SightlineParams), C.POINTER(Sightlines)]),
    "mcrat_hip_pool_sightline_photons": (C.c_int, [_ctx, _ctx, C.POINTER(SightlineParams), C.POINTER(Sightlines)]),
    "mcrat_hip_synchronize": (C.c_int, [_ctx]),
    "mcrat_hip_device_bytes": (C.c_size_t, [_ctx]),
    "mcrat_hip_eval_function": (C.c_int, [_ctx, C.c_int, C.c_int, _dp, _dp, C.c_uint64]),
    "mcrat_hip_lookup_cell": (C.c_int, [_ctx, C.c_int, _dp, _dp, _dp, _ip]),
}

_lib = None


def load_library():
    global _lib
    if _lib is None:
        if not os.path.exists(LIB_PATH):
            raise RuntimeError(
                "libmcrat_hip.so is missing (%s): build it with `python -m mcrat_amd.build`; "
                "there is no CPU fallback for the photon loop" % LIB_PATH)
        try:
            import torch
        except ImportError:
            pass
        lib = C.CDLL(os.environ.get("MCRAT_HIP_LIB", LIB_PATH))
        for name, (res, args) in SYMBOLS.items():
            f = getattr(lib, name)
            f.restype, f.argtypes = res, args
        _lib = lib
    return _lib


class McratHipError(RuntimeError):
    pass


def _f8(a):
    return np.ascontiguousarray(a, dtype=np.float64)


def observer_angles(theta_obs_deg, dtheta_deg):
    th = np.radians(np.atleast_1d(_f8(theta_obs_deg)))
    half = 0.5 * np.radians(np.broadcast_to(_f8(dtheta_deg), th.shape))
    lo, hi = th - half, th + half
    cos_lo = np.where(lo <= 0.0, np.nextafter(1.0, 2.0), np.cos(np.maximum(lo, 0.0)))
    cos_hi = np.where(hi >= np.pi, -np.nextafter(1.0, 2.0), np.cos(np.minimum(hi, np.pi)))
    return np.cos(th), np.sin(th), cos_lo, cos_hi


class Engine:

    def __init__(self, dimensions, geometry, stokes=0, device=0, stream=None, rng_stream=0,
                 iterations_per_sync=0, use_graph=False, profile=False, virtual_rank_photons=0, tau_calculation=TAU_DIRECT,
                 cyclosynchrotron=0):
        self.lib = load_library()
        self.cfg = Config(ABI_VERSION, int(dimensions), int(geometry), int(bool(stokes)), int(tau_calculation), int(cyclosynchrotron),
                          int(device), C.c_void_p(stream) if stream else None, int(rng_stream),
                          int(iterations_per_sync), int(bool(use_graph)), int(bool(profile)), int(virtual_rank_photons))
        self.ctx = _ctx()
        rc = self.lib.mcrat_hip_init(C.byref(self.ctx), C.byref(self.cfg))
        if rc != 0:
            self.ctx = _ctx()
            raise McratHipError("mcrat_hip_init: %s" % self.lib.mcrat_hip_strerror(rc).decode())
        self.n = 0

    def close(self):
        if getattr(self, "ctx", None):
            if getattr(self, "pool", None) is None:
                self.lib.mcrat_hip_destroy(self.ctx)
            self.ctx = _ctx()
            for v in getattr(self, "views", {}).values():
                v.ctx = _ctx()

    def pool_create(self, n_ranks, slots_per_rank):
        self._check(self.lib.mcrat_hip_pool_create(self.ctx, int(n_ranks), int(slots_per_rank)), "pool_create")
        for v in getattr(self, "views", {}).values():
            v.ctx = _ctx()
        self.views = {}
        self.n_pool_ranks = int(n_ranks)
        self.n = int(self.lib.mcrat_hip_num_photon_slots(self.ctx))

    def pool_rank(self, rank, rng_stream=0):
        ctx = _ctx()
        self._check(self.lib.mcrat_hip_pool_rank(self.ctx, int(rank), int(rng_stream), C.byref(ctx)), "pool_rank")
        if not hasattr(self, "views"):
            self.views = {}
        v = self.views.get(rank)
        if v is None or v.ctx.value != ctx.value:
            v = Engine.__new__(Engine)
            v.lib, v.cfg, v.ctx, v.n, v.pool = self.lib, self.cfg, ctx, 0, self
            self.views[rank] = v
        v.n = int(self.lib.mcrat_hip_num_photon_slots(ctx))
        if getattr(self, "num_elements", None) is not None:
            v.num_elements = self.num_elements
        return v

    def pool_set_photons(self, ranks, records):
        n = len(ranks)
        arrs = [np.ascontiguousarray(a, dtype=PHOTON_DTYPE) for a in records]
        lists = (PhotonList * n)()
        for j, a in enumerate(arrs):
            nulls = int(np.count_nonzero(a["type"] == b"N"))
            lists[j] = PhotonList(a.ctypes.data, None, len(a) - nulls, nulls, len(a))
        rk = np.ascontiguousarray(ranks, dtype=np.int32)
        self._check(self.lib.mcrat_hip_pool_set_photons(self.ctx, n, rk.ctypes.data_as(_ip), C.cast(lists, C.c_void_p)), "pool_set_photons")
        for r in ranks:
            if hasattr(self, "views") and r in self.views:
                self.views[r].n = int(self.lib.mcrat_hip_num_photon_slots(self.views[r].ctx))

    def pool_scatter_frames_cyclosynch(self, lists, max_photons, fps, b_field_calc=1, epsilon_b=0.5, rebin_e_perc=0.1, rebin_ang=0.5, rebin_ang_phi=10.0):
        R = self.n_pool_ranks
        arr = (PoolCsList * R)()
        for r, d in enumerate(lists):
            if d is None:
                continue
            arr[r] = PoolCsList(1, int(d.get("emit_pool", 1)), int(d.get("scatt_frame_number", 0)), int(d.get("inj_frame_number", 0)), int(d["seed"]),
                                float(d["time_now"]), float(d["remaining_time"]), float(d["r_inj"]), float(d["ph_weight_suggest"]), float(d["theta_min"]),
                                float(d["theta_max"]))
        cs = Cyclosynch(int(b_field_calc), float(epsilon_b), float(rebin_e_perc), float(rebin_ang), float(rebin_ang_phi), 0, 0)
        st, cnt = (FrameStats * R)(), (CyclosynchCounts * R)()
        for r, d in enumerate(lists):
            if d is not None:
                cnt[r].scatt_cyclosynch_num_ph = int(d.get("scatt_cyclosynch_num_ph", 0))
        self._check(self.lib.mcrat_hip_pool_scatter_frames_cyclosynch(self.ctx, C.byref(cs), int(max_photons), float(fps), arr, st, cnt),
                    "pool_scatter_frames_cyclosynch")
        return list(st), list(cnt)

    def pool_inject_photons(self, fps, lists):
        R = self.n_pool_ranks
        arr = (PoolInjectList * R)()
        for r, q in enumerate(lists):
            if q is None:
                continue
            a = arr[r]
            a.inject, a.spect = 1, q["spect"].encode() if isinstance(q["spect"], str) else q["spect"]
            a.min_photons, a.max_photons = int(q["min_photons"]), int(q["max_photons"])
            a.r_inj, a.ph_weight, a.theta_min, a.theta_max, a.seed = float(q["r_inj"]), float(q["ph_weight"]), float(q["theta_min"]), float(q["theta_max"]), int(q["seed"])
        self._check(self.lib.mcrat_hip_pool_inject_photons(self.ctx, float(fps), arr), "pool_inject_photons")
        out = []
        for r, q in enumerate(lists):
            if q is None:
                out.append(None)
                continue
            v = self.views.get(r) if hasattr(self, "views") else None
            if v is not None:
                v.n = int(arr[r].num_photons)
            out.append((int(arr[r].num_photons), float(arr[r].ph_weight_adjusted)))
        return out

    def pool_summaries(self):
        out = (RankSummary * self.n_pool_ranks)()
        self._check(self.lib.mcrat_hip_pool_summaries(self.ctx, out), "pool_summaries")
        return list(out)

    def __del__(self):
        try:
            self.close()
        except Exception:
            pass

    def _check(self, rc, what):
# ... 387 lines not shown
        self._check(self.lib.mcrat_hip_frame_statistics(self.ctx, C.byref(st)), "frame_statistics")
        return st

    def update_photon_position(self, t):
        self._check(self.lib.mcrat_hip_update_photon_position(self.ctx, float(t)), "update_photon_position")

    def step_event(self):
        st = FrameStats()
        self._check(self.lib.mcrat_hip_step_event(self.ctx, C.byref(st)), "step_event")
        return st

    def shared_clock_bytes_per_rank(self):
        return int(self.lib.mcrat_hip_shared_clock_bytes_per_rank())

    def shared_clock_attach(self, world, rank, slot_base, send_ptr=None, recv_ptr=None):
        self._check(self.lib.mcrat_hip_shared_clock_attach(self.ctx, int(world), int(rank), int(slot_base),
                                                           C.c_void_p(send_ptr) if send_ptr else None,
                                                           C.c_void_p(recv_ptr) if recv_ptr else None), "shared_clock_attach")

    def shared_clock_attach_device(self, world, rank, slot_base):
        self._check(self.lib.mcrat_hip_shared_clock_attach_device(self.ctx, int(world), int(rank), int(slot_base)), "shared_clock_attach_device")
        r, f, rb, fb = C.c_void_p(), C.c_void_p(), C.c_size_t(), C.c_size_t()
        self._check(self.lib.mcrat_hip_shared_clock_peer_buffers(self.ctx, C.byref(r), C.byref(rb), C.byref(f), C.byref(fb)), "shared_clock_peer_buffers")
        return r.value, rb.value, f.value, fb.value

    def shared_clock_set_peers(self, peer_recv, peer_flags):
        n = len(peer_recv)
        a = (C.c_void_p * n)(*[C.c_void_p(x) for x in peer_recv])
        b = (C.c_void_p * n)(*[C.c_void_p(x) for x in peer_flags])
        self._check(self.lib.mcrat_hip_shared_clock_set_peers(self.ctx, a, b), "shared_clock_set_peers")

    def shared_clock_exchange_push(self):
        self._check(self.lib.mcrat_hip_shared_clock_exchange_push(self.ctx), "shared_clock_exchange_push")

    def shared_clock_exchange_wait(self):
        self._check(self.lib.mcrat_hip_shared_clock_exchange_wait(self.ctx), "shared_clock_exchange_wait")

    def shared_clock_reset_exchange(self):
        self._check(self.lib.mcrat_hip_shared_clock_reset_exchange(self.ctx), "shared_clock_reset_exchange")

    def shared_clock_propose(self):
        self._check(self.lib.mcrat_hip_shared_clock_propose(self.ctx), "shared_clock_propose")

    def shared_clock_resolve(self):
        self._check(self.lib.mcrat_hip_shared_clock_resolve(self.ctx), "shared_clock_resolve")

    def shared_clock_poll(self):
        st = FrameStats()
        done = C.c_int(0)
        self._check(self.lib.mcrat_hip_shared_clock_poll(self.ctx, C.byref(done), C.byref(st)), "shared_clock_poll")
        return bool(done.value), st

    def shared_clock_finish(self):
        st = FrameStats()
        self._check(self.lib.mcrat_hip_shared_clock_finish(self.ctx, C.byref(st)), "shared_clock_finish")
        return st

    def ph_minmax(self):
        v = [C.c_double() for _ in range(4)]
        self._check(self.lib.mcrat_hip_ph_minmax(self.ctx, *[C.byref(x) for x in v]), "ph_minmax")
        return tuple(x.value for x in v)

    def scatt_stats(self):
        mx, mn, avg, ravg = C.c_int(), C.c_int(), C.c_double(), C.c_double()
        self._check(self.lib.mcrat_hip_scatt_stats(self.ctx, C.byref(mx), C.byref(mn), C.byref(avg), C.byref(ravg)), "scatt_stats")
        return mx.value, mn.value, avg.value, ravg.value

    def avg_energy(self):
        e = C.c_double()
        self._check(self.lib.mcrat_hip_avg_energy(self.ctx, C.byref(e)), "avg_energy")
        return e.value

    def _observe(self, call, what, cos_obs, sin_obs, cos_lo, cos_hi, t_edges, e_edges, time_now):
        co, so, cl, ch, te, ee = (_f8(a).ravel() for a in (cos_obs, sin_obs, cos_lo, cos_hi, t_edges, e_edges))
        n_obs, n_t, n_e = len(co), len(te) - 1, len(ee) - 1
        if not (len(so) == len(cl) == len(ch) == n_obs):
            raise ValueError("%s: cos_obs, sin_obs, cos_lo and cos_hi must have one entry per observer" % what)
        obs = Observer(n_obs, co.ctypes.data_as(_dp), so.ctypes.data_as(_dp), cl.ctypes.data_as(_dp), ch.ctypes.data_as(_dp),
                       n_t, te.ctypes.data_as(_dp), n_e, ee.ctypes.data_as(_dp))
        shape = (max(n_obs, 0), max(n_t, 0), max(n_e, 0))
        res = {"count": np.zeros(shape, dtype=np.int64), "n_accepted": np.zeros(shape[0], dtype=np.int64), "n_outside": np.zeros(shape[0], dtype=np.int64)}
        for k in ("w", "we", "i", "q", "u", "v"):
            res[k] = np.zeros(shape)
        ll = C.POINTER(C.c_longlong)
        out = Observation(res["count"].ctypes.data_as(ll), *[res[k].ctypes.data_as(_dp) for k in ("w", "we", "i", "q", "u", "v")],
                          res["n_accepted"].ctypes.data_as(ll), res["n_outside"].ctypes.data_as(ll))
        self._check(call(self.ctx, C.byref(obs), time_now, C.byref(out)), what)
        return res

    def observe(self, cos_obs, sin_obs, cos_lo, cos_hi, t_edges, e_edges, time_now):
        return self._observe(self.lib.mcrat_hip_observe, "observe", cos_obs, sin_obs, cos_lo, cos_hi, t_edges, e_edges, float(time_now))

    def pool_observe(self, cos_obs, sin_obs, cos_lo, cos_hi, t_edges, e_edges, time_now):
        tn = _f8(time_now).ravel()
        if len(tn) != self.n_pool_ranks:
            raise ValueError("pool_observe: time_now needs one clock per rank of the pool")
        return self._observe(self.lib.mcrat_hip_pool_observe, "pool_observe", cos_obs, sin_obs, cos_lo, cos_hi, t_edges, e_edges, tn.ctypes.data_as(_dp))

    def observe_path(self):
        return int(self.lib.mcrat_hip_observe_path(self.ctx))

    def _sightlines(self, what, n, call, step_frac, h_min, max_steps, tau_stop, surface_level):
        par = SightlineParams(float(step_frac), float(h_min), int(max_steps), float(tau_stop), float(surface_level))
        m = max(int(n), 0)
        res = {"tau": np.zeros(m), "path": np.zeros(m), "steps": np.zeros(m, dtype=np.int32), "status": np.zeros(m, dtype=np.int32),
               "surface_step": np.zeros(m, dtype=np.int32), "surface_r": np.zeros((3, m))}
        out = Sightlines(res["tau"].ctypes.data_as(_dp), res["path"].ctypes.data_as(_dp), res["steps"].ctypes.data_as(_ip),
                         res["status"].ctypes.data_as(_ip), res["surface_step"].ctypes.data_as(_ip),
                         *[res["surface_r"][k].ctypes.data_as(_dp) for k in range(3)])
        self._check(call(C.byref(par), C.byref(out)), what)
        res["n_status"] = np.array(list(out.n_status), dtype=np.int64)
        return res

    def sightline_rays(self, r, p, step_frac, h_min, max_steps, tau_stop=np.inf, surface_level=-1.0, hydro=None):
        cols = [_f8(a).ravel() for a in list(r) + list(p)]
        if len(cols) != 7 or any(len(a) != len(cols[0]) for a in cols):
            raise ValueError("sightline_rays: r needs three and p four arrays of one length")
        n, h = len(cols[0]), hydro.ctx if hydro is not None else None
        ptrs = [a.ctypes.data_as(_dp) for a in cols]
        return self._sightlines("sightline_rays", n, lambda par, out: self.lib.mcrat_hip_sightline_rays(self.ctx, h, par, n, *ptrs, out),
                                step_frac, h_min, max_steps, tau_stop, surface_level)

    def sightline_photons(self, step_frac, h_min, max_steps, tau_stop=np.inf, surface_level=-1.0, hydro=None):
        h = hydro.ctx if hydro is not None else None
        n = int(self.lib.mcrat_hip_num_photon_slots(self.ctx))
        return self._sightlines("sightline_photons", n, lambda par, out: self.lib.mcrat_hip_sightline_photons(self.ctx, h, par, out),
                                step_frac, h_min, max_steps, tau_stop, surface_level)

    def pool_sightline_photons(self, step_frac, h_min, max_steps, tau_stop=np.inf, surface_level=-1.0, hydro=None):
        h = hydro.ctx if hydro is not None else None
        n = int(self.lib.mcrat_hip_num_photon_slots(self.ctx))
        return self._sightlines("pool_sightline_photons", n, lambda par, out: self.lib.mcrat_hip_pool_sightline_photons(self.ctx, h, par, out),
                                step_frac, h_min, max_steps, tau_stop, surface_level)

    def synchronize(self):
        self._check(self.lib.mcrat_hip_synchronize(self.ctx), "synchronize")

    def device_bytes(self):
        return int(self.lib.mcrat_hip_device_bytes(self.ctx))

    FN = dict(kn_cross_section=(1, 1, 1), lorentz_boost_photon=(2, 7, 4), lorentz_boost_electron=(3, 7, 4), stokes_rotation=(4, 13, 4),
              thermal_electron=(5, 5, 4), thermal_electron_wave=(6, 5, 4), electron_and_scatter=(7, 9, 13),
              rcp_nr=(8, 1, 1), rsqrt_nr=(9, 1, 1), sqrt_nr=(10, 1, 1), cell_operands=(11, 5, 5), boost_with_photon=(12, 9, 4),
              boost_with_electron=(13, 9, 4), boost_staged_photon=(14, 7, 4), optical_depth_staged=(15, 9, 2), azimuth=(16, 2, 4),
              hydro_coords=(17, 3, 3), thermal_cross_section=(18, 2, 4), kn_cross_section_ieee=(19, 1, 1))

    def eval_function(self, name, rows, seed=0):
        fn, wi, wo = self.FN[name]
        a = np.ascontiguousarray(rows, dtype=np.float64).reshape(-1, wi)
        out = np.empty((a.shape[0], wo))
        self._check(self.lib.mcrat_hip_eval_function(self.ctx, fn, a.shape[0], a.ctypes.data_as(_dp), out.ctypes.data_as(_dp), int(seed)), "eval_function")
        return out

    def lookup_cell(self, a0, a1, a2=None):
        a0, a1 = _f8(a0), _f8(a1)
        a2p = _f8(a2) if a2 is not None else None
        out = np.empty(len(a0), dtype=np.int32)
        self._check(self.lib.mcrat_hip_lookup_cell(self.ctx, len(a0), a0.ctypes.data_as(_dp), a1.ctypes.data_as(_dp),
                                                   a2p.ctypes.data_as(_dp) if a2p is not None else None,
                                                   out.ctypes.data_as(_ip)), "lookup_cell")
        return out
```

Before: 18.29 million.

## Add covered-octant table to skip bucket lookup and containment test on relocation

Builds, per grid bucket octant, a precomputed cell id when the hinted cell provably covers the whole octant with margin. Relocation and cell lookup then read one int plus the cell's fluid record instead of the bucket directory, a 128-byte fat cell and a well-inside geometric test. This costs extra grid memory and build work, plus a runtime branch between two template paths. Correctness relies on the conservative coverage check with its guard margins.

```diff
diff --git a/include/mcrat_hip.h b/include/mcrat_hip.h
--- a/include/mcrat_hip.h
+++ b/include/mcrat_hip.h
@@ -427,6 +427,7 @@
 int mcrat_hip_synchronize(mcrat_hip_ctx *ctx);
 size_t mcrat_hip_device_bytes(const mcrat_hip_ctx *ctx);
 int mcrat_hip_lookup_cell(mcrat_hip_ctx *ctx, int n, const double *a0, const double *a1, const double *a2, int *cell_out);
+long long mcrat_hip_covered_octants(mcrat_hip_ctx *ctx, int *out, long long cap);
 
 #if defined(__GNUC__)
 #pragma GCC visibility pop
diff --git a/mcrat_amd/csrc/device_types.hpp b/mcrat_amd/csrc/device_types.hpp
--- a/mcrat_amd/csrc/device_types.hpp
+++ b/mcrat_amd/csrc/device_types.hpp
@@ -108,6 +108,7 @@
     unsigned pad;
 };
 
+constexpr double GRID_ACCEPT_MARGIN = 1e-6;
 struct GridDev {
     const BucketDir *dir;
     const FatCell *cells;
@@ -116,7 +117,14 @@
     int dim[3];
     int logmap[3];
     int naxes;
-};
+    int cov_back;
+};
+static_assert(sizeof(GridDev) == 96, "cov_back fills what was padding");
+constexpr long long GRID_COVERED_MAX_INTS = 1ll << 26;
+#if defined(__HIPCC__)
+__host__ __device__
+#endif
+inline int covered_index(int code, int naxes) { return ((code & GRID_CODE_BUCKET_MASK) << naxes) | ((code >> GRID_CODE_OCT_SHIFT) & ((1 << naxes) - 1)); }
 
 struct HydroDev {
     const CellGeom *geom;
diff --git a/mcrat_amd/csrc/engine.hip b/mcrat_amd/csrc/engine.hip
--- a/mcrat_amd/csrc/engine.hip
+++ b/mcrat_amd/csrc/engine.hip
@@ -536,6 +536,7 @@
     GridScale scale{};
     GridPlan plan{};
     long long nb = 0, entries = 0;
+    size_t covered_ints = 0;
     bool any_hot = false;
     template <class T> T *cell_at(size_t o) const { return reinterpret_cast<T *>(static_cast<char *>(c->hy_buf) + o); }
     template <class T> T *grid_at(size_t o) const { return reinterpret_cast<T *>(static_cast<char *>(c->grid_buf) + o); }
@@ -661,7 +662,10 @@
 
 int ensure_grid_buffer(HydroStage &s)
 {
-    s.grid = grid_layout(s.nb, s.entries, grid_scan_scratch_ints(s.nb));
+    s.covered_ints = covered_table_ints(s.plan, s.nb, getenv("MCRAT_HIP_NO_COVERED") == nullptr);
+    s.grid = grid_layout(s.nb, s.entries, grid_scan_scratch_ints(s.nb), s.covered_ints);
+    if (getenv("MCRAT_HIP_VERBOSE"))
+        fprintf(stderr, "mcrat_hip: covered-octant table %zu B of the grid's %zu B\n", s.grid.dir - s.grid.covered, s.grid.total);
     return ensure_device_bytes(s.c, &s.c->grid_buf, &s.c->grid_bytes, s.grid.total);
 }
 
@@ -670,7 +674,8 @@
     mcrat_hip_ctx *c = s.c;
     const GridLayout &g = s.grid;
     HIPCHK(c, grid_build(s.plan, c->hy.geom, c->hy.geom2, c->hy.fluid, c->hy.fluid_c, s.M, c->grid_count, s.grid_at<int>(g.start), s.grid_at<int>(g.scan),
-                         s.grid_at<int>(g.entries), s.grid_at<FatCell>(g.cells), s.grid_at<BucketDir>(g.dir), s.nb, s.entries, c->stream));
+                         s.grid_at<int>(g.entries), s.grid_at<FatCell>(g.cells), s.grid_at<BucketDir>(g.dir),
+                         s.covered_ints ? s.grid_at<int>(g.covered) : nullptr, s.nb, s.entries, c->stream));
     HIPCHK(c, hipStreamSynchronize(c->stream));
     return MCRAT_HIP_OK;
 }
@@ -686,6 +691,7 @@
     for (size_t b = 0; b < (size_t)s.nb; ++b) {
         dir[b].e0 = g.start[b]; dir[b].n = g.start[b + 1] - g.start[b]; dir[b].hints = g.hints[b]; dir[b].pad = 0;
     }
+    if (s.covered_ints) memcpy(gh.data() + s.grid.covered, g.covered.data(), sizeof(int) * s.covered_ints);
     FatCell *fat = reinterpret_cast<FatCell *>(gh.data() + s.grid.cells);
     for (size_t e = 0; e < g.cells.size(); ++e) {
         const int ci = g.cells[e];
@@ -701,6 +707,7 @@
     hy.grid.dir = s.grid_at<const BucketDir>(s.grid.dir);
     hy.grid.cells = s.grid_at<const FatCell>(s.grid.cells);
     grid_plan_to_dev(s.plan, hy.grid);
+    hy.grid.cov_back = s.covered_ints ? (int)((s.grid.dir - s.grid.covered) / sizeof(int)) : 0;
     apply_hot_table(s.c);
 }
 
@@ -3972,6 +3979,23 @@
     return MCRAT_HIP_OK;
 }
 
+extern "C" long long mcrat_hip_covered_octants(mcrat_hip_ctx *c, int *out, long long cap)
+{
+    if (!c || cap < 0 || (cap > 0 && !out)) return MCRAT_HIP_EINVAL;
+    if (!c->have_hydro) return MCRAT_HIP_ESTATE;
+    const GridDev &g = c->hy.grid;
+    if (!g.cov_back) return 0;
+    const long long n = ((long long)g.dim[0] * g.dim[1] * g.dim[2]) << g.naxes;
+    if (std::min(n, cap) > 0) {
+        if (hipStreamSynchronize(c->stream) != hipSuccess ||
+            hipMemcpy(out, reinterpret_cast<const int *>(g.dir) - g.cov_back, sizeof(int) * (size_t)std::min(n, cap), hipMemcpyDeviceToHost) != hipSuccess) {
+            c->last_error = "covered_octants failed";
+            return MCRAT_HIP_EHIP;
+        }
+    }
+    return n;
+}
+
 extern "C" int mcrat_hip_lookup_cell(mcrat_hip_ctx *c, int n, const double *a0, const double *a1, const double *a2, int *out)
 {
     if (!c || n <= 0 || !a0 || !a1 || !out) return MCRAT_HIP_EINVAL;
diff --git a/mcrat_amd/csrc/grid_build.hip b/mcrat_amd/csrc/grid_build.hip
--- a/mcrat_amd/csrc/grid_build.hip
+++ b/mcrat_amd/csrc/grid_build.hip
@@ -177,7 +177,7 @@
 
 __global__ __launch_bounds__(256) void grid_finish_kernel(GridPlan p, long long nb, const int *__restrict__ start, int *__restrict__ entries,
                                                           const CellGeom *__restrict__ geom, const CellGeom2 *__restrict__ geom2,
-                                                          BucketDir *__restrict__ dir)
+                                                          BucketDir *__restrict__ dir, int *__restrict__ covered)
 {
     const long long b = (long long)blockIdx.x * 256 + threadIdx.x;
     if (b >= nb) return;
@@ -201,6 +201,7 @@
         half[k] = 0.5 * w;
     }
     unsigned char cnt[8] = {0, 0, 0, 0, 0, 0, 0, 0}, first[8] = {0, 0, 0, 0, 0, 0, 0, 0};
+    int cov[8] = {-1, -1, -1, -1, -1, -1, -1, -1};
     for (int e = 0; e < n; ++e) {
         const int ci = entries[e0 + e];
         const CellGeom g = geom[ci];
@@ -216,7 +217,10 @@
         for (int o = 0; o < nocts; ++o) {
             const bool reaches = r[0][o & 1] && r[1][(o >> 1) & 1] && r[2][(o >> 2) & 1];
             if (reaches) {
-                if (cnt[o] == 0) first[o] = (unsigned char)(e < (int)GRID_NO_HINT ? e : GRID_NO_HINT);
+                if (cnt[o] == 0) {
+                    first[o] = (unsigned char)(e < (int)GRID_NO_HINT ? e : GRID_NO_HINT);
+                    if (covered && e < (int)GRID_NO_HINT && octant_covered(p, bi, o, cc, ss)) cov[o] = ci;
+                }
                 if (cnt[o] < 2) cnt[o] += 1;
             }
         }
@@ -229,6 +233,8 @@
     BucketDir d;
     d.e0 = e0; d.n = n; d.hints = hints; d.pad = 0;
     dir[b] = d;
+    if (covered)
+        for (int o = 0; o < nocts; ++o) covered[(b << p.naxes) + o] = cnt[o] == 1 ? cov[o] : -1;
 }
 
 }
@@ -255,7 +261,7 @@
 }
 
 hipError_t grid_build(const GridPlan &p, const CellGeom *geom, const CellGeom2 *geom2, const CellFluid *fluid, const double *fluid_c, int M,
-                      unsigned *count, int *start, int *scan_scratch, int *entries, FatCell *cells, BucketDir *dir, long long nb,
+                      unsigned *count, int *start, int *scan_scratch, int *entries, FatCell *cells, BucketDir *dir, int *covered, long long nb,
                       long long total, hipStream_t stream)
 {
     hipError_t e = launch_exclusive_scan(count, nb, start, scan_scratch, total, stream);
@@ -263,7 +269,7 @@
     e = hipMemsetAsync(count, 0, sizeof(unsigned) * (size_t)nb, stream);
     if (e != hipSuccess) return e;
     grid_fill_kernel<<<dim3((M + 255) / 256), dim3(256), 0, stream>>>(p, geom, geom2, M, start, count, entries);
-    grid_finish_kernel<<<dim3((unsigned)((nb + 255) / 256)), dim3(256), 0, stream>>>(p, nb, start, entries, geom, geom2, dir);
+    grid_finish_kernel<<<dim3((unsigned)((nb + 255) / 256)), dim3(256), 0, stream>>>(p, nb, start, entries, geom, geom2, dir, covered);
     if (total > 0)
         grid_records_kernel<<<dim3((unsigned)((total + 255) / 256)), dim3(256), 0, stream>>>(p.naxes, total, entries, geom, geom2, fluid, fluid_c, cells);
     return hipGetLastError();
diff --git a/mcrat_amd/csrc/hydro_plan.hpp b/mcrat_amd/csrc/hydro_plan.hpp
--- a/mcrat_amd/csrc/hydro_plan.hpp
+++ b/mcrat_amd/csrc/hydro_plan.hpp
@@ -171,6 +171,7 @@
     long long nb = 0;
     std::vector<int> start, cells;
     std::vector<unsigned> hints;
+    std::vector<int> covered;
 };
 inline void cell_bucket_range(const GridPlan &p, int k, double c, double s, int &b0, int &b1)
 {
@@ -207,6 +208,43 @@
     }
     return h;
 }
+constexpr double GRID_COVER_GUARD = 64 * 2.220446049250313e-16;
+#if defined(__HIPCC__)
+__host__ __device__
+#endif
+inline bool octant_covered(const GridPlan &p, const int bi[3], int o, const double c[3], const double s[3])
+{
+    bool covered = true;
+    for (int k = 0; k < p.naxes; ++k) {
+        const double w = 1.0 / p.inv[k];
+        const double olo = p.org[k] + (bi[k] + 0.5 * ((o >> k) & 1)) * w, ohi = olo + 0.5 * w;
+        const double m = 0.5 * GRID_ACCEPT_MARGIN * w;
+        const bool holds = (c[k] - 0.5 * s[k] <= olo + m) & (c[k] + 0.5 * s[k] >= ohi - m);
+        const bool implied = m >= 1e-8 * s[k] + GRID_COVER_GUARD * (fabs(c[k]) + s[k]);
+        covered = covered & holds & implied & (p.logmap[k] == 0);
+    }
+    return covered;
+}
+inline size_t covered_table_ints(const GridPlan &p, long long nb, bool enabled)
+{
+    if (!enabled || nb <= 0) return 0;
+    for (int k = 0; k < p.naxes; ++k)
+        if (p.logmap[k]) return 0;
+    const long long ints = nb << p.naxes;
+    return ints > GRID_COVERED_MAX_INTS ? 0 : (size_t)ints;
+}
+inline void bucket_covered(const GridPlan &p, const int bi[3], const int *list, unsigned hints, const double *const c[3], const double *const s[3], int *out)
+{
+    for (int o = 0; o < (1 << p.naxes); ++o) {
+        const unsigned pick = (hints >> (4 * o)) & 15u;
+        out[o] = -1;
+        if (pick == GRID_NO_HINT) continue;
+        const int ci = list[pick];
+        double cc[3] = {0, 0, 0}, ss[3] = {0, 0, 0};
+        for (int k = 0; k < p.naxes; ++k) { cc[k] = c[k][ci]; ss[k] = s[k][ci]; }
+        if (octant_covered(p, bi, o, cc, ss)) out[o] = ci;
+    }
+}
 inline bool build_grid(const double *const c[3], const double *const s[3], int M, int naxes, GridHost &g)
 {
     GridScale scale;
@@ -249,12 +287,20 @@
         const int e0 = g.start[(size_t)b];
         g.hints[(size_t)b] = bucket_hints(p, bi, g.cells.data() + e0, g.start[(size_t)b + 1] - e0, c, s);
     }
+    g.covered.assign(covered_table_ints(p, nb, true), -1);
+    for (long long b = 0; b < nb && !g.covered.empty(); ++b) {
+        const int bi[3] = {(int)(b % p.dim[0]), (int)((b / p.dim[0]) % p.dim[1]), (int)(b / ((long long)p.dim[0] * p.dim[1]))};
+        bucket_covered(p, bi, g.cells.data() + g.start[(size_t)b], g.hints[(size_t)b], c, s, g.covered.data() + ((size_t)b << naxes));
+    }
     if (getenv("MCRAT_HIP_VERBOSE")) {
         const int nocts = 1 << naxes;
         long long hinted = 0;
         for (long long b = 0; b < nb; ++b)
             for (int o = 0; o < nocts; ++o) hinted += ((g.hints[(size_t)b] >> (4 * o)) & 15u) != GRID_NO_HINT;
         fprintf(stderr, "mcrat_hip: %.1f %% of the bucket octants have a single-cell hint\n", 100.0 * hinted / ((double)nb * nocts));
+        long long cov = 0;
+        for (int e : g.covered) cov += e >= 0;
+        fprintf(stderr, "mcrat_hip: %.1f %% of the bucket octants are covered by their hinted cell\n", 100.0 * cov / ((double)nb * nocts));
     }
     return true;
 }
@@ -314,12 +360,13 @@
     return l;
 }
 struct GridLayout {
-    size_t dir, cells, start, scan, entries, total;
-};
-inline GridLayout grid_layout(long long nb, long long entries, size_t scan_scratch_ints)
+    size_t dir, cells, start, scan, entries, total, covered;
+};
+inline GridLayout grid_layout(long long nb, long long entries, size_t scan_scratch_ints, size_t covered_ints = 0)
 {
     GridLayout l{};
     size_t off = 0;
+    l.covered = layout_take(off, sizeof(int) * covered_ints);
     l.dir = layout_take(off, sizeof(BucketDir) * (size_t)nb);
     l.cells = layout_take(off, sizeof(FatCell) * std::max<size_t>((size_t)entries, 1));
     l.start = layout_take(off, sizeof(int) * ((size_t)nb + 1));
diff --git a/mcrat_amd/csrc/kernels.hip b/mcrat_amd/csrc/kernels.hip
--- a/mcrat_amd/csrc/kernels.hip
+++ b/mcrat_amd/csrc/kernels.hip
@@ -267,7 +267,7 @@
     if (relocate) {
         phys::hydro_coords<DIMS, GEOM>(r0, r1, r2, a0, a1, a2);
         FatCell hit;
-        cell = phys::find_in_bucket<DIMS>(hy.grid, bucket, a0, a1, a2, hit);
+        cell = phys::find_in_bucket<DIMS>(hy, bucket, a0, a1, a2, hit);
         ph.idx(i) = cell;
         if (cell != -1) {
             fa = hit.a; fb = hit.b; fc = hit.c; fw = hit.w; fnsig = hit.nsig; fgam = hit.gam; fkf = phys::kf_of_gamma(hit.gam);
@@ -339,35 +339,51 @@
     bool *same;
 };
 
-template <int DIMS, int GEOM, int K, bool LOGS = false, class PH>
-__device__ __forceinline__ void relocate_lockstep(const PH &ph, const HydroDev &hy, const int (&slot)[K], bool (&todo)[K],
-                                                  const double (&r0)[K], const double (&r1)[K], const double (&a0)[K], const double (&a1)[K],
-                                                  const double (&a2)[K], const int (&code)[K], const uint64_t (&bits)[K], const unsigned (&fl)[K],
-                                                  bool count_it, double (&t)[K], int &relocated, const LockstepProbe *probe = nullptr)
+template <int DIMS, int GEOM, int K, bool LOGS, bool COVERED, class PH>
+__device__ __forceinline__ void relocate_lockstep_impl(const PH &ph, const HydroDev &hy, const int (&slot)[K], bool (&todo)[K],
+                                                       const double (&r0)[K], const double (&r1)[K], const double (&a0)[K], const double (&a1)[K],
+                                                       const double (&a2)[K], const int (&code)[K], const uint64_t (&bits)[K], const unsigned (&fl)[K],
+                                                       bool count_it, double (&t)[K], int &relocated, const LockstepProbe *probe)
 {
     static_assert(!TABLE_MODE, "DIRECT optical depths");
     const GridDev &g = hy.grid;
-    BucketDir d[K];
     double p0[K], p1[K], p2[K], p3[K];
     bool take[K];
+    FatCell f[K];
+    if constexpr (COVERED) {
+        int cell[K];
+#pragma unroll
+        for (int k = 0; k < K; ++k) {
+            take[k] = todo[k] && code[k] >= 0 && (code[k] & GRID_CODE_HINT_OK) != 0;
+            cell[k] = phys::covered_cell<DIMS>(g, take[k] ? code[k] : 0);
+            const int i = slot[k];
+            p0[k] = ph.p0(i); p1[k] = ph.p1(i); p2[k] = ph.p2(i); p3[k] = ph.p3(i);
+        }
+#pragma unroll
+        for (int k = 0; k < K; ++k) {
+            take[k] = take[k] & (cell[k] >= 0);
+            phys::fat_from_fluid(hy.fluid, take[k] ? cell[k] : 0, f[k]);
+        }
+    } else {
+        BucketDir d[K];
+#pragma unroll
+        for (int k = 0; k < K; ++k) {
+            take[k] = todo[k] && code[k] >= 0;
+            d[k] = g.dir[take[k] ? (code[k] & GRID_CODE_BUCKET_MASK) : 0];
+            const int i = slot[k];
+            p0[k] = ph.p0(i); p1[k] = ph.p1(i); p2[k] = ph.p2(i); p3[k] = ph.p3(i);
+        }
+#pragma unroll
+        for (int k = 0; k < K; ++k) {
+            const unsigned hint = (d[k].hints >> (4 * ((code[k] >> GRID_CODE_OCT_SHIFT) & 7))) & 15u;
+            take[k] = take[k] & (d[k].n > 0) & ((code[k] & GRID_CODE_HINT_OK) != 0) & (hint != GRID_NO_HINT);
+            f[k] = g.cells[take[k] ? d[k].e0 + (int)hint : 0];
+        }
+    }
+    double comv[K][4], tau[K], ntau[K];
 #pragma unroll
     for (int k = 0; k < K; ++k) {
-        take[k] = todo[k] && code[k] >= 0;
-        d[k] = g.dir[take[k] ? (code[k] & GRID_CODE_BUCKET_MASK) : 0];
-        const int i = slot[k];
-        p0[k] = ph.p0(i); p1[k] = ph.p1(i); p2[k] = ph.p2(i); p3[k] = ph.p3(i);
-    }
-    FatCell f[K];
-#pragma unroll
-    for (int k = 0; k < K; ++k) {
-        const unsigned hint = (d[k].hints >> (4 * ((code[k] >> GRID_CODE_OCT_SHIFT) & 7))) & 15u;
-        take[k] = take[k] & (d[k].n > 0) & ((code[k] & GRID_CODE_HINT_OK) != 0) & (hint != GRID_NO_HINT);
-        f[k] = g.cells[take[k] ? d[k].e0 + (int)hint : 0];
-    }
-    double comv[K][4], tau[K], ntau[K];
-#pragma unroll
-    for (int k = 0; k < K; ++k) {
-        take[k] = take[k] & phys::well_in_fat_cell<DIMS>(f[k], a0[k], a1[k], a2[k]);
+        if constexpr (!COVERED) take[k] = take[k] & phys::well_in_fat_cell<DIMS>(f[k], a0[k], a1[k], a2[k]);
         double cphi, sphi;
         phys::relocation_azimuth<DIMS, GEOM>(r0[k], r1[k], a0[k], cphi, sphi);
         double beta[3];
@@ -398,6 +414,15 @@
         if (count_it) relocated += 1;
         todo[k] = false;
     }
+}
+template <int DIMS, int GEOM, int K, bool LOGS = false, class PH>
+__device__ __forceinline__ void relocate_lockstep(const PH &ph, const HydroDev &hy, const int (&slot)[K], bool (&todo)[K],
+                                                  const double (&r0)[K], const double (&r1)[K], const double (&a0)[K], const double (&a1)[K],
+                                                  const double (&a2)[K], const int (&code)[K], const uint64_t (&bits)[K], const unsigned (&fl)[K],
+                                                  bool count_it, double (&t)[K], int &relocated, const LockstepProbe *probe = nullptr)
+{
+    if (hy.grid.cov_back) relocate_lockstep_impl<DIMS, GEOM, K, LOGS, true>(ph, hy, slot, todo, r0, r1, a0, a1, a2, code, bits, fl, count_it, t, relocated, probe);
+    else relocate_lockstep_impl<DIMS, GEOM, K, LOGS, false>(ph, hy, slot, todo, r0, r1, a0, a1, a2, code, bits, fl, count_it, t, relocated, probe);
 }
 
 struct PairIn {
diff --git a/mcrat_amd/csrc/launch.hpp b/mcrat_amd/csrc/launch.hpp
--- a/mcrat_amd/csrc/launch.hpp
+++ b/mcrat_amd/csrc/launch.hpp
@@ -282,7 +282,7 @@
 hipError_t launch_rebin_pool_range(const PhotonDev &pool, int three, const RebinPoolList *lists, int n_lists, RebinRange *out, hipStream_t stream);
 hipError_t launch_rebin_pool(const PhotonDev &pool, RebinPoolList *lists, int n_lists, char *scratch, hipStream_t stream);
 hipError_t grid_build(const GridPlan &p, const CellGeom *geom, const CellGeom2 *geom2, const CellFluid *fluid, const double *fluid_c, int M,
-                      unsigned *count, int *start, int *scan_scratch, int *entries, FatCell *cells, BucketDir *dir, long long nb,
+                      unsigned *count, int *start, int *scan_scratch, int *entries, FatCell *cells, BucketDir *dir, int *covered, long long nb,
                       long long total, hipStream_t stream);
 hipError_t launch_lookup(const KernelConfig &kc, const HydroDev &hy, int n, const double *a0, const double *a1,
                          const double *a2, int *out, hipStream_t stream);
diff --git a/mcrat_amd/csrc/physics.hpp b/mcrat_amd/csrc/physics.hpp
--- a/mcrat_amd/csrc/physics.hpp
+++ b/mcrat_amd/csrc/physics.hpp
@@ -163,10 +163,27 @@
 }
 
 template <int DIMS>
-__device__ __forceinline__ int find_in_bucket(const GridDev &g, int code, double a0, double a1, double a2, FatCell &hit)
-{
+__device__ __forceinline__ int covered_cell(const GridDev &g, int code)
+{
+    return reinterpret_cast<const int *>(g.dir)[covered_index(code, DIMS == DIM_THREE ? 3 : 2) - g.cov_back];
+}
+__device__ __forceinline__ void fat_from_fluid(const CellFluid *fluid, int cell, FatCell &hit)
+{
+    const double2 ab = *reinterpret_cast<const double2 *>(&fluid[cell].a), cw = *reinterpret_cast<const double2 *>(&fluid[cell].c),
+                  ng = *reinterpret_cast<const double2 *>(&fluid[cell].nsig);
+    hit.a = ab.x; hit.b = ab.y; hit.c = cw.x; hit.w = cw.y; hit.nsig = ng.x; hit.gam = ng.y;
+    hit.cell = cell;
+}
+template <int DIMS>
+__device__ __forceinline__ int find_in_bucket(const HydroDev &h, int code, double a0, double a1, double a2, FatCell &hit)
+{
+    const GridDev &g = h.grid;
     hit.cell = -1;
     if (code < 0) return -1;
+    if (g.cov_back && (code & GRID_CODE_HINT_OK)) {
+        const int cell = covered_cell<DIMS>(g, code);
+        if (cell >= 0) { fat_from_fluid(h.fluid, cell, hit); return cell; }
+    }
     const BucketDir d = g.dir[code & GRID_CODE_BUCKET_MASK];
     if (d.n <= 0) return -1;
     const unsigned hint = (d.hints >> (4 * ((code >> GRID_CODE_OCT_SHIFT) & 7))) & 15u;
@@ -181,7 +198,7 @@
 __device__ __forceinline__ int find_containing_block(const HydroDev &h, double a0, double a1, double a2)
 {
     FatCell hit;
-    return find_in_bucket<DIMS>(h.grid, grid_bucket_of<DIMS>(h.grid, a0, a1, a2), a0, a1, a2, hit);
+    return find_in_bucket<DIMS>(h, grid_bucket_of<DIMS>(h.grid, a0, a1, a2), a0, a1, a2, hit);
 }
 
 template <int DIMS>
diff --git a/mcrat_amd/csrc/sightline.hip b/mcrat_amd/csrc/sightline.hip
--- a/mcrat_amd/csrc/sightline.hip
+++ b/mcrat_amd/csrc/sightline.hip
@@ -131,7 +131,7 @@
                 FatCell hit;
                 hit.cell = -1;
                 if (phys::in_domain<DIMS>(hy, a0, a1, a2))
-                    phys::find_in_bucket<DIMS>(hy.grid, phys::grid_bucket_of<DIMS>(hy.grid, a0, a1, a2), a0, a1, a2, hit);
+                    phys::find_in_bucket<DIMS>(hy, phys::grid_bucket_of<DIMS>(hy.grid, a0, a1, a2), a0, a1, a2, hit);
                 if (hit.cell < 0) {
                     status = SIGHTLINE_LEFT_MESH;
                 } else {
diff --git a/mcrat_amd/engine.py b/mcrat_amd/engine.py
--- a/mcrat_amd/engine.py
+++ b/mcrat_amd/engine.py
@@ -298,6 +298,7 @@
     "mcrat_hip_device_bytes": (C.c_size_t, [_ctx]),
     "mcrat_hip_eval_function": (C.c_int, [_ctx, C.c_int, C.c_int, _dp, _dp, C.c_uint64]),
     "mcrat_hip_lookup_cell": (C.c_int, [_ctx, C.c_int, _dp, _dp, _dp, _ip]),
+    "mcrat_hip_covered_octants": (C.c_longlong, [_ctx, _ip, C.c_longlong]),
 }
 
 _lib = None
@@ -991,6 +992,14 @@
         self._check(self.lib.mcrat_hip_eval_function(self.ctx, fn, a.shape[0], a.ctypes.data_as(_dp), out.ctypes.data_as(_dp), int(seed)), "eval_function")
         return out
 
+    def covered_octants(self):
+        n = int(self.lib.mcrat_hip_covered_octants(self.ctx, None, 0))
+        self._check(min(n, 0), "covered_octants")
+        out = np.empty(n, dtype=np.int32)
+        if n:
+            self._check(min(int(self.lib.mcrat_hip_covered_octants(self.ctx, out.ctypes.data_as(_ip), n)), 0), "covered_octants")
+        return out
+
     def lookup_cell(self, a0, a1, a2=None):
         a0, a1 = _f8(a0), _f8(a1)
         a2p = _f8(a2) if a2 is not None else None
```

Measured after the change: 21.39 million (median of 6 runs). +17.0%, better.
